# ColumbiaDVMM/ColumbiaImageSearch

Hardware: AMD Instinct MI355X
Metric: queries/sec @ recall@10 on 10M LOPQ index (higher is better)
Workload: dtype f64

## Files before the change

### columbiaimagesearch_amd/_lib.py

```python
import ctypes
import os
from ctypes import POINTER, c_char_p, c_double, c_float, c_int, c_int32, c_int64, c_uint8, c_uint16, c_uint32, c_void_p

import numpy as np

CIS_F32, CIS_F64 = 4, 8
CIS_OK, CIS_EINVAL, CIS_EHIP, CIS_ENOMEM, CIS_EUNSUPPORTED, CIS_ENODEVICE = 0, -1, -2, -3, -4, -5

_HERE = os.path.dirname(os.path.abspath(__file__))
LIB_PATH = os.environ.get("CIS_LIB_PATH") or os.path.join(_HERE, "lib", "libcis_hip.so")


class cis_hit(ctypes.Structure):
    _fields_ = [("dist", c_double), ("visit_rank", c_uint32), ("pos", c_uint32), ("id", c_int64),
                ("cell", c_int32), ("reserved", c_int32)]


HIT_DTYPE = np.dtype([("dist", "<f8"), ("visit_rank", "<u4"), ("pos", "<u4"), ("id", "<i8"),
                      ("cell", "<i4"), ("reserved", "<i4")])
assert HIT_DTYPE.itemsize == ctypes.sizeof(cis_hit) == 32


class HipError(RuntimeError):
    """A HIP runtime call inside libcis_hip.so failed (or no gfx950 device is visible)."""
# ... 7 lines not shown
    "cis_set_device": (c_int, [c_int]),
    "cis_selftest": (c_int, [POINTER(c_int)]),
    "cis_model_create": (c_int, [POINTER(c_void_p), c_int, c_int, c_int, c_int, c_int, c_int, c_void_p, c_void_p,
                                 c_void_p, c_void_p, c_void_p, c_void_p, c_int, c_int]),
    "cis_model_destroy": (None, [c_void_p]),
    "cis_apply_pca": (c_int, [c_void_p, c_void_p, c_int, c_int64, c_void_p]),
    "cis_encode": (c_int, [c_void_p, c_void_p, c_int, c_int64, c_void_p, c_void_p]),
    "cis_encode_dev": (c_int, [c_void_p, c_void_p, c_int, c_int64, c_void_p, c_void_p, c_void_p]),
    "cis_predict_coarse": (c_int, [c_void_p, c_void_p, c_int, c_int64, c_void_p]),
    "cis_project": (c_int, [c_void_p, c_void_p, c_int, c_int64, c_void_p, c_void_p]),
    "cis_predict_fine": (c_int, [c_void_p, c_void_p, c_int, c_int64, c_void_p, c_void_p]),
    "cis_subquantizer_distances": (c_int, [c_void_p, c_void_p, c_int, c_int64, c_void_p, c_void_p]),
    "cis_reconstruct": (c_int, [c_void_p, c_void_p, c_void_p, c_int64, c_void_p]),
    "cis_predict_cluster": (c_int, [c_void_p, c_int, c_void_p, c_int, c_int64, c_int, c_int, c_void_p]),
    "cis_multisequence": (c_int, [c_void_p, c_int, c_void_p, c_void_p, c_int, c_int64, c_int, c_int, c_int, c_void_p, c_void_p,
                                  POINTER(c_int)]),
    "cis_index_create": (c_int, [POINTER(c_void_p), c_void_p]),
    "cis_index_destroy": (None, [c_void_p]),
    "cis_index_create_view": (c_int, [POINTER(c_void_p), c_void_p]),
    "cis_index_insert_counters": (c_int, [c_void_p, c_void_p]),
    "cis_index_set_shard": (c_int, [c_void_p, c_int, c_int, c_void_p]),
    "cis_index_cell_counts": (c_int, [c_void_p, c_void_p]),
    "cis_index_add_remote_counts": (c_int, [c_void_p, c_void_p]),
    "cis_index_add": (c_int, [c_void_p, c_void_p, c_void_p, c_void_p, c_int64, c_int, POINTER(c_int64)]),
    "cis_index_size": (c_int64, [c_void_p]),
    "cis_index_add_dev": (c_int, [c_void_p, c_void_p, c_void_p, c_void_p, c_int64, c_int, POINTER(c_int64), POINTER(c_int64),
                                  c_void_p, c_void_p]),
    "cis_l2_normalize_dev": (c_int, [c_void_p, c_int, c_int64, c_int, c_void_p]),
    "cis_index_cell_counts_dev": (c_int, [c_void_p, c_void_p, c_void_p]),
    "cis_index_add_remote_counts_dev": (c_int, [c_void_p, c_void_p, c_void_p]),
    "cis_index_route_pack_dev": (c_int, [c_void_p, c_void_p, c_void_p, c_void_p, c_int64, c_void_p, c_void_p, c_void_p]),
    "cis_index_add_records_dev": (c_int, [c_void_p, c_void_p, c_int64, c_int, POINTER(c_int64), POINTER(c_int64), c_void_p,
                                          c_void_p]),
    "cis_index_get_cell": (c_int, [c_void_p, c_int, c_int, c_int64, c_void_p, c_void_p, POINTER(c_int64)]),
    "cis_index_get_codes": (c_int, [c_void_p, c_void_p, c_void_p, c_int64, c_void_p]),
    "cis_index_search": (c_int, [c_void_p, c_void_p, c_int, c_int, c_int64, c_int, c_void_p, c_void_p, c_void_p,
                                 c_void_p, c_void_p, c_void_p]),
    "cis_index_search_async": (c_int, [c_void_p, c_void_p, c_int, c_int, c_int64, c_int, c_void_p, c_void_p, c_void_p,
                                       c_void_p, c_void_p, c_void_p]),
    "cis_index_search_wait": (c_int, [c_void_p]),
    "cis_host_alloc": (c_int, [POINTER(c_void_p), ctypes.c_size_t]),
    "cis_host_free": (None, [c_void_p]),
    "cis_index_search_dev": (c_int, [c_void_p, c_void_p, c_int, c_int, c_int64, c_int, c_void_p, c_void_p, c_void_p,
                                     c_void_p, c_void_p, c_void_p, c_void_p]),
    "cis_index_search_partial_dev": (c_int, [c_void_p, c_void_p, c_int, c_int, c_int64, c_int, c_void_p, c_void_p,
                                             c_void_p]),
    "cis_index_query_owners_dev": (c_int, [c_void_p, c_void_p, c_int, c_int, c_int64, c_void_p, c_void_p, c_void_p]),
    "cis_routed_merge_tables_dev": (c_int, [c_void_p, c_int, c_int, c_void_p, c_void_p, c_int, c_void_p, c_void_p, c_void_p]),
    "cis_route_queries_dev": (c_int, [c_void_p, c_int, c_int, c_void_p, c_int, c_int, c_void_p, c_void_p, c_void_p, c_void_p, c_void_p]),
    "cis_index_search_partial_packed_dev": (c_int, [c_void_p, c_void_p, c_int, c_int, c_int64, c_int, c_void_p, c_void_p,
                                                    c_void_p, c_void_p, c_void_p, c_void_p]),
    "cis_merge_hits_dev": (c_int, [c_void_p, c_int, c_int, c_int, c_void_p, c_void_p, c_void_p, c_void_p, c_void_p,
                                   c_void_p]),
    "cis_merge_packed_dev": (c_int, [c_void_p, c_int, c_int64, c_void_p, c_void_p, c_int, c_int, c_void_p, c_void_p,
                                     c_void_p, c_void_p, c_void_p, c_void_p]),
    "cis_pyramid_down2_dev": (c_int, [c_void_p, c_int, c_int, c_void_p, c_void_p, c_void_p]),
    "cis_extract_chips_dev": (c_int, [c_void_p, c_int, c_int, c_void_p, c_int, c_int, c_void_p, c_void_p]),
    "cis_exchange_offsets_dev": (c_int, [c_void_p, c_int, c_int, c_int64, c_void_p, c_void_p, c_void_p, c_void_p]),
    "cis_rerank_dev": (c_int, [c_void_p, c_int, c_int64, c_int, c_void_p, c_int, c_void_p, c_int, c_void_p, c_void_p]),
    "cis_idmap_build_dev": (c_int, [c_void_p, c_int64, c_void_p, c_void_p, c_int64, c_void_p]),
    "cis_idmap_lookup_dev": (c_int, [c_void_p, c_void_p, c_int64, c_int64, c_void_p, c_int64, c_void_p, c_void_p]),
    "cis_rerank_select_dev": (c_int, [c_void_p, c_int, c_int64, c_int, c_void_p, c_void_p, c_int64, c_void_p, c_int, c_void_p,
                                      c_void_p, c_int, c_int, c_int, c_int, c_double, c_void_p, c_void_p, c_void_p, c_void_p,
                                      c_void_p]),
    "cis_exact_knn_dev": (c_int, [c_void_p, c_int, c_int64, c_int, c_void_p, c_int, c_int, c_int, c_int64, c_int, c_void_p, c_void_p,
                                  c_void_p]),
    "cis_exact_knn": (c_int, [c_void_p, c_int, c_int64, c_int, c_void_p, c_int, c_int, c_int, c_int64, c_int, c_void_p, c_void_p]),
    "cis_exact_knn_set_mode": (c_int, [c_int]),
    "cis_exact_knn_stats": (c_int, [c_void_p]),
    "cis_kmeans": (c_int, [c_void_p, c_int64, c_int, c_int, c_int, c_void_p, c_void_p, c_void_p]),
    "cis_train_gram": (c_int, [c_void_p, c_int64, c_int, c_void_p, c_int, c_void_p, c_void_p]),
    "cis_train_project": (c_int, [c_void_p, c_int64, c_int, c_void_p, c_int, c_void_p, c_void_p, c_void_p]),
    "cis_index_last_stats": (c_int, [c_void_p, c_void_p]),
    "cis_index_last_scan_kernel": (c_int, [c_void_p]),
    "cis_cnn_create": (c_int, [POINTER(c_void_p), c_int, c_void_p, c_int]),
    "cis_cnn_destroy": (None, [c_void_p]),
    "cis_cnn_create_view": (c_int, [POINTER(c_void_p), c_void_p]),
    "cis_cnn_feat_dim": (c_int, [c_int]),
    "cis_cnn_forward": (c_int, [c_void_p, c_void_p, c_int, c_void_p]),
    "cis_cnn_forward_dev": (c_int, [c_void_p, c_void_p, c_int, c_void_p, c_void_p]),
    "cis_index_set_profiling": (c_int, [c_void_p, c_int]),
    "cis_index_set_scan_mode": (c_int, [c_void_p, c_int]),
    "cis_index_stream_counters": (c_int, [c_void_p, c_void_p]),
    "cis_index_read_profile": (c_int, [c_void_p, c_void_p, POINTER(c_int64)]),
}

_lib = None


def exported_symbols():
    return sorted(_PROTOS)


def _load_hip_runtime():
    cands = []
    try:
        import torch
        cands.append(os.path.join(os.path.dirname(torch.__file__), "lib", "libamdhip64.so"))
    except ImportError:
        pass
    cands += ["libamdhip64.so.7", "/opt/rocm/lib/libamdhip64.so.7", "/opt/rocm/lib/libamdhip64.so", "libamdhip64.so"]
    for c in cands:
        try:
            return ctypes.CDLL(c, mode=ctypes.RTLD_GLOBAL)
        except OSError:
            continue
    raise ImportError("no HIP runtime (libamdhip64.so) found: install ROCm or PyTorch-ROCm")


def lib():
    global _lib
    if _lib is None:
        if not os.path.exists(LIB_PATH):
            raise ImportError(
                "%s not found: build it with `python -c 'import __graft_entry__ as g; g.build()'` "
                "(or `make -C columbiaimagesearch_amd/csrc`). columbiaimagesearch_amd has no CPU fallback." % LIB_PATH)
        _load_hip_runtime()
        L = ctypes.CDLL(LIB_PATH)
        for name, (res, args) in _PROTOS.items():
            fn = getattr(L, name)
            fn.restype = res
            fn.argtypes = args
        _lib = L
    return _lib


def last_error():
    return lib().cis_last_error().decode("utf-8", "replace")


def check(rc):
    if rc == CIS_OK:
        return
    msg = last_error()
    if rc == CIS_EINVAL:
        raise ValueError(msg)
    if rc == CIS_EUNSUPPORTED:
        raise NotImplementedError(msg)
    if rc == CIS_ENOMEM:
        raise MemoryError(msg)
    raise HipError(msg)


def ptr(a):
    if a is None:
        return None
    assert a.flags["C_CONTIGUOUS"]
    return a.ctypes.data_as(c_void_p)


def dtype_code(a):
    if a.dtype == np.float32:
        return CIS_F32
    if a.dtype == np.float64:
        return CIS_F64
    raise ValueError("only float32 / float64 vectors are supported, got %s" % a.dtype)


def as_float_matrix(x, cols=None):
    a = np.asarray(x)
    if a.dtype != np.float32 and a.dtype != np.float64:
        a = a.astype(np.float64)
    if a.ndim == 1:
        a = a[None, :]
    if a.ndim != 2:
        raise ValueError("expected a vector or a matrix of vectors, got shape %r" % (a.shape,))
# ... 41 lines not shown
```

### columbiaimagesearch_amd/csrc/lopq_batch.h

```cpp
#pragma once
#include <atomic>
#include <chrono>

#include "lopq_index.h"
#include "scan_common.h"

static const int GRP_SUB = 32;
#define GRP_WORDS(V) (6 * (V) * GRP_SUB + 2)
#define GRP_TILES(V) ((2 * (V) * GRP_SUB + 1023) / 1024)

static const int PLAN_PAR_STAGE = 4096;

struct Front {
    const void* xc;
    int ct;
    int* grp_cnt;
};

static const float* coarse_centroids(const cis_model* m, float) { return m->d_Cs32; }
static const double* coarse_centroids(const cis_model* m, double) { return m->d_Cs64; }

struct Scan2Geom { int G, NW, U, S; size_t lds; };

struct Route {
    bool w_pow2;
    bool split_tables;
    bool big;
    bool fast;
    bool tiny_cells;
    bool use3;
    bool stream_hint;
    bool par_plan, fused_front;
    int seg_max;
    int64_t stream_min;
    Scan2Geom geom;
    bool direct;
    bool stream;
    bool use5;
    bool drop_t32;
    Scan3Geom geom3;
    int S;
};

struct Batch {
    cis_index* ix;
    const void* dQ;
    int q_dtype, nq;
    int64_t quota;
    int L;
    SearchOut out;
    hipStream_t st;
    Front f;
    PlanOut* plan;
    int64_t *item_off, *tab_off, *totals;
    unsigned long long* qbound;
    int *grp_cur, *grp_base;
    int* plan_fb;
    uint64_t* vis_list;
    int vis_cap;
    unsigned long long* plan_hint;
    int hint_slot;
    const int64_t* d_tot;
    int64_t n_items, n_tabs, n_cand_all;
    WorkItem* items;
    TabDesc* tabs;
    int* tab_order;
    double *T, *px_buf;
    float* T32;
    cis_index::ProfRec pr;
    std::chrono::steady_clock::time_point t_entry;
};

static int mark(Batch& b, int i) {
    if (!b.ix->profiling) return CIS_OK;
    if (b.ix->profiling == 1 && i != 5 && i != 3) return CIS_OK;
    CIS_CHECK_HIP(hipEventCreate(&b.pr.ev[i]));
    CIS_CHECK_HIP(hipEventRecord(b.pr.ev[i], b.st));
    return CIS_OK;
}

struct Slots {
    int* qctr;
    int* n_slots;
    int* fhdr;
    int* slots;
    int* fslots;
    int64_t max_slots;
};
enum SlotMode {
    SLOTS_SORTED,
    SLOTS_IDENTITY,
    SLOTS_NONE
};

int front_prepare(cis_index* ix, const void* dQ, int q_dtype, int nq, hipStream_t st, Front* f);
template <typename CT>
int front_count(Batch& b, const Route& r);
int dump_plan_fallbacks(const Batch& b);
int plan_totals(Batch& b, const Route& r);
template <typename CT>
void emit_plan(Batch& b, const Route& r);
int build_slots(const Batch& b, SlotMode mode, int G, int64_t CH , int seg_max, Slots* s);
```

### columbiaimagesearch_amd/csrc/lopq_host.hip

```cpp
#include <algorithm>
#include <mutex>

#include "lopq_index.h"

static std::mutex g_copy_mu;
static hipStream_t g_copy_stream[64] = {nullptr};
static int cis_copy_stream(int device, hipStream_t* out) {
    std::lock_guard<std::mutex> lk(g_copy_mu);
    const int d = device & 63;
    if (!g_copy_stream[d]) CIS_CHECK_HIP(hipStreamCreateWithFlags(&g_copy_stream[d], hipStreamNonBlocking));
    *out = g_copy_stream[d];
    return CIS_OK;
}

static std::vector<cis_index*> g_host_pending;

static hipError_t host_copy_out_locked(cis_index* ix, hipStream_t cp) {
    const cis_index::HostOut& o = ix->h_out;
    const int nq = o.nq, L = o.L;
    hipError_t e = hipSuccess;
    auto cpy = [&](void* dst, const void* src, size_t bytes) { if (e == hipSuccess && dst) e = hipMemcpyAsync(dst, src, bytes, hipMemcpyDeviceToHost, cp); };
    if (nq > 0) {
        if (L > 0) {
            cpy(o.ids, ix->w_oids.p, (size_t)nq * L * sizeof(int64_t));
// ... 13 lines not shown
    for (size_t i = 0; i < g_host_pending.size();) {
        cis_index* o = g_host_pending[i];
        if (o != self && o->m->device == device && hipEventQuery(o->h_ev_out) == hipSuccess && host_copy_out_locked(o, cp) == hipSuccess) {
            g_host_pending[i] = g_host_pending.back();
            g_host_pending.pop_back();
        } else {
            ++i;
        }
    }
    (void)hipGetLastError();
}

void cis_host_forget(cis_index* ix) {
    std::lock_guard<std::mutex> lk(g_copy_mu);
    g_host_pending.erase(std::remove(g_host_pending.begin(), g_host_pending.end(), ix), g_host_pending.end());
}

static void host_abandon(cis_index* ix) {
    std::lock_guard<std::mutex> lk(g_copy_mu);
    g_host_pending.erase(std::remove(g_host_pending.begin(), g_host_pending.end(), ix), g_host_pending.end());
    ix->h_out = {nullptr, nullptr, nullptr, nullptr, nullptr, nullptr, 0, 0};
}

extern "C" int cis_host_alloc(void** out, size_t bytes) {
    CIS_REQUIRE(out != nullptr, "out is NULL");
    *out = nullptr;
    CIS_TRY(cis_lazy_init());
    hipError_t e = hipHostMalloc(out, bytes > 0 ? bytes : 1, hipHostMallocDefault);
    if (e != hipSuccess) {
        cis_set_error("hipHostMalloc(%zu) failed: %s", bytes, hipGetErrorString(e));
        *out = nullptr;
        return CIS_ENOMEM;
    }
    return CIS_OK;
}

extern "C" void cis_host_free(void* p) {
    if (p) (void)hipHostFree(p);
}

extern "C" int cis_index_search_wait(cis_index* ix);

extern "C" int cis_index_search_async(cis_index* ix, const void* Q, int q_dtype, int nq, int64_t quota, int limit,
                                      int64_t* ids, double* dists, int32_t* n_found, int32_t* visited, int32_t* cells,
                                      uint32_t* pos) {
    CIS_REQUIRE(ix != nullptr, "index is NULL");
    CIS_REQUIRE(q_dtype == CIS_F32 || q_dtype == CIS_F64, "q_dtype must be 4 or 8");
    int L;
    CIS_TRY(effective_limit(quota, limit, &L));
    if (nq == 0) return CIS_OK;
    CIS_REQUIRE(Q && n_found && visited && (L == 0 || (ids && dists)), "NULL buffer");
    CIS_TRY(cis_lazy_init());
    CIS_CHECK_HIP(hipSetDevice(ix->m->device));
    hipStream_t cp = nullptr;
    CIS_TRY(cis_copy_stream(ix->m->device, &cp));
    if (!ix->h_stream) {
        CIS_CHECK_HIP(hipStreamCreateWithFlags(&ix->h_stream, hipStreamNonBlocking));
        CIS_CHECK_HIP(hipEventCreateWithFlags(&ix->h_ev_in, hipEventDisableTiming));
        CIS_CHECK_HIP(hipEventCreateWithFlags(&ix->h_ev_out, hipEventDisableTiming));
        CIS_CHECK_HIP(hipEventCreateWithFlags(&ix->h_ev_done, hipEventDisableTiming));
    }
    hipStream_t st = ix->h_stream;
    if (ix->h_pending) CIS_TRY(cis_index_search_wait(ix));
    const size_t qbytes = (size_t)nq * ix->m->D_in * q_dtype;
    const int Lk = L > 0 ? L : 1;
    CIS_TRY(ix->w_q.reserve(qbytes));
    CIS_TRY(ix->w_oids.reserve((size_t)nq * Lk * sizeof(int64_t)));
    CIS_TRY(ix->w_odists.reserve((size_t)nq * Lk * sizeof(double)));
    CIS_TRY(ix->w_onf.reserve((size_t)nq * sizeof(int32_t)));
    CIS_TRY(ix->w_ovis.reserve((size_t)nq * sizeof(int32_t)));
    CIS_TRY(ix->w_ocell.reserve((size_t)nq * Lk * sizeof(int32_t)));
    CIS_TRY(ix->w_opos.reserve((size_t)nq * Lk * sizeof(uint32_t)));
    {
        std::lock_guard<std::mutex> lk(g_copy_mu);
        CIS_CHECK_HIP(hipMemcpyAsync(ix->w_q.p, Q, qbytes, hipMemcpyHostToDevice, cp));
        CIS_CHECK_HIP(hipEventRecord(ix->h_ev_in, cp));
        host_pump_locked(ix->m->device, cp, ix);
    }
    struct Guard {
        cis_index* ix; hipStream_t st; bool armed;
        ~Guard() { if (armed) { (void)hipStreamSynchronize(st); ix->h_pending = false; host_abandon(ix); } }
    } guard{ix, st, true};
    CIS_CHECK_HIP(hipStreamWaitEvent(st, ix->h_ev_in, 0));
    int rc = cis_index_search_dev(ix, ix->w_q.p, q_dtype, nq, quota, limit, ix->w_oids.as<int64_t>(),
                                  ix->w_odists.as<double>(), ix->w_onf.as<int32_t>(), ix->w_ovis.as<int32_t>(),
                                  ix->w_ocell.as<int32_t>(), ix->w_opos.as<uint32_t>(), st);
    if (rc != CIS_OK) return rc;
    CIS_CHECK_HIP(hipEventRecord(ix->h_ev_out, st));
    ix->h_out = {ids, dists, n_found, visited, cells, pos, nq, L};
    ix->h_out_enqueued = false;
    ix->h_pending = true;
    guard.armed = false;
    {
        std::lock_guard<std::mutex> lk(g_copy_mu);
        g_host_pending.push_back(ix);
    }
    return CIS_OK;
}

static int host_wait_pending(cis_index* ix) {
    CIS_CHECK_HIP(hipSetDevice(ix->m->device));
    ix->h_pending = false;
    hipStream_t cp = nullptr;
    CIS_TRY(cis_copy_stream(ix->m->device, &cp));
    bool enq;
    {
        std::lock_guard<std::mutex> lk(g_copy_mu);
        enq = ix->h_out_enqueued;
    }
    if (!enq) {
        CIS_CHECK_HIP(hipEventSynchronize(ix->h_ev_out));
        std::lock_guard<std::mutex> lk(g_copy_mu);
        if (!ix->h_out_enqueued) {
            g_host_pending.erase(std::remove(g_host_pending.begin(), g_host_pending.end(), ix), g_host_pending.end());
            CIS_CHECK_HIP(host_copy_out_locked(ix, cp));
        }
        host_pump_locked(ix->m->device, cp, ix);
    }
    CIS_CHECK_HIP(hipEventSynchronize(ix->h_ev_done));
    return CIS_OK;
}

extern "C" int cis_index_search_wait(cis_index* ix) {
    CIS_REQUIRE(ix != nullptr, "index is NULL");
    if (!(ix->h_stream && ix->h_pending)) return CIS_OK;
    const int rc = host_wait_pending(ix);
    if (rc != CIS_OK) {
        ix->h_pending = false;
        host_abandon(ix);
    }
    return rc;
}

extern "C" int cis_index_search(cis_index* ix, const void* Q, int q_dtype, int nq, int64_t quota, int limit,
                                int64_t* ids, double* dists, int32_t* n_found, int32_t* visited, int32_t* cells,
                                uint32_t* pos) {
    CIS_TRY(cis_index_search_async(ix, Q, q_dtype, nq, quota, limit, ids, dists, n_found, visited, cells, pos));
    return cis_index_search_wait(ix);
}
```

### columbiaimagesearch_amd/csrc/lopq_index.h

```cpp
#pragma once
#include "lopq_model.h"

struct CellStore {
    DevBuf codes[2];
    DevBuf ids[2];
    DevBuf loff[2];
    DevBuf cmax;
    int cur = 0;
    int64_t n = 0;
    int64_t cap = 0;
    bool with_codes = true;
    bool init = false;
    void release() {
        for (int i = 0; i < 2; ++i) { codes[i].release(); ids[i].release(); loff[i].release(); }
        cmax.release();
    }
};

struct cis_index {
    cis_model* m = nullptr;
    int V = 0, M = 0;
    int64_t ncells = 0;
    int rank = 0, world = 1;
    std::vector<int32_t> owner;
    DevBuf d_owner;
    CellStore own;
    CellStore ghost;
    DevBuf d_gcount;
    DevBuf d_plan_hint;
    bool had_plain_remote = false;
    int64_t nb_indexed = 0;
    bool stats_fresh = false;
    int64_t n_inplace = 0, n_rebuild = 0;
    cis_index* base = nullptr;
    std::vector<cis_index*> views;
    bool orphaned = false;
    const cis_index* st() const { return base ? base : this; }
    const uint8_t* codes_ptr() const { const cis_index* s = st(); return s->own.codes[s->own.cur].as<uint8_t>(); }
    const int64_t* ids_ptr() const { const cis_index* s = st(); return s->own.ids[s->own.cur].as<int64_t>(); }
    const int64_t* loff_ptr() const { const cis_index* s = st(); return s->own.loff[s->own.cur].as<int64_t>(); }
    const int64_t* gcount_ptr() const { return st()->d_gcount.as<int64_t>(); }
    unsigned long long* plan_hint_ptr() const { return st()->d_plan_hint.as<unsigned long long>(); }
    void sync_from_base() {
        if (!base) return;
        ncells = base->ncells; rank = base->rank; world = base->world; nb_indexed = base->nb_indexed; n_local = base->n_local;
        n_total = base->n_total; max_cell = base->max_cell; nonempty_cells = base->nonempty_cells;
    }
    int64_t n_local = 0;
    DevBuf wi_key[2], wi_val[2], wi_hist, wi_sid, wi_acc, wi_apre, wi_tmp, wi_in_ids, wi_in_coarse, wi_in_fine, wi_scan, wi_cnt, wi_cnt2;
    DevBuf d_stats;
    int64_t* h_ins = nullptr;
    DevBuf w_slack;
    DevBuf w_planfb, w_vis;
    DevBuf w_tiles;
    DevBuf w_xp, w_cd, w_order, w_sorted, w_plan, w_off, w_items, w_tabs, w_T, w_hits, w_hitn, w_part, w_q,
        w_oids, w_odists, w_onf, w_ovis, w_ocell, w_opos, w_order2, w_px, w_T32, w_grp, w_tord, w_y64, w_x64;
    int64_t stats[4] = {0, 0, 0, 0};
    bool force_exact_scan = false;
    bool force_scan2 = false;
    bool force_scan3 = false;
    int force_two_pass = -1;
    int batch_hint = 0;
    int64_t batch_hint_quota = -1;
    double retry_fraction = 0.5;
    int m16_holdoff = 0;
    int64_t m16_backoffs = 0;
    int last_scan_kernel = 0;
    bool force_prefilter_scan = false;
    hipStream_t h_stream = nullptr;
    hipEvent_t h_ev_in = nullptr, h_ev_out = nullptr, h_ev_done = nullptr;
    bool h_pending = false;
    bool h_out_enqueued = false;
    struct HostOut { int64_t* ids; double* dists; int32_t* n_found; int32_t* visited; int32_t* cells; uint32_t* pos; int nq, L; };
    HostOut h_out = {nullptr, nullptr, nullptr, nullptr, nullptr, nullptr, 0, 0};
    bool force_scan5 = false;
    DevBuf w_s5;
    DevBuf w_bmin;
    bool force_stream = false;
    bool stream_off = false;
    int64_t stream_batches = 0, stream_fallbacks = 0;
    int profiling = 0;
    int64_t* h_totals = nullptr;
    int64_t* d_h_totals = nullptr;
    int64_t plan_seq = 0;
    int64_t stats_pending_seq = 0;
    int64_t n_total = 0, max_cell = 0, nonempty_cells = 0;
    struct ProfRec { hipEvent_t ev[6]; bool has_scan; };
    std::vector<ProfRec> prof;
    double prof_ms[5] = {0, 0, 0, 0, 0};
    int64_t prof_launches = 0;

    bool owns(int64_t cell) const {
        if (world <= 1) return true;
        if (!owner.empty()) return owner[cell] == rank;
        return (int)(cell % world) == rank;
    }
};

int cis_index_ready(cis_index* ix);

void cis_host_forget(cis_index* ix);

static const int MAX_LDS_LIMIT = 3072;
static const int MAX_LIMIT = 1 << 24;

static inline int effective_limit(int64_t quota, int limit, int* L) {
    int64_t l = limit < 0 ? quota : limit;
    if (l < 0) l = 0;
    if (l > MAX_LIMIT) {
        cis_set_error("limit=%lld exceeds the %d ranked results per query supported by this build", (long long)l, MAX_LIMIT);
        return CIS_EUNSUPPORTED;
    }
    *L = (int)l;
    return CIS_OK;
}

int cis_search_partial(cis_index* ix, const void* dQ, int q_dtype, int nq, int64_t quota, int L, cis_hit* d_hits, int32_t* d_n_found,
                       int32_t* d_visited, hipStream_t st);
```

### columbiaimagesearch_amd/csrc/lopq_index.hip

```cpp
#include <algorithm>

#include "lopq_index.h"

static const int SCAN_T = 256, SCAN_PER = 8, SCAN_TILE = SCAN_T * SCAN_PER;

template <typename T>
__device__ __forceinline__ T wave_incl_scan(T v) {
    const int lane = threadIdx.x & 63;
#pragma unroll
    for (int o = 1; o < 64; o <<= 1) {
        const T u = __shfl_up(v, o);
        if (lane >= o) v += u;
    }
    return v;
}

template <typename T>
__device__ __forceinline__ T block_excl_scan(T v, T* sh , T* total) {
    const int lane = threadIdx.x & 63, w = threadIdx.x >> 6;
    const T inc = wave_incl_scan(v);
    if (lane == 63) sh[w] = inc;
    __syncthreads();
    T base = 0, tot = 0;
#pragma unroll
// ... 31 lines not shown
template <typename TO>
__global__ __launch_bounds__(SCAN_T) void k_scan_sums(TO* __restrict__ sums, int64_t m, TO* __restrict__ total, int64_t* __restrict__ total2) {
    __shared__ TO sh[SCAN_T / 64 + 1];
    TO carry = 0;
    for (int64_t b = 0; b < m; b += SCAN_T) {
        const int64_t i = b + threadIdx.x;
        const TO v = i < m ? sums[i] : (TO)0;
        TO tot;
        const TO e = block_excl_scan<TO>(v, sh, &tot);
        if (i < m) sums[i] = carry + e;
        carry += tot;
    }
    if (threadIdx.x == 0) {
        if (total) total[0] = carry;
        if (total2) total2[0] = (int64_t)carry;
    }
}

template <typename TO>
__global__ __launch_bounds__(SCAN_T) void k_scan_add(TO* __restrict__ out, const TO* __restrict__ sums, int64_t n) {
    const TO add = sums[blockIdx.x];
    const int64_t base = (int64_t)blockIdx.x * SCAN_TILE + (int64_t)threadIdx.x * SCAN_PER;
#pragma unroll
    for (int i = 0; i < SCAN_PER; ++i)
        if (base + i < n) out[base + i] += add;
}

template <typename TI, typename TO>
static void dev_exclusive_scan(const TI* in, TO* out, int64_t n, TO* sums, TO* total, int64_t* total2, hipStream_t st) {
    const int64_t m = n > 0 ? ceil_div(n, SCAN_TILE) : 0;
    if (m > 0) hipLaunchKernelGGL((k_scan_tiles<TI, TO>), dim3((unsigned)m), dim3(SCAN_T), 0, st, in, out, sums, n);
    hipLaunchKernelGGL((k_scan_sums<TO>), dim3(1), dim3(SCAN_T), 0, st, sums, m, total, total2);
    if (m > 1) hipLaunchKernelGGL((k_scan_add<TO>), dim3((unsigned)m), dim3(SCAN_T), 0, st, out, (const TO*)sums, n);
}

static const int RS_ROWS = 32, RS_TILE = RS_ROWS * 64;

__global__ __launch_bounds__(64) void k_rs_hist(const uint32_t* __restrict__ key, int64_t n, int shift, uint32_t* __restrict__ H, int nblk) {
    __shared__ uint32_t h[256];
    for (int i = threadIdx.x; i < 256; i += 64) h[i] = 0;
    __syncthreads();
    const int64_t base = (int64_t)blockIdx.x * RS_TILE;
    for (int r = 0; r < RS_ROWS; ++r) {
        const int64_t i = base + r * 64 + threadIdx.x;
        if (i < n) atomicAdd(&h[(key[i] >> shift) & 255u], 1u);
    }
    __syncthreads();
    for (int d = threadIdx.x; d < 256; d += 64) H[(int64_t)d * nblk + blockIdx.x] = h[d];
}

__global__ __launch_bounds__(64) void k_rs_scatter(const uint32_t* __restrict__ key, const uint32_t* __restrict__ val, int64_t n, int shift,
                                                   const uint32_t* __restrict__ H, int nblk, uint32_t* __restrict__ key_out,
                                                   uint32_t* __restrict__ val_out) {
    __shared__ uint32_t base[256];
    for (int d = threadIdx.x; d < 256; d += 64) base[d] = H[(int64_t)d * nblk + blockIdx.x];
    __syncthreads();
    const int lane = threadIdx.x;
    const int64_t b0 = (int64_t)blockIdx.x * RS_TILE;
    for (int r = 0; r < RS_ROWS; ++r) {
        const int64_t i = b0 + r * 64 + lane;
        const bool ok = i < n;
        const uint32_t k = ok ? key[i] : 0u;
        const uint32_t v = ok ? val[i] : 0u;
        const uint32_t d = (k >> shift) & 255u;
        unsigned long long peers = __ballot(ok);
#pragma unroll
        for (int b = 0; b < 8; ++b) {
            const unsigned long long m = __ballot((d >> b) & 1u);
            peers &= ((d >> b) & 1u) ? m : ~m;
        }
        const int before = __builtin_amdgcn_mbcnt_hi((unsigned)(peers >> 32), __builtin_amdgcn_mbcnt_lo((unsigned)peers, 0));
        const uint32_t start = base[d];
        __syncthreads();
        if (ok) {
            key_out[start + before] = k;
            val_out[start + before] = v;
            if (before == 0) base[d] = start + (uint32_t)__popcll(peers);
        }
        __syncthreads();
    }
}

enum { INS_ACC_OWN = 0, INS_INVALID = 1, INS_NTOTAL = 2, INS_MAXCELL = 3, INS_NONEMPTY = 4, INS_ERR = 5, INS_ACC_GHOST = 6,
       INS_REMOTE_PLAIN = 7, INS_OVERFLOW = 8, INS_WORDS = 9 };

__device__ __forceinline__ bool dev_owns(int64_t cell, const int32_t* __restrict__ owner, int rank, int world) {
    if (world <= 1) return true;
    return owner ? owner[cell] == rank : (int)(cell % world) == rank;
}

__global__ void k_ins_keys(const int64_t* __restrict__ ids, const uint16_t* __restrict__ coarse, const uint8_t* __restrict__ fine,
                           int64_t n, int V, int M, int K, const int32_t* __restrict__ owner, int rank, int world, int sel,
                           int dedup, uint32_t* __restrict__ key, uint32_t* __restrict__ val, int64_t* __restrict__ idv,
                           int64_t* __restrict__ gcount, int64_t* __restrict__ stats) {
    const int64_t i = (int64_t)blockIdx.x * blockDim.x + threadIdx.x;
    if (i >= n) return;
    const int c0 = coarse[2 * i], c1 = coarse[2 * i + 1];
    const int64_t id = ids[i];
    bool valid = c0 < V && c1 < V && id >= 0;
    if (valid && K < 256) {
        for (int j = 0; j < M; ++j) valid = valid && fine[i * M + j] < K;
    }
    uint32_t k = 0;
    int64_t keep = -1;
    if (!valid) {
        if (sel == 0) atomicAdd((unsigned long long*)&stats[INS_INVALID], 1ull);
    } else {
        const int64_t cell = (int64_t)c0 * V + c1;
        const bool mine = dev_owns(cell, owner, rank, world);
        if (mine == (sel == 0)) {
            k = (uint32_t)cell;
            keep = id;
        } else if (sel == 0 && !dedup) {
            atomicAdd((unsigned long long*)&gcount[cell], 1ull);
            atomicAdd((unsigned long long*)&stats[INS_REMOTE_PLAIN], 1ull);
        }
    }
    key[i] = k;
    val[i] = (uint32_t)i;
    idv[i] = keep;
}

__global__ void k_ins_gather(const int64_t* __restrict__ idv, const uint32_t* __restrict__ perm, int64_t n, int64_t* __restrict__ sid) {
    const int64_t j = (int64_t)blockIdx.x * blockDim.x + threadIdx.x;
    if (j < n) sid[j] = idv[perm[j]];
}

__device__ __forceinline__ int64_t lower_bound_u32(const uint32_t* __restrict__ a, int64_t n, uint32_t x) {
    int64_t lo = 0, hi = n;
    while (lo < hi) {
        const int64_t mid = (lo + hi) >> 1;
        if (a[mid] < x) lo = mid + 1;
        else hi = mid;
    }
    return lo;
}

__global__ __launch_bounds__(256) void k_ins_dedup(const uint32_t* __restrict__ key, const int64_t* __restrict__ sid, int64_t n, int dedup,
                                                   const int64_t* __restrict__ loff, const int64_t* __restrict__ lend,
                                                   const int64_t* __restrict__ old_ids, const unsigned long long* __restrict__ cmaxp,
                                                   uint32_t* __restrict__ acc) {
    const int64_t j = (int64_t)blockIdx.x * 4 + (threadIdx.x >> 6);
    const int lane = threadIdx.x & 63;
    if (j >= n) return;
    const int64_t id = sid[j];
    uint32_t a = id >= 0 ? 1u : 0u;
    if (a && dedup) {
        const uint32_t c = key[j];
        bool dup = false;
        if ((unsigned long long)id < cmaxp[c]) {
            const int64_t b = loff[c], e = lend[c];
            for (int64_t p0 = b; p0 < e && !dup; p0 += 64) {
                const int64_t p = p0 + lane;
                dup = __ballot(p < e && old_ids[p] == id) != 0ull;
            }
        }
        if (!dup) {
            const int64_t first = lower_bound_u32(key, n, c);
            for (int64_t j0 = first; j0 < j && !dup; j0 += 64) {
                const int64_t jj = j0 + lane;
                dup = __ballot(jj < j && sid[jj] == id) != 0ull;
            }
        }
        a = dup ? 0u : 1u;
    }
    if (lane == 0) acc[j] = a;
}
// ... 224 lines not shown
    if (on) {
        const int64_t dst = lend[c] + (int64_t)(pre - s_pre[l0]);
        const bool fits = dst < loff[c + 1];
        if (!fits) { s_over = 1; stats[INS_OVERFLOW] = 1; }
        const int64_t id = sid[j];
        if (fits) {
            ids_cur[dst] = id;
            if (codes_cur) {
                const int64_t i = perm[j];
                for (int bb = 0; bb < M; ++bb) codes_cur[dst * M + bb] = fine[i * M + bb];
            }
        }
        v = (unsigned long long)id + 1ull;
    }
    const uint32_t cm = on ? c : 0xffffffffu;
#pragma unroll
    for (int o = 1; o < 64; o <<= 1) {
        const unsigned long long u = __shfl_up(v, o);
        const uint32_t cu = __shfl_up(cm, o);
        if (lane >= o && cu == cm && u > v) v = u;
    }
    const uint32_t cn = __shfl_down(cm, 1);
    if (on && (lane == 63 || cn != cm)) atomicMax(&cmaxp[c], v);
    __threadfence();
    __syncthreads();
    if (s_over != 0) return;
    if (j < n && (j + 1 >= n || s_key[j + 1] != c)) {
        const int64_t add = (int64_t)(pre + a) - (int64_t)s_pre[l0];
        if (add > 0) {
            lend[c] += add;
            gcount[c] += add;
        }
    }
    if (!do_stats) return;
    __threadfence();
    __syncthreads();
    long long sum = 0, mx = 0, ne = 0;
    for (int64_t cc = j; cc < ncells; cc += 1024) {
        const long long g = gcount[cc];
        sum += g;
        mx = g > mx ? g : mx;
        ne += g > 0;
    }
    for (int o = 32; o > 0; o >>= 1) {
        sum += __shfl_xor(sum, o);
        const long long m2 = __shfl_xor(mx, o);
        mx = m2 > mx ? m2 : mx;
        ne += __shfl_xor(ne, o);
    }
    if (lane == 0) { s_sum[wv] = sum; s_max[wv] = mx; s_ne[wv] = ne; }
    __syncthreads();
    if (j == 0) {
        for (int w = 1; w < 16; ++w) { sum += s_sum[w]; mx = s_max[w] > mx ? s_max[w] : mx; ne += s_ne[w]; }
        stats[INS_NTOTAL] = sum; stats[INS_MAXCELL] = mx; stats[INS_NONEMPTY] = ne;
    }
}

__global__ __launch_bounds__(256) void k_gcount_stats(const int64_t* __restrict__ gcount, int64_t ncells, int64_t* __restrict__ stats) {
    __shared__ long long s_sum[4], s_max[4], s_ne[4];
    long long sum = 0, mx = 0, ne = 0;
    for (int64_t c = (int64_t)blockIdx.x * blockDim.x + threadIdx.x; c < ncells; c += (int64_t)gridDim.x * blockDim.x) {
        const long long g = gcount[c];
        sum += g;
        mx = g > mx ? g : mx;
        ne += g > 0;
    }
    for (int o = 32; o > 0; o >>= 1) {
        sum += __shfl_xor(sum, o);
        const long long m2 = __shfl_xor(mx, o);
        mx = m2 > mx ? m2 : mx;
        ne += __shfl_xor(ne, o);
    }
    const int w = threadIdx.x >> 6;
    if ((threadIdx.x & 63) == 0) { s_sum[w] = sum; s_max[w] = mx; s_ne[w] = ne; }
    __syncthreads();
    if (threadIdx.x == 0) {
        for (int i = 1; i < 4; ++i) { sum += s_sum[i]; mx = s_max[i] > mx ? s_max[i] : mx; ne += s_ne[i]; }
        atomicAdd((unsigned long long*)&stats[INS_NTOTAL], (unsigned long long)sum);
        atomicMax((unsigned long long*)&stats[INS_MAXCELL], (unsigned long long)mx);
        atomicAdd((unsigned long long*)&stats[INS_NONEMPTY], (unsigned long long)ne);
    }
}

__global__ void k_cell_delta(const int64_t* __restrict__ gcount, int64_t* __restrict__ delta, int64_t ncells) {
    const int64_t c = (int64_t)blockIdx.x * blockDim.x + threadIdx.x;
    if (c < ncells) delta[c] = gcount[c] - delta[c];
}

__global__ void k_add_remote(int64_t* __restrict__ gcount, const int64_t* __restrict__ delta, int64_t ncells,
                             const int32_t* __restrict__ owner, int rank, int world, int64_t* __restrict__ stats) {
    const int64_t c = (int64_t)blockIdx.x * blockDim.x + threadIdx.x;
    if (c >= ncells) return;
    const int64_t d = delta[c];
    if (d < 0) { stats[INS_ERR] = 1; return; }
    if (d == 0 || dev_owns(c, owner, rank, world)) return;
    gcount[c] += d;
}

__global__ void k_get_codes(const int32_t* __restrict__ cells, const uint32_t* __restrict__ pos, int64_t n, int64_t ncells,
                            const int64_t* __restrict__ loff, const uint8_t* __restrict__ codes, int M, uint8_t* __restrict__ out,
                            int64_t* __restrict__ stats) {
    const int64_t i = (int64_t)blockIdx.x * blockDim.x + threadIdx.x;
    if (i >= n) return;
    const int64_t c = cells[i];
    if (c < 0 || c >= ncells) { stats[INS_ERR] = 1 + i; return; }
    const int64_t a = loff[c], b = loff[ncells + 1 + c];
    if ((int64_t)pos[i] >= b - a) { stats[INS_ERR] = 1 + i; return; }
    for (int j = 0; j < M; ++j) out[i * M + j] = codes[(a + pos[i]) * M + j];
}

__global__ void k_route_keys(const uint16_t* __restrict__ coarse, int64_t n, int V, const int32_t* __restrict__ owner, int world,
                             uint32_t* __restrict__ key, uint32_t* __restrict__ val, int64_t* __restrict__ counts) {
    const int64_t i = (int64_t)blockIdx.x * blockDim.x + threadIdx.x;
    if (i >= n) return;
    const int c0 = coarse[2 * i], c1 = coarse[2 * i + 1];
    uint32_t dst = 0;
    if (c0 < V && c1 < V) {
        const int64_t cell = (int64_t)c0 * V + c1;
        dst = (uint32_t)(owner ? owner[cell] : (int)(cell % world));
    }
    key[i] = dst;
    val[i] = (uint32_t)i;
    atomicAdd((unsigned long long*)&counts[dst], 1ull);
}

__global__ void k_route_pack(const uint32_t* __restrict__ perm, const int64_t* __restrict__ ids, const uint16_t* __restrict__ coarse,
                             const uint8_t* __restrict__ fine, int64_t n, int M, uint8_t* __restrict__ rec) {
    const int64_t j = (int64_t)blockIdx.x * blockDim.x + threadIdx.x;
    if (j >= n) return;
    const int64_t i = perm[j];
    uint8_t* r = rec + j * (12 + M);
    const int64_t id = ids[i];
    for (int b = 0; b < 8; ++b) r[b] = (uint8_t)((uint64_t)id >> (8 * b));
    const uint16_t c0 = coarse[2 * i], c1 = coarse[2 * i + 1];
    r[8] = (uint8_t)c0; r[9] = (uint8_t)(c0 >> 8); r[10] = (uint8_t)c1; r[11] = (uint8_t)(c1 >> 8);
    for (int b = 0; b < M; ++b) r[12 + b] = fine[i * M + b];
}

__global__ void k_route_unpack(const uint8_t* __restrict__ rec, int64_t n, int M, int64_t* __restrict__ ids, uint16_t* __restrict__ coarse,
                               uint8_t* __restrict__ fine) {
    const int64_t j = (int64_t)blockIdx.x * blockDim.x + threadIdx.x;
    if (j >= n) return;
    const uint8_t* r = rec + j * (12 + M);
    uint64_t id = 0;
    for (int b = 0; b < 8; ++b) id |= (uint64_t)r[b] << (8 * b);
    ids[j] = (int64_t)id;
    coarse[2 * j] = (uint16_t)(r[8] | (r[9] << 8));
    coarse[2 * j + 1] = (uint16_t)(r[10] | (r[11] << 8));
    for (int b = 0; b < M; ++b) fine[j * M + b] = r[12 + b];
}

static inline unsigned grid_for(int64_t n, int t) { return (unsigned)(n > 0 ? ceil_div(n, t) : 1); }

static int store_init(cis_index* ix, CellStore& s, bool with_codes) {
    if (s.init) return CIS_OK;
    const int64_t nc = ix->ncells;
    s.with_codes = with_codes;
    for (int g = 0; g < 2; ++g) CIS_TRY(s.loff[g].reserve((size_t)(2 * nc + 1) * sizeof(int64_t)));
    CIS_TRY(s.cmax.reserve((size_t)nc * sizeof(int64_t)));
    CIS_TRY(s.ids[0].reserve(256));
    if (with_codes) CIS_TRY(s.codes[0].reserve(256));
    CIS_CHECK_HIP(hipMemset(s.loff[0].p, 0, (size_t)(2 * nc + 1) * sizeof(int64_t)));
    CIS_CHECK_HIP(hipMemset(s.cmax.p, 0, (size_t)nc * sizeof(int64_t)));
    s.cur = 0;
    s.n = 0;
    s.init = true;
    return CIS_OK;
}

int cis_index_ready(cis_index* ix) {
    CIS_REQUIRE(ix->base == nullptr, "this handle is a search view (cis_index_create_view): inserts and reads go to the base index");
    if (ix->own.init && ix->h_ins) return CIS_OK;
    CIS_TRY(cis_lazy_init());
    CIS_CHECK_HIP(hipSetDevice(ix->m->device));
    CIS_TRY(store_init(ix, ix->own, true));
    if (!ix->d_gcount.p) {
        CIS_TRY(ix->d_gcount.reserve((size_t)ix->ncells * sizeof(int64_t)));
        CIS_CHECK_HIP(hipMemset(ix->d_gcount.p, 0, (size_t)ix->ncells * sizeof(int64_t)));
    }
    if (!ix->d_plan_hint.p) {
        CIS_TRY(ix->d_plan_hint.reserve(4 * sizeof(unsigned long long)));
        CIS_CHECK_HIP(hipMemset(ix->d_plan_hint.p, 0, 4 * sizeof(unsigned long long)));
    }
    if (!ix->owner.empty() && !ix->d_owner.p) {
        CIS_TRY(ix->d_owner.reserve((size_t)ix->ncells * sizeof(int32_t)));
        CIS_CHECK_HIP(hipMemcpy(ix->d_owner.p, ix->owner.data(), (size_t)ix->ncells * sizeof(int32_t), hipMemcpyHostToDevice));
    }
    if (!ix->h_ins) {
        CIS_TRY(ix->d_stats.reserve(INS_WORDS * sizeof(int64_t)));
        CIS_CHECK_HIP(hipMemset(ix->d_stats.p, 0, INS_WORDS * sizeof(int64_t)));
        CIS_CHECK_HIP(hipHostMalloc((void**)&ix->h_ins, INS_WORDS * sizeof(int64_t), hipHostMallocDefault));
        for (int i = 0; i < INS_WORDS; ++i) ix->h_ins[i] = 0;
    }
    return CIS_OK;
}

extern "C" int cis_index_create(cis_index** out, cis_model* m) {
    CIS_REQUIRE(out != nullptr, "out is NULL");
    *out = nullptr;
    CIS_REQUIRE(m != nullptr, "model is NULL");
    cis_index* ix = new cis_index();
    ix->m = m;
    ix->V = m->V;
    ix->M = m->M;
    ix->ncells = (int64_t)m->V * m->V;
    *out = ix;
    return CIS_OK;
}

extern "C" int cis_index_create_view(cis_index** out, cis_index* base) {
    CIS_REQUIRE(out != nullptr, "out is NULL");
    *out = nullptr;
    CIS_REQUIRE(base != nullptr, "base index is NULL");
    CIS_REQUIRE(base->base == nullptr, "a view of a view: create views from the base index");
    cis_index* ix = new cis_index();
    ix->m = base->m;
    ix->V = base->V;
    ix->M = base->M;
    ix->base = base;
    ix->force_exact_scan = base->force_exact_scan; ix->force_scan2 = base->force_scan2; ix->force_scan3 = base->force_scan3;
    ix->force_two_pass = base->force_two_pass; ix->force_prefilter_scan = base->force_prefilter_scan; ix->force_stream = base->force_stream; ix->force_scan5 = base->force_scan5;
    ix->sync_from_base();
    base->views.push_back(ix);
    *out = ix;
    return CIS_OK;
}

extern "C" void cis_index_destroy(cis_index* ix) {
    if (!ix) return;
    if (ix->m) (void)hipSetDevice(ix->m->device);
    if (ix->base) {
        std::vector<cis_index*>& v = ix->base->views;
        for (size_t i = 0; i < v.size(); ++i)
            if (v[i] == ix) { v.erase(v.begin() + i); break; }
    }
    for (cis_index* v : ix->views) { v->base = nullptr; v->orphaned = true; }
    ix->views.clear();
    cis_host_forget(ix);
    if (ix->h_stream) {
        if (ix->h_pending && ix->h_ev_done) (void)hipEventSynchronize(ix->h_ev_done);
        (void)hipStreamSynchronize(ix->h_stream);
        (void)hipStreamDestroy(ix->h_stream);
        ix->h_stream = nullptr;
        for (hipEvent_t e : {ix->h_ev_in, ix->h_ev_out, ix->h_ev_done})
            if (e) (void)hipEventDestroy(e);
    }
    DevBuf* bufs[] = {&ix->d_gcount, &ix->d_plan_hint, &ix->d_owner, &ix->w_xp, &ix->w_cd, &ix->w_order,
                      &ix->w_sorted, &ix->w_plan, &ix->w_off, &ix->w_items, &ix->w_tabs, &ix->w_T, &ix->w_hits,
                      &ix->w_hitn, &ix->w_slack, &ix->w_planfb, &ix->w_vis, &ix->w_tiles, &ix->w_part, &ix->w_q, &ix->w_oids, &ix->w_odists, &ix->w_onf, &ix->w_ovis,
                      &ix->w_ocell, &ix->w_opos, &ix->w_order2, &ix->w_px, &ix->w_T32, &ix->w_grp, &ix->w_tord, &ix->w_y64, &ix->w_x64,
                      &ix->wi_key[0], &ix->wi_key[1], &ix->wi_val[0], &ix->wi_val[1], &ix->wi_hist, &ix->wi_sid, &ix->wi_acc,
                      &ix->w_s5, &ix->w_bmin, &ix->wi_apre, &ix->wi_tmp, &ix->wi_in_ids, &ix->wi_in_coarse, &ix->wi_in_fine, &ix->wi_scan, &ix->wi_cnt, &ix->wi_cnt2, &ix->d_stats};
    for (DevBuf* b : bufs) b->release();
    ix->own.release();
    ix->ghost.release();
    if (ix->h_totals) (void)hipHostFree(ix->h_totals);
    if (ix->h_ins) (void)hipHostFree(ix->h_ins);
    delete ix;
}

extern "C" int cis_index_set_shard(cis_index* ix, int rank, int world, const int32_t* owner) {
    CIS_REQUIRE(ix != nullptr, "index is NULL");
    CIS_REQUIRE(world >= 1 && rank >= 0 && rank < world, "bad shard %d of %d", rank, world);
    CIS_REQUIRE(ix->nb_indexed == 0, "set_shard must be called on an empty index");
    ix->rank = rank;
    ix->world = world;
    ix->owner.clear();
    ix->d_owner.release();
    if (owner) {
        ix->owner.assign(owner, owner + ix->ncells);
        for (int64_t c = 0; c < ix->ncells; ++c)
            CIS_REQUIRE(owner[c] >= 0 && owner[c] < world, "owner[%lld]=%d out of range", (long long)c, owner[c]);
    }
    return CIS_OK;
}
// ... 11 lines not shown
    const int64_t hn = (int64_t)256 * nblk;
    CIS_TRY(ix->wi_hist.reserve((size_t)hn * sizeof(uint32_t)));
    CIS_TRY(ix->wi_scan.reserve((size_t)(ceil_div(hn, SCAN_TILE) + 2) * sizeof(int64_t) + 64));
    int gen = 0;
    for (int shift = 0; shift < bits; shift += 8) {
        uint32_t* k0 = ix->wi_key[gen].as<uint32_t>();
        uint32_t* v0 = ix->wi_val[gen].as<uint32_t>();
        uint32_t* k1 = ix->wi_key[1 - gen].as<uint32_t>();
        uint32_t* v1 = ix->wi_val[1 - gen].as<uint32_t>();
        uint32_t* H = ix->wi_hist.as<uint32_t>();
        hipLaunchKernelGGL(k_rs_hist, dim3(nblk), dim3(64), 0, st, (const uint32_t*)k0, n, shift, H, nblk);
        dev_exclusive_scan<uint32_t, uint32_t>(H, H, hn, ix->wi_scan.as<uint32_t>(), nullptr, nullptr, st);
        hipLaunchKernelGGL(k_rs_scatter, dim3(nblk), dim3(64), 0, st, (const uint32_t*)k0, (const uint32_t*)v0, n, shift,
                           (const uint32_t*)H, nblk, k1, v1);
        gen = 1 - gen;
    }
    *gen_out = gen;
    return CIS_OK;
}

static int slack_const(const cis_index* ix) {
    static const int env = getenv("CIS_INSERT_SLACK") ? atoi(getenv("CIS_INSERT_SLACK")) : -2;
    if (env != -2) return env;
    return ix->ncells <= 65536 ? 32 : 2;
}
static const int64_t INPLACE_MAX = 65536;

static int store_merge(cis_index* ix, CellStore& s, int sel, const int64_t* d_ids, const uint16_t* d_coarse, const uint8_t* d_fine,
                       int64_t n, int dedup, int acc_word, hipStream_t st) {
    const int M = ix->M, V = ix->V, K = ix->m->K;
    const int64_t nc = ix->ncells;
    CIS_REQUIRE(n < ((int64_t)1 << 31), "at most 2^31 - 1 items per insert call");
    ix->stats_fresh = false;
    for (int g = 0; g < 2; ++g) {
        CIS_TRY(ix->wi_key[g].reserve((size_t)n * sizeof(uint32_t)));
        CIS_TRY(ix->wi_val[g].reserve((size_t)n * sizeof(uint32_t)));
    }
    CIS_TRY(ix->wi_tmp.reserve((size_t)n * sizeof(int64_t)));
    CIS_TRY(ix->wi_sid.reserve((size_t)n * sizeof(int64_t)));
    CIS_TRY(ix->wi_acc.reserve((size_t)n * sizeof(uint32_t)));
    CIS_TRY(ix->wi_apre.reserve((size_t)(n + 2) * sizeof(uint32_t)));
    CIS_TRY(ix->wi_scan.reserve((size_t)(ceil_div(std::max<int64_t>(std::max<int64_t>(n, nc + 1), (int64_t)256 * ceil_div(n, RS_TILE)), SCAN_TILE) + 2) * sizeof(int64_t) + 64));
    const int32_t* d_owner = ix->d_owner.as<int32_t>();
    int64_t* stats = ix->d_stats.as<int64_t>();
    int64_t* gcount = ix->d_gcount.as<int64_t>();
    static const bool no_small = getenv("CIS_INS_NO_SMALL") != nullptr;
    const bool small = n > 0 && n <= INS_SMALL && !no_small;
    int gen = 0;
    int64_t* sid = ix->wi_sid.as<int64_t>();
    if (small) {
        gen = 1;
        hipLaunchKernelGGL(k_ins_small_sort, dim3(1), dim3(1024), 0, st, d_ids, d_coarse, d_fine, (int)n, V, M, K, d_owner, ix->rank, ix->world, sel,
                           dedup, ix->wi_key[1].as<uint32_t>(), ix->wi_val[1].as<uint32_t>(), ix->wi_tmp.as<int64_t>(), sid, gcount, stats);
    } else {
        hipLaunchKernelGGL(k_ins_keys, dim3(grid_for(n, 256)), dim3(256), 0, st, d_ids, d_coarse, d_fine, n, V, M, K, d_owner, ix->rank,
                           ix->world, sel, dedup, ix->wi_key[0].as<uint32_t>(), ix->wi_val[0].as<uint32_t>(), ix->wi_tmp.as<int64_t>(),
                           gcount, stats);
        CIS_TRY(radix_sort_pairs(ix, n, key_bits(nc), st, &gen));
    }
    const uint32_t* skey = ix->wi_key[gen].as<uint32_t>();
    const uint32_t* perm = ix->wi_val[gen].as<uint32_t>();
    uint32_t* acc = ix->wi_acc.as<uint32_t>();
    uint32_t* apre = ix->wi_apre.as<uint32_t>();
    uint32_t* total = apre + n;
    int64_t* loff = s.loff[s.cur].as<int64_t>();
    int64_t* lend = loff + nc + 1;
    unsigned long long* cmaxp = s.cmax.as<unsigned long long>();
    if (!small) hipLaunchKernelGGL(k_ins_gather, dim3(grid_for(n, 256)), dim3(256), 0, st, (const int64_t*)ix->wi_tmp.as<int64_t>(), perm, n, sid);
    hipLaunchKernelGGL(k_ins_dedup, dim3(grid_for(n, 4)), dim3(256), 0, st, skey, (const int64_t*)sid, n, dedup, (const int64_t*)loff,
                       (const int64_t*)lend, (const int64_t*)s.ids[s.cur].as<int64_t>(), (const unsigned long long*)cmaxp, acc);
    const int slack = slack_const(ix);
    int64_t* gsink = gcount;
    const bool small_place = small && slack >= 0 && s.n > 0;
    if (!small_place) dev_exclusive_scan<uint32_t, uint32_t>(acc, apre, n, ix->wi_scan.as<uint32_t>(), total, stats + acc_word, st);
    if (small_place) {
        uint8_t* codes_cur = s.with_codes ? s.codes[s.cur].as<uint8_t>() : nullptr;
        const int do_stats = nc <= 65536 ? 1 : 0;
        hipLaunchKernelGGL(k_ins_small_place, dim3(1), dim3(1024), 0, st, skey, perm, (const int64_t*)sid, (const uint32_t*)acc, apre, (int)n, acc_word,
                           (const int64_t*)loff, lend, d_fine, M, s.ids[s.cur].as<int64_t>(), codes_cur, cmaxp, gsink, nc, do_stats, stats);
        if (!do_stats) {
            CIS_CHECK_HIP(hipMemsetAsync(stats + INS_NTOTAL, 0, 3 * sizeof(int64_t), st));
            hipLaunchKernelGGL(k_gcount_stats, dim3((unsigned)std::min<int64_t>(ceil_div(nc, 256), 1024)), dim3(256), 0, st, (const int64_t*)gcount, nc, stats);
        }
        CIS_CHECK_HIP(hipGetLastError());
        CIS_CHECK_HIP(hipMemcpyAsync(ix->h_ins, ix->d_stats.p, INS_WORDS * sizeof(int64_t), hipMemcpyDeviceToHost, st));
        CIS_CHECK_HIP(hipStreamSynchronize(st));
        if (ix->h_ins[INS_OVERFLOW] == 0) {
            s.n += ix->h_ins[acc_word];
            if (sel == 0) ix->n_inplace += 1;
            ix->n_total = ix->h_ins[INS_NTOTAL];
            ix->max_cell = ix->h_ins[INS_MAXCELL];
            ix->nonempty_cells = ix->h_ins[INS_NONEMPTY];
            ix->nb_indexed = ix->n_total;
            ix->stats_fresh = true;
            return CIS_OK;
        }
        CIS_CHECK_HIP(hipMemsetAsync(stats + INS_OVERFLOW, 0, sizeof(int64_t), st));
    }
    if (!small_place && slack >= 0 && s.n > 0 && n <= INPLACE_MAX) {
        uint8_t* codes_cur = s.with_codes ? s.codes[s.cur].as<uint8_t>() : nullptr;
        hipLaunchKernelGGL((k_ins_scatter<true>), dim3(grid_for(n, 256)), dim3(256), 0, st, skey, perm, (const int64_t*)sid, (const uint32_t*)acc,
                           (const uint32_t*)apre, n, (const int64_t*)loff, (const int64_t*)lend, (const int64_t*)nullptr, (const uint32_t*)nullptr,
                           d_fine, M, s.ids[s.cur].as<int64_t>(), codes_cur, cmaxp, stats);
        hipLaunchKernelGGL(k_ins_commit, dim3(grid_for(n, 256)), dim3(256), 0, st, skey, (const uint32_t*)acc, (const uint32_t*)apre, n, lend,
                           gsink, (const int64_t*)stats);
        CIS_CHECK_HIP(hipMemsetAsync(stats + INS_NTOTAL, 0, 3 * sizeof(int64_t), st));
        hipLaunchKernelGGL(k_gcount_stats, dim3((unsigned)std::min<int64_t>(ceil_div(nc, 256), 1024)), dim3(256), 0, st, (const int64_t*)gcount, nc, stats);
        CIS_CHECK_HIP(hipGetLastError());
        CIS_CHECK_HIP(hipMemcpyAsync(ix->h_ins, ix->d_stats.p, INS_WORDS * sizeof(int64_t), hipMemcpyDeviceToHost, st));
        CIS_CHECK_HIP(hipStreamSynchronize(st));
        if (ix->h_ins[INS_OVERFLOW] == 0) {
            s.n += ix->h_ins[acc_word];
            if (sel == 0) ix->n_inplace += 1;
            ix->n_total = ix->h_ins[INS_NTOTAL];
            ix->max_cell = ix->h_ins[INS_MAXCELL];
            ix->nonempty_cells = ix->h_ins[INS_NONEMPTY];
            ix->nb_indexed = ix->n_total;
            ix->stats_fresh = true;
            return CIS_OK;
        }
        CIS_CHECK_HIP(hipMemsetAsync(stats + INS_OVERFLOW, 0, sizeof(int64_t), st));
    }
    const int nxt = 1 - s.cur;
    const int64_t items_bound = s.n + n;
    const int64_t cap_new_bound = slack < 0 ? items_bound : items_bound + items_bound / 8 + (int64_t)slack * nc + 64;
    CIS_TRY(s.ids[nxt].reserve((size_t)(cap_new_bound > 0 ? cap_new_bound : 1) * sizeof(int64_t)));
    if (s.with_codes) CIS_TRY(s.codes[nxt].reserve((size_t)(cap_new_bound > 0 ? cap_new_bound : 1) * M + 64));
    CIS_TRY(ix->wi_cnt.reserve((size_t)(2 * nc + 2) * sizeof(int64_t) + (size_t)(nc + 1) * sizeof(uint32_t)));
    int64_t* cnt_new = ix->wi_cnt.as<int64_t>();
    int64_t* cap_new = cnt_new + nc + 1;
    uint32_t* a0v = reinterpret_cast<uint32_t*>(cap_new + nc + 1);
    int64_t* noff = s.loff[nxt].as<int64_t>();
    int64_t* nend = noff + nc + 1;
    hipLaunchKernelGGL(k_ins_counts, dim3(grid_for(nc, 256)), dim3(256), 0, st, skey, (const uint32_t*)apre, (const uint32_t*)total, n, nc,
                       (const int64_t*)loff, (const int64_t*)lend, cnt_new, cap_new, a0v, gsink, slack);
    dev_exclusive_scan<int64_t, int64_t>(cap_new, noff, nc, ix->wi_scan.as<int64_t>(), noff + nc, nullptr, st);
    hipLaunchKernelGGL(k_ins_ends, dim3(grid_for(nc, 256)), dim3(256), 0, st, (const int64_t*)noff, (const int64_t*)cnt_new, nc, nend);
    const uint8_t* ocodes = s.with_codes ? s.codes[s.cur].as<uint8_t>() : nullptr;
    uint8_t* ncodes = s.with_codes ? s.codes[nxt].as<uint8_t>() : nullptr;
    if (s.n > 0) {
        if (s.n / nc < 16 && nc >= 65536) {
            hipLaunchKernelGGL(k_ins_move_cells, dim3(grid_for(nc, 256)), dim3(256), 0, st, (const int64_t*)loff, (const int64_t*)lend, (const int64_t*)noff, nc,
                               (const int64_t*)s.ids[s.cur].as<int64_t>(), ocodes, M, s.ids[nxt].as<int64_t>(), ncodes);
        } else {
#define CIS_MOVE(MW)                                                                                                             \
    hipLaunchKernelGGL((k_ins_move<MW>), dim3(grid_for(s.cap, 256)), dim3(256), 0, st, (const int64_t*)loff, (const int64_t*)lend, (const int64_t*)noff, nc, s.cap, \
                       (const int64_t*)s.ids[s.cur].as<int64_t>(), ocodes, M, s.ids[nxt].as<int64_t>(), ncodes)
            if (M == 4) CIS_MOVE(1);
            else if (M == 8) CIS_MOVE(2);
            else if (M == 16) CIS_MOVE(4);
            else if (M == 32) CIS_MOVE(8);
            else CIS_MOVE(0);
#undef CIS_MOVE
        }
    }
    hipLaunchKernelGGL((k_ins_scatter<false>), dim3(grid_for(n, 256)), dim3(256), 0, st, skey, perm, (const int64_t*)sid, (const uint32_t*)acc,
                       (const uint32_t*)apre, n, (const int64_t*)loff, (const int64_t*)lend, (const int64_t*)noff, (const uint32_t*)a0v, d_fine, M,
                       s.ids[nxt].as<int64_t>(), ncodes, cmaxp, stats);
    CIS_CHECK_HIP(hipGetLastError());
    CIS_CHECK_HIP(hipMemcpyAsync(ix->h_ins, ix->d_stats.p, INS_WORDS * sizeof(int64_t), hipMemcpyDeviceToHost, st));
    CIS_CHECK_HIP(hipStreamSynchronize(st));
    s.n += ix->h_ins[acc_word];
    if (sel == 0) ix->n_rebuild += 1;
    s.cap = cap_new_bound;
    s.cur = nxt;
    return CIS_OK;
}

static int stats_zero(cis_index* ix, hipStream_t st) {
    CIS_CHECK_HIP(hipMemsetAsync(ix->d_stats.p, 0, INS_WORDS * sizeof(int64_t), st));
    return CIS_OK;
}

static int stats_fetch(cis_index* ix, hipStream_t st) {
    CIS_CHECK_HIP(hipMemcpyAsync(ix->h_ins, ix->d_stats.p, INS_WORDS * sizeof(int64_t), hipMemcpyDeviceToHost, st));
    CIS_CHECK_HIP(hipStreamSynchronize(st));
    return CIS_OK;
}

static int refresh_stats(cis_index* ix, hipStream_t st) {
    int64_t* stats = ix->d_stats.as<int64_t>();
    CIS_CHECK_HIP(hipMemsetAsync(stats + INS_NTOTAL, 0, 3 * sizeof(int64_t), st));
    const int64_t nc = ix->ncells;
    const unsigned grid = (unsigned)std::min<int64_t>(ceil_div(nc, 256), 1024);
    hipLaunchKernelGGL(k_gcount_stats, dim3(grid), dim3(256), 0, st, (const int64_t*)ix->d_gcount.as<int64_t>(), nc, stats);
    CIS_TRY(stats_fetch(ix, st));
    ix->n_total = ix->h_ins[INS_NTOTAL];
    ix->max_cell = ix->h_ins[INS_MAXCELL];
    ix->nonempty_cells = ix->h_ins[INS_NONEMPTY];
    ix->nb_indexed = ix->n_total;
    return CIS_OK;
}

static const int64_t DEDUP_CHUNK = 262144;
static const int64_t PLAIN_CHUNK = (int64_t)1 << 28;

static int index_add_dev(cis_index* ix, const int64_t* d_ids, const uint16_t* d_coarse, const uint8_t* d_fine, int64_t n, int dedup,
                         int64_t* n_added, int64_t* n_invalid, int64_t* d_cell_delta, hipStream_t st) {
    CIS_TRY(cis_index_ready(ix));
    CIS_CHECK_HIP(hipSetDevice(ix->m->device));
    if (n_added) *n_added = 0;
    if (n_invalid) *n_invalid = 0;
    if (d_cell_delta) {
        if (n == 0) CIS_CHECK_HIP(hipMemsetAsync(d_cell_delta, 0, (size_t)ix->ncells * sizeof(int64_t), st));
        else CIS_CHECK_HIP(hipMemcpyAsync(d_cell_delta, ix->d_gcount.p, (size_t)ix->ncells * sizeof(int64_t), hipMemcpyDeviceToDevice, st));
    }
    if (n == 0) return CIS_OK;
    const bool sharded = ix->world > 1;
    if (dedup && ix->had_plain_remote) {
        cis_set_error("dedup add after plain (dedup=0) adds that counted other shards' cells is not supported on a sharded index");
        return CIS_EUNSUPPORTED;
    }
    const int64_t chunk = dedup ? DEDUP_CHUNK : PLAIN_CHUNK;
    int64_t added = 0, invalid = 0;
    for (int64_t a = 0; a < n; a += chunk) {
        const int64_t bn = std::min(chunk, n - a);
        ix->stats_fresh = false;
        CIS_TRY(stats_zero(ix, st));
        CIS_TRY(store_merge(ix, ix->own, 0, d_ids + a, d_coarse + 2 * a, d_fine + a * ix->M, bn, dedup, INS_ACC_OWN, st));
        if (sharded && dedup) {
            const int64_t seen = ix->h_ins[INS_ACC_OWN] + ix->h_ins[INS_INVALID];
            added += ix->h_ins[INS_ACC_OWN];
            invalid += ix->h_ins[INS_INVALID];
            bool foreign = seen < bn;
            if (foreign) {
                CIS_TRY(store_init(ix, ix->ghost, false));
                CIS_TRY(store_merge(ix, ix->ghost, 1, d_ids + a, d_coarse + 2 * a, d_fine + a * ix->M, bn, 1, INS_ACC_GHOST, st));
                added += ix->h_ins[INS_ACC_GHOST];
            }
        } else {
            added += ix->h_ins[INS_ACC_OWN] + ix->h_ins[INS_REMOTE_PLAIN];
            invalid += ix->h_ins[INS_INVALID];
            if (ix->h_ins[INS_REMOTE_PLAIN] > 0) ix->had_plain_remote = true;
        }
    }
    ix->n_local = ix->own.n;
    if (d_cell_delta)
        hipLaunchKernelGGL(k_cell_delta, dim3(grid_for(ix->ncells, 256)), dim3(256), 0, st, (const int64_t*)ix->d_gcount.as<int64_t>(),
                           d_cell_delta, ix->ncells);
    if (!ix->stats_fresh) CIS_TRY(refresh_stats(ix, st));
    if (n_added) *n_added = added;
    if (n_invalid) *n_invalid = invalid;
    return CIS_OK;
}

extern "C" int cis_index_add_dev(cis_index* ix, const int64_t* d_ids, const uint16_t* d_coarse, const uint8_t* d_fine, int64_t n,
                                 int dedup, int64_t* n_added, int64_t* n_invalid, int64_t* d_cell_delta, void* stream) {
    CIS_REQUIRE(ix != nullptr, "index is NULL");
    CIS_REQUIRE(n >= 0 && (n == 0 || (d_ids && d_coarse && d_fine)), "NULL buffer");
    return index_add_dev(ix, d_ids, d_coarse, d_fine, n, dedup, n_added, n_invalid, d_cell_delta, (hipStream_t)stream);
}

extern "C" int cis_index_add(cis_index* ix, const int64_t* ids, const uint16_t* coarse, const uint8_t* fine,
                             int64_t n, int dedup, int64_t* n_added) {
    CIS_REQUIRE(ix != nullptr, "index is NULL");
    CIS_REQUIRE(n >= 0 && (n == 0 || (ids && coarse && fine)), "NULL buffer");
    const int V = ix->V, M = ix->M, K = ix->m->K;
    for (int64_t i = 0; i < n; ++i)
        CIS_REQUIRE(coarse[2 * i] < V && coarse[2 * i + 1] < V, "item %lld: coarse code out of range (V=%d)",
                    (long long)i, V);
    if (K < 256)
        for (int64_t i = 0; i < n * M; ++i)
            CIS_REQUIRE(fine[i] < K, "fine code %d out of range (K=%d)", (int)fine[i], K);
    for (int64_t i = 0; i < n; ++i) CIS_REQUIRE(ids[i] >= 0, "item %lld: ids must be >= 0", (long long)i);
    if (n_added) *n_added = 0;
    if (n == 0) return CIS_OK;
    CIS_TRY(cis_index_ready(ix));
    CIS_CHECK_HIP(hipSetDevice(ix->m->device));
    CIS_TRY(ix->wi_in_ids.reserve((size_t)n * sizeof(int64_t)));
    CIS_TRY(ix->wi_in_coarse.reserve((size_t)n * 2 * sizeof(uint16_t)));
    CIS_TRY(ix->wi_in_fine.reserve((size_t)n * M));
    CIS_CHECK_HIP(hipMemcpy(ix->wi_in_ids.p, ids, (size_t)n * sizeof(int64_t), hipMemcpyHostToDevice));
    CIS_CHECK_HIP(hipMemcpy(ix->wi_in_coarse.p, coarse, (size_t)n * 2 * sizeof(uint16_t), hipMemcpyHostToDevice));
// ... 174 lines not shown
```

### columbiaimagesearch_amd/csrc/lopq_plan.hip

```cpp
#include "lopq_batch.h"

template <typename CT>
__global__ void k_rank(const CT* __restrict__ dist , int nq, int V,
                       uint16_t* __restrict__ order , CT* __restrict__ sorted ,
                       int* __restrict__ grp ) {
    extern __shared__ __attribute__((aligned(16))) char smem[];
    uint64_t* sb = reinterpret_cast<uint64_t*>(smem);
    const int q = blockIdx.x, s = blockIdx.y;
    if (q == 0 && s == 0)
        for (int i = threadIdx.x; i < 4 * V * GRP_SUB; i += blockDim.x) grp[i] = 0;
    const CT* d = dist + ((int64_t)s * nq + q) * V;
    for (int v = threadIdx.x; v < V; v += blockDim.x) sb[v] = f2bits(d[v]);
    __syncthreads();
    for (int v = threadIdx.x; v < V; v += blockDim.x) {
        const uint64_t mine = sb[v];
        int r = 0;
        for (int u = 0; u < V; ++u) {
            const uint64_t o = sb[u];
            r += (o < mine) || (o == mine && u < v);
        }
        order[((int64_t)q * 2 + s) * V + r] = (uint16_t)v;
        sorted[((int64_t)q * 2 + s) * V + r] = d[v];
    }
}
// ... 20 lines not shown
            const uint32_t oij = __shfl_xor(bij, off);
            if (ok < bk || (ok == bk && oij < bij)) { bk = ok; bij = oij; }
        }
    } else {
        bij = (uint32_t)__builtin_amdgcn_readfirstlane((int)bij);
    }
    return bij;
}

static __device__ __forceinline__ void walk_advance(int* t, int& rows, int V, int lane, int bi, int bj) {
    __syncthreads();
    if (lane == 0) t[bi] = bj + 1;
    if (bi + 2 > rows) rows = (bi + 2 < V) ? bi + 2 : V;
    __syncthreads();
}

template <typename CT, bool FIRST_ALONE, bool LISTS, typename Visit>
static __device__ __forceinline__ int walk_quota(const CT* d0, const CT* d1, const uint16_t* o0, const uint16_t* o1, int* t, int V, int lane,
                                                 const int64_t* __restrict__ gcount, const int64_t* __restrict__ loff, int64_t quota, Visit visit) {
    int visited = 0;
    int64_t retrieved = 0;
    int rows = 1;
    const int64_t total_cells = (int64_t)V * V;
    while ((int64_t)visited < total_cells) {
        const uint32_t bij = walk_step<CT, FIRST_ALONE>(d0, d1, t, rows, V, lane);
        if (bij == WALK_NONE) break;
        const int bi = (int)(bij >> 16), bj = (int)(bij & 0xffff);
        const int c0 = o0[bi], c1 = o1[bj];
        const int64_t cell = (int64_t)c0 * V + c1;
        const int64_t gc = gcount[cell];
        int64_t ls = 0, ll = 0;
        if constexpr (LISTS) {
            ls = loff[cell];
            ll = loff[(int64_t)V * V + 1 + cell] - ls;
        }
        visit(visited, bi, bj, cell, gc, ls, ll);
        visited += 1;
        retrieved += gc;
        walk_advance(t, rows, V, lane, bi, bj);
        if (retrieved >= quota) break;
    }
    return visited;
}

static __device__ __forceinline__ void count_table_group(int* __restrict__ grp_cnt, int g, int q) {
    atomicAdd(&grp_cnt[g * GRP_SUB + (q % GRP_SUB)], 1);
}

static __device__ __forceinline__ void walk_count_out(PlanOut* __restrict__ plan, int* __restrict__ grp_cnt, const uint16_t* o0, const uint16_t* o1,
                                                      int V, int q, int lane, int visited, int n_items, int max_i, int max_j, int64_t ncand) {
    if (lane == 0) {
        PlanOut p;
        p.visited = visited; p.n_items = n_items; p.ntab0 = max_i + 1; p.ntab1 = max_j + 1; p.ncand = ncand;
        plan[q] = p;
    }
    for (int i = lane; i < max_i + 1 + max_j + 1; i += 64)
        count_table_group(grp_cnt, i <= max_i ? (int)o0[i] : V + (int)o1[i - (max_i + 1)], q);
}

static __device__ __forceinline__ void emit_chunks(WorkItem* __restrict__ dst, int q, int rank, int tab0, int tab1, int64_t cell, int64_t ls,
                                                   int64_t ll, int seg_max, int nch, int ch0, int step) {
    for (int ch = ch0; ch < nch; ch += step) {
        WorkItem it;
        it.q = q; it.rank = rank;
        it.tab0 = tab0;
        it.tab1 = tab1;
        it.pos0 = ch * seg_max;
        it.cell = (int)cell; it.pad = 0;
        it.start = ls + (int64_t)ch * seg_max;
        const int64_t rem = ll - (int64_t)ch * seg_max;
        it.len = (int)(rem < seg_max ? rem : seg_max);
        dst[ch] = it;
    }
}

template <typename CT, bool EMIT>
__global__ __launch_bounds__(64) void k_plan(const CT* __restrict__ sorted, const uint16_t* __restrict__ order,
                                             const int64_t* __restrict__ gcount, const int64_t* __restrict__ loff,
                                             int nq, int V, int64_t quota, int seg_max, PlanOut* __restrict__ plan,
                                             const int64_t* __restrict__ item_off, const int64_t* __restrict__ tab_off,
                                             WorkItem* __restrict__ items, TabDesc* __restrict__ tabs,
                                             int* __restrict__ grp_cnt , const int* __restrict__ grp_base ,
                                             int* __restrict__ grp_cur , int* __restrict__ tab_order ,
                                             const int* __restrict__ only ) {
    extern __shared__ __attribute__((aligned(16))) char smem[];
    int* t = reinterpret_cast<int*>(smem);
    const int q = blockIdx.x;
    const int lane = threadIdx.x;
    if (only && !only[q]) return;
    const CT* d0 = sorted + ((int64_t)q * 2 + 0) * V;
    const CT* d1 = sorted + ((int64_t)q * 2 + 1) * V;
    const uint16_t* o0 = order + ((int64_t)q * 2 + 0) * V;
    const uint16_t* o1 = order + ((int64_t)q * 2 + 1) * V;
    for (int i = lane; i < V; i += 64) t[i] = 0;
    __syncthreads();
    int n_items = 0, max_i = -1, max_j = -1;
    int64_t ncand = 0;
    int64_t ibase = 0, tbase = 0;
    int ntab0 = 0;
    if (EMIT) {
        ibase = item_off[q];
        tbase = tab_off[q];
        ntab0 = plan[q].ntab0;
    }
    const int visited = walk_quota<CT, false, true>(d0, d1, o0, o1, t, V, lane, gcount, loff, quota,
                                                    [&](int rank, int bi, int bj, int64_t cell, int64_t, int64_t ls, int64_t ll) {
        if (ll > 0) {
            const int nch = (int)((ll + seg_max - 1) / seg_max);
            if (EMIT) emit_chunks(items + ibase + n_items, q, rank, (int)(tbase + bi), (int)(tbase + ntab0 + bj), cell, ls, ll, seg_max, nch, lane, 64);
            n_items += nch;
            ncand += ll;
            max_i = bi > max_i ? bi : max_i;
            max_j = bj > max_j ? bj : max_j;
        }
    });
    if (!EMIT) {
        walk_count_out(plan, grp_cnt, o0, o1, V, q, lane, visited, n_items, max_i, max_j, ncand);
    } else {
        const int nt0 = plan[q].ntab0, nt1 = plan[q].ntab1;
        for (int i = lane; i < nt0 + nt1; i += 64) {
            TabDesc td;
            td.q = q; td.pad = 0;
            if (i < nt0) { td.split = 0; td.cluster = o0[i]; }
            else { td.split = 1; td.cluster = o1[i - nt0]; }
            tabs[tbase + i] = td;
            const int g = (td.split * V + td.cluster) * GRP_SUB + (q % GRP_SUB);
            tab_order[grp_base[g] + atomicAdd(&grp_cur[g], 1)] = (int)(tbase + i);
        }
    }
}

template <typename CT>
__global__ __launch_bounds__(64) void k_front_small(const CT* __restrict__ X , int D, int h, const CT* __restrict__ Cs ,
                                                    PwProg prog, const int64_t* __restrict__ gcount, const int64_t* __restrict__ loff,
                                                    int nq, int V, int64_t quota, int seg_max, uint16_t* __restrict__ order ,
                                                    CT* __restrict__ sorted , PlanOut* __restrict__ plan,
                                                    int* __restrict__ grp_cnt ) {
    extern __shared__ __attribute__((aligned(16))) char smem[];
    uint64_t* sb = reinterpret_cast<uint64_t*>(smem);
    CT* sd = reinterpret_cast<CT*>(sb + 2 * V);
    uint16_t* so = reinterpret_cast<uint16_t*>(sb + 4 * V);
    int* t = reinterpret_cast<int*>(so + 2 * V);
    const int q = blockIdx.x, lane = threadIdx.x;
    const CT* xr = X + (int64_t)q * D;
    for (int e = lane; e < 2 * V; e += 64) {
        const int s = e / V, c = e - s * V;
        const CT* x = xr + s * h;
        const CT* cc = Cs + ((int64_t)s * V + c) * h;
        auto elem = [&](int i) -> CT { const CT df = x[i] - cc[i]; return df * df; };
        const CT d = pw_sum<CT>(prog, elem);
        sb[e] = f2bits(d);
    }
    for (int i = lane; i < V; i += 64) t[i] = 0;
    __syncthreads();
    for (int e = lane; e < 2 * V; e += 64) {
        const int s = e / V, v = e - s * V;
        const uint64_t mine = sb[e];
        int r = 0;
        for (int u = 0; u < V; ++u) {
            const uint64_t o = sb[s * V + u];
            r += (o < mine) || (o == mine && u < v);
        }
        CT d;
        if constexpr (sizeof(CT) == 4) d = __uint_as_float((uint32_t)mine);
        else d = __longlong_as_double((long long)mine);
        sd[s * V + r] = d;
        so[s * V + r] = (uint16_t)v;
        order[((int64_t)q * 2 + s) * V + r] = (uint16_t)v;
        sorted[((int64_t)q * 2 + s) * V + r] = d;
    }
    __syncthreads();
    const CT* d0 = sd;
// ... 524 lines not shown
                count_table_group(grp_cnt, split ? V + (int)o1[r] : (int)o0[r], q);
            }
        }
        PLAN_DBG(11, wall_clock64() - dbg_k0);
    }
}

template <typename CT>
__global__ __launch_bounds__(64) void k_multiseq_list(const CT* __restrict__ sorted, const uint16_t* __restrict__ order, int V,
                                                      int max_cells, int32_t* __restrict__ cells, double* __restrict__ dists) {
    extern __shared__ __attribute__((aligned(16))) char smem[];
    int* t = reinterpret_cast<int*>(smem);
    const int q = blockIdx.x, lane = threadIdx.x;
    const CT* d0 = sorted + ((int64_t)q * 2 + 0) * V;
    const CT* d1 = sorted + ((int64_t)q * 2 + 1) * V;
    const uint16_t* o0 = order + ((int64_t)q * 2 + 0) * V;
    const uint16_t* o1 = order + ((int64_t)q * 2 + 1) * V;
    for (int i = lane; i < V; i += 64) t[i] = 0;
    __syncthreads();
    int rows = 1;
    for (int n = 0; n < max_cells; ++n) {
        const uint32_t bij = walk_step<CT, false>(d0, d1, t, rows, V, lane);
        if (bij == WALK_NONE) break;
        const int bi = (int)(bij >> 16), bj = (int)(bij & 0xffff);
        if (lane == 0) {
            cells[((int64_t)q * max_cells + n) * 2 + 0] = o0[bi];
            cells[((int64_t)q * max_cells + n) * 2 + 1] = o1[bj];
            dists[(int64_t)q * max_cells + n] = (double)(CT)(d0[bi] + d1[bj]);
        }
        walk_advance(t, rows, V, lane, bi, bj);
    }
}

static const int GROUP_TILE = 1024;
__global__ __launch_bounds__(256) void k_group_bases(int* __restrict__ grp_cnt, int* __restrict__ grp_base, int n_groups,
                                                     unsigned long long* __restrict__ agg , uint32_t tag) {
    __shared__ int s_w[8];
    const int tid = threadIdx.x, lane = tid & 63, wv = tid >> 6, t = blockIdx.x;
    const int g = t * GROUP_TILE + tid * 4;
    int c[4];
#pragma unroll
    for (int i = 0; i < 4; ++i) c[i] = g + i < n_groups ? grp_cnt[g + i] : 0;
    const int tot = c[0] + c[1] + c[2] + c[3];
    int x = tot;
#pragma unroll
    for (int d = 1; d < 64; d <<= 1) {
        const int y = __shfl_up(x, d);
        if (lane >= d) x += y;
    }
    if (lane == 63) s_w[wv] = x;
    __syncthreads();
    if (tid == 0)
        __hip_atomic_store(&agg[t], ((unsigned long long)tag << 32) | (unsigned long long)(uint32_t)(s_w[0] + s_w[1] + s_w[2] + s_w[3]),
                           __ATOMIC_RELEASE, __HIP_MEMORY_SCOPE_AGENT);
    int pre = 0;
    for (int p = tid; p < t; p += 256) {
        unsigned long long v;
        do { v = __hip_atomic_load(&agg[p], __ATOMIC_ACQUIRE, __HIP_MEMORY_SCOPE_AGENT); } while ((uint32_t)(v >> 32) != tag);
        pre += (int)(uint32_t)v;
    }
#pragma unroll
    for (int o = 32; o > 0; o >>= 1) pre += __shfl_xor(pre, o);
    if (lane == 0) s_w[4 + wv] = pre;
    __syncthreads();
    int r = s_w[4] + s_w[5] + s_w[6] + s_w[7] + x - tot;
    for (int w = 0; w < wv; ++w) r += s_w[w];
#pragma unroll
    for (int i = 0; i < 4; ++i) {
        if (g + i < n_groups) {
            grp_base[g + i] = r;
            grp_cnt[g + i] = 0;
            grp_cnt[n_groups + g + i] = 0;
        }
        r += c[i];
    }
}

__global__ __launch_bounds__(1024) void k_plan_scan(const PlanOut* __restrict__ plan, int nq, int64_t* __restrict__ item_off,
                                                    int64_t* __restrict__ tab_off, int64_t* __restrict__ totals,
                                                    unsigned long long* __restrict__ qbound ,
                                                    volatile int64_t* __restrict__ host_totals , int64_t seq,
                                                    int* __restrict__ grp_cnt ,
                                                    int* __restrict__ grp_base, int n_groups,
                                                    unsigned long long* __restrict__ hint_zero ) {
    if (hint_zero && threadIdx.x == 0) { hint_zero[0] = 0ull; hint_zero[1] = 0ull; }
    constexpr int R = 8;
    __shared__ int s_wi[R][16], s_wt[R][16];
    __shared__ int64_t s_cand[16];
    __shared__ int64_t s_base_i[R][16], s_base_t[R][16];
    const int tid = threadIdx.x, lane = tid & 63, wv = tid >> 6;
    if (wv == 15 && n_groups > 0) {
        int run = 0;
        for (int g0 = 0; g0 < n_groups; g0 += 1024) {
            int c[16];
#pragma unroll
            for (int i = 0; i < 16; ++i) {
                const int g = g0 + lane * 16 + i;
                c[i] = g < n_groups ? grp_cnt[g] : 0;
            }
            int tot = 0;
#pragma unroll
            for (int i = 0; i < 16; ++i) tot += c[i];
            int x = tot;
#pragma unroll
            for (int d = 1; d < 64; d <<= 1) {
                const int y = __shfl_up(x, d);
                if (lane >= d) x += y;
            }
            int r = run + x - tot;
#pragma unroll
            for (int i = 0; i < 16; ++i) {
                const int g = g0 + lane * 16 + i;
                if (g < n_groups) {
                    grp_base[g] = r;
                    grp_cnt[g] = 0;
                    grp_cnt[n_groups + g] = 0;
                }
                r += c[i];
            }
            run += __shfl(x, 63);
        }
    }
    int ni[R], nt[R], xi[R], xt[R];
    int64_t lc = 0;
#pragma unroll
    for (int r = 0; r < R; ++r) {
        const int q = r * 1024 + tid;
        const bool on = q < nq;
        const PlanOut pl = plan[on ? q : 0];
        ni[r] = on ? pl.n_items : 0;
        nt[r] = on ? pl.ntab0 + pl.ntab1 : 0;
        lc += on ? pl.ncand : 0;
        xi[r] = ni[r]; xt[r] = nt[r];
    }
    for (int q = R * 1024 + tid; q < nq; q += 1024) lc += plan[q].ncand;
#pragma unroll
    for (int d = 1; d < 64; d <<= 1) {
#pragma unroll
        for (int r = 0; r < R; ++r) {
            const int yi = __shfl_up(xi[r], d), yt = __shfl_up(xt[r], d);
            if (lane >= d) { xi[r] += yi; xt[r] += yt; }
        }
    }
#pragma unroll
    for (int d = 32; d > 0; d >>= 1) lc += __shfl_xor(lc, d);
    if (lane == 63) {
#pragma unroll
        for (int r = 0; r < R; ++r) { s_wi[r][wv] = xi[r]; s_wt[r][wv] = xt[r]; }
    }
    if (lane == 0) s_cand[wv] = lc;
    __syncthreads();
    if (wv == 0) {
        const int e0 = 2 * lane, e1 = 2 * lane + 1;
        const int a_i = (&s_wi[0][0])[e0], b_i = (&s_wi[0][0])[e1], a_t = (&s_wt[0][0])[e0], b_t = (&s_wt[0][0])[e1];
        int64_t xi2 = (int64_t)a_i + b_i, xt2 = (int64_t)a_t + b_t;
        const int64_t own_i = xi2, own_t = xt2;
#pragma unroll
        for (int d = 1; d < 64; d <<= 1) {
            const int64_t yi = __shfl_up(xi2, d), yt = __shfl_up(xt2, d);
            if (lane >= d) { xi2 += yi; xt2 += yt; }
        }
        (&s_base_i[0][0])[e0] = xi2 - own_i; (&s_base_i[0][0])[e1] = xi2 - own_i + a_i;
        (&s_base_t[0][0])[e0] = xt2 - own_t; (&s_base_t[0][0])[e1] = xt2 - own_t + a_t;
        int64_t ri = __shfl(xi2, 63), rt = __shfl(xt2, 63);
        int64_t rc = lane < 16 ? s_cand[lane] : 0;
#pragma unroll
        for (int d = 32; d > 0; d >>= 1) rc += __shfl_xor(rc, d);
        if (lane == 0) {
            for (int q = R * 1024; q < nq; ++q) {
                item_off[q] = ri; tab_off[q] = rt;
                qbound[q] = 0x7ff0000000000000ull;
                ri += plan[q].n_items; rt += plan[q].ntab0 + plan[q].ntab1;
            }
            totals[0] = ri; totals[1] = rt; totals[2] = rc;
            host_totals[0] = ri; host_totals[1] = rt; host_totals[2] = rc;
            __threadfence_system();
            host_totals[3] = seq;
            __threadfence_system();
            item_off[nq] = ri; tab_off[nq] = rt;
        }
    }
    __syncthreads();
#pragma unroll
    for (int r = 0; r < R; ++r) {
        const int q = r * 1024 + tid;
        if (q < nq) {
            item_off[q] = s_base_i[r][wv] + xi[r] - ni[r];
            tab_off[q] = s_base_t[r][wv] + xt[r] - nt[r];
            qbound[q] = 0x7ff0000000000000ull;
        }
    }
}

__global__ void k_slots_init(int* __restrict__ qctr16, int* __restrict__ cell_cnt, int ncells, int* __restrict__ slots,
                             int64_t n_slot_entries) {
    const int64_t i = (int64_t)blockIdx.x * blockDim.x + threadIdx.x;
    if (i < 64) qctr16[i] = 0;
    if (i < ncells) cell_cnt[i] = 0;
    if (i < n_slot_entries) slots[i] = -1;
}

static __device__ __forceinline__ int q8_begin(int x, int ncells) { return (int)(((int64_t)x * ncells + 7) / 8); }
static __device__ __forceinline__ int slot_key(const WorkItem& it, int ncells, int CH, int seg_max) {
    const int x = (int)(((int64_t)it.cell * 8) / ncells);
    const int b = q8_begin(x, ncells), sz = q8_begin(x + 1, ncells) - b;
    int ch = CH > 1 ? it.pos0 / seg_max : 0;
    ch = ch < CH ? ch : CH - 1;
    return (2 * b + (it.rank > 0 ? sz : 0) + (it.cell - b)) * CH + ch;
}

__global__ void k_item_hist(const WorkItem* __restrict__ items, int64_t n, int* __restrict__ cell_cnt, int ncells, int CH, int seg_max,
                            const int64_t* __restrict__ d_totals = nullptr ) {
    if (d_totals) n = d_totals[0];
    const int64_t i = (int64_t)blockIdx.x * blockDim.x + threadIdx.x;
    if (i < n) atomicAdd(&cell_cnt[slot_key(items[i], ncells, CH, seg_max)], 1);
}

__global__ __launch_bounds__(1024) void k_cell_scan(int* __restrict__ cell_cnt, int* __restrict__ slot_off, int nkeys, int G,
                                                    int* __restrict__ n_slots, int* __restrict__ qstart , int CH) {
    __shared__ int s_w[16];
    __shared__ int s_tot;
    const int tid = threadIdx.x, lane = tid & 63, wv = tid >> 6;
    int run = 0;
    for (int c0 = 0; c0 < nkeys; c0 += 1024) {
        const int c = c0 + tid;
        const int x = c < nkeys ? (cell_cnt[c] + G - 1) / G : 0;
        int inc = x;
#pragma unroll
        for (int d = 1; d < 64; d <<= 1) {
            const int y = __shfl_up(inc, d);
            if (lane >= d) inc += y;
        }
        __syncthreads();
        if (lane == 63) s_w[wv] = inc;
        __syncthreads();
        int base = run, tot = 0;
#pragma unroll
        for (int w = 0; w < 16; ++w) {
            const int v = s_w[w];
            if (w < wv) base += v;
            tot += v;
        }
        if (c < nkeys) {
            slot_off[c] = base + inc - x;
            cell_cnt[c] = 0;
        }
        run += tot;
    }
    if (tid == 0) { *n_slots = run; s_tot = run; }
    __threadfence();
    __syncthreads();
    if (tid < 8) {
        const int k0 = 2 * q8_begin(tid, nkeys / (2 * CH)) * CH;
        qstart[tid] = k0 < nkeys ? __hip_atomic_load(&slot_off[k0], __ATOMIC_RELAXED, __HIP_MEMORY_SCOPE_AGENT) : s_tot;
    }
    if (tid == 8) qstart[8] = s_tot;
}

__global__ void k_item_scatter(const WorkItem* __restrict__ items, int64_t n, const int* __restrict__ slot_off,
                               int* __restrict__ cursor, int G, int* __restrict__ slots, int ncells, int CH, int seg_max,
                               const int64_t* __restrict__ d_totals = nullptr ) {
    if (d_totals) n = d_totals[0];
    const int64_t i = (int64_t)blockIdx.x * blockDim.x + threadIdx.x;
    if (i >= n) return;
    const int c = slot_key(items[i], ncells, CH, seg_max);
    const int r = atomicAdd(&cursor[c], 1);
    slots[(slot_off[c] + r / G) * G + (r % G)] = (int)i;
}

__global__ void k_identity_slots(int64_t n, int G, int* __restrict__ slots, int* __restrict__ n_slots, int* __restrict__ qstart) {
    const int64_t i = (int64_t)blockIdx.x * blockDim.x + threadIdx.x;
// ... 142 lines not shown
template <typename CT>
static void launch_rank(cis_index* ix, int nq, bool reg_sorts, int* grp_cnt, hipStream_t st) {
    const int V = ix->m->V;
    int Vp2 = 64;
    while (Vp2 < V) Vp2 <<= 1;
    const CT* cd = ix->w_cd.as<CT>();
    uint16_t* order = ix->w_order.as<uint16_t>();
    CT* sorted = ix->w_sorted.as<CT>();
    if constexpr (sizeof(CT) == 4) {
        const bool sort_lds = getenv("CIS_RANK_SORT_LDS") != nullptr;
        if (reg_sorts && V > 256 && !sort_lds && (Vp2 == 1024 || Vp2 == 2048 || Vp2 == 4096)) {
            if (Vp2 == 1024) hipLaunchKernelGGL(k_rank_sort_reg<4>, dim3(nq, 2), dim3(256), 0, st, cd, nq, V, order, sorted, grp_cnt);
            else if (Vp2 == 2048) hipLaunchKernelGGL(k_rank_sort_reg<8>, dim3(nq, 2), dim3(256), 0, st, cd, nq, V, order, sorted, grp_cnt);
            else hipLaunchKernelGGL(k_rank_sort_reg<16>, dim3(nq, 2), dim3(256), 0, st, cd, nq, V, order, sorted, grp_cnt);
            return;
        }
    }
    if (V > 256 && Vp2 <= 4096)
        hipLaunchKernelGGL(k_rank_sort<CT>, dim3(nq, 2), dim3(256), (size_t)Vp2 * 16, st, cd, nq, V, Vp2, order, sorted, grp_cnt);
    else
        hipLaunchKernelGGL(k_rank<CT>, dim3(nq, 2), dim3(V <= 64 ? 64 : 256), (size_t)V * 8, st, cd, nq, V, order, sorted, grp_cnt);
}

#ifdef CIS_PLAN_DBG
static void dump_plan_dbg(int nq) {
    unsigned long long h[12];
    (void)hipDeviceSynchronize();
    (void)hipMemcpyFromSymbol(h, HIP_SYMBOL(g_plan_dbg), sizeof(h));
    fprintf(stderr, "[cis] k_plan_par: %d queries, probes %.1f / query, bands %.2f / query, bisection %.1f us / query, after rows %.1f, after cells %.1f, after sort %.1f, after cut %.1f us / query (cumulative), cells per band %.0f (100 MHz clock)\n",
            nq, (double)h[0] / nq, (double)h[1] / nq, (double)h[2] / nq / 100.0, (double)h[5] / nq / 100.0, (double)h[6] / nq / 100.0, (double)h[7] / nq / 100.0, (double)h[3] / nq / 100.0, h[1] ? (double)h[4] / (double)h[1] : 0.0);
    fprintf(stderr, "[cis] k_plan_par since kernel start: staged %.1f, bands done %.1f, visited pass %.1f, end %.1f us / query\n", (double)h[8] / nq / 100.0, (double)h[9] / nq / 100.0, (double)h[10] / nq / 100.0, (double)h[11] / nq / 100.0);
    memset(h, 0, sizeof(h));
    (void)hipMemcpyToSymbol(HIP_SYMBOL(g_plan_dbg), h, sizeof(h));
}
#endif

int dump_plan_fallbacks(const Batch& b) {
    std::vector<int> fbh(b.nq);
    CIS_CHECK_HIP(hipMemcpyAsync(fbh.data(), b.plan_fb, (size_t)b.nq * sizeof(int), hipMemcpyDeviceToHost, b.st));
    CIS_CHECK_HIP(hipStreamSynchronize(b.st));
    int nfb = 0;
    for (int i = 0; i < b.nq; ++i) nfb += fbh[i] != 0;
    fprintf(stderr, "[cis] k_plan_par: %d of %d queries fall back to the frontier walk (quota %lld)\n", nfb, b.nq, (long long)b.quota);
    return CIS_OK;
}

static void host_timing(const Batch& b, std::chrono::steady_clock::time_point t0) {
    static const bool ht = getenv("CIS_HOST_TIMING") != nullptr;
    if (!ht) return;
    static std::atomic<long long> n_{0}, wait_ns{0}, front_ns{0};
    const auto t1 = std::chrono::steady_clock::now();
    wait_ns += std::chrono::duration_cast<std::chrono::nanoseconds>(t1 - t0).count();
    front_ns += std::chrono::duration_cast<std::chrono::nanoseconds>(t0 - b.t_entry).count();
    if (++n_ % 400 == 0)
        fprintf(stderr, "[cis] host timing over %lld batches: front-end enqueue %.1f us, wait for the plan totals %.1f us per batch\n", (long long)n_,
                front_ns / 1e3 / n_, wait_ns / 1e3 / n_);
}

template <typename CT>
int front_count(Batch& b, const Route& r) {
    cis_index* ix = b.ix;
    cis_model* m = ix->m;
    hipStream_t st = b.st;
    const int V = m->V, nq = b.nq;
    uint16_t* order = ix->w_order.as<uint16_t>();
    CT* sorted = ix->w_sorted.as<CT>();
    if (r.fused_front) {
        const size_t flds = (size_t)V * (32 + 4 + 4);
        hipLaunchKernelGGL(k_front_small<CT>, dim3(nq), dim3(64), flds, st, (const CT*)b.f.xc, m->D, m->h, coarse_centroids(m, CT()), m->prog_h,
                           ix->gcount_ptr(), ix->loff_ptr(), nq, V, b.quota, r.seg_max, order, sorted, b.plan, b.f.grp_cnt);
        return CIS_OK;
    }
    CIS_TRY(cis_launch_sqdist_both(m, b.f.xc, b.f.ct, nq, ix->w_cd.p, st));
    launch_rank<CT>(ix, nq, true, b.f.grp_cnt, st);
    if (r.par_plan)
        hipLaunchKernelGGL((k_plan_par<CT, false>), dim3(nq), dim3(256), (size_t)2 * (V < PLAN_SP ? V : PLAN_SP) * sizeof(CT), st, sorted, order,
                           ix->gcount_ptr(), ix->loff_ptr(), nq, V, b.quota, r.seg_max, b.plan, nullptr, nullptr, nullptr,
                           nullptr, b.f.grp_cnt, nullptr, nullptr, nullptr, b.vis_list, b.plan_fb, b.vis_cap, b.plan_hint, b.hint_slot);
#ifdef CIS_PLAN_DBG
    if constexpr (sizeof(CT) == 4)
        if (r.par_plan) dump_plan_dbg(nq);
#endif
    hipLaunchKernelGGL((k_plan<CT, false>), dim3(nq), dim3(64), (size_t)V * sizeof(int), st, sorted, order, ix->gcount_ptr(), ix->loff_ptr(), nq, V,
                       b.quota, r.seg_max, b.plan, nullptr, nullptr, nullptr, nullptr, b.f.grp_cnt, nullptr, nullptr, nullptr, b.plan_fb);
    return CIS_OK;
}
template int front_count<float>(Batch&, const Route&);
template int front_count<double>(Batch&, const Route&);

template <typename CT>
void emit_plan(Batch& b, const Route& r) {
    cis_index* ix = b.ix;
    cis_model* m = ix->m;
    hipStream_t st = b.st;
    const int V = m->V, nq = b.nq;
    const uint16_t* order = ix->w_order.as<uint16_t>();
    const CT* sorted = ix->w_sorted.as<CT>();
    if (r.par_plan)
        hipLaunchKernelGGL((k_plan_par<CT, true>), dim3(nq), dim3(256), 0, st, sorted, order, ix->gcount_ptr(), ix->loff_ptr(), nq, V, b.quota,
                           r.seg_max, b.plan, b.item_off, b.tab_off, b.items, b.tabs, nullptr, b.grp_base, b.grp_cur, b.tab_order, b.vis_list,
                           b.plan_fb, b.vis_cap, nullptr, 0);
    hipLaunchKernelGGL((k_plan<CT, true>), dim3(nq), dim3(64), (size_t)V * sizeof(int), st, sorted, order, ix->gcount_ptr(), ix->loff_ptr(), nq, V,
                       b.quota, r.seg_max, b.plan, b.item_off, b.tab_off, b.items, b.tabs, nullptr, b.grp_base, b.grp_cur, b.tab_order, b.plan_fb);
}
template void emit_plan<float>(Batch&, const Route&);
template void emit_plan<double>(Batch&, const Route&);

int plan_totals(Batch& b, const Route& r) {
    cis_index* ix = b.ix;
    cis_model* m = ix->m;
    hipStream_t st = b.st;
    const int V = m->V, nq = b.nq, L = b.L;
    if (!ix->h_totals) {
        CIS_CHECK_HIP(hipHostMalloc((void**)&ix->h_totals, 12 * sizeof(int64_t), hipHostMallocMapped | hipHostMallocCoherent));
        CIS_CHECK_HIP(hipHostGetDevicePointer((void**)&ix->d_h_totals, ix->h_totals, 0));
        ix->h_totals[3] = 0;
        ix->h_totals[4] = 0;
        for (int i = 6; i < 12; ++i) ix->h_totals[i] = 0;
    }
    const int64_t seq = ++ix->plan_seq;
    const int n_groups = 2 * V * GRP_SUB;
    const bool groups_apart = n_groups > 8192;
    int* grp_cnt = b.f.grp_cnt;
    if (groups_apart)
        hipLaunchKernelGGL(k_group_bases, dim3((n_groups + GROUP_TILE - 1) / GROUP_TILE), dim3(256), 0, st, grp_cnt, b.grp_base, n_groups,
                           reinterpret_cast<unsigned long long*>(grp_cnt + GRP_WORDS(V)), (uint32_t)(seq & 0x7fffffff) | 0x80000000u);
    hipLaunchKernelGGL(k_plan_scan, dim3(1), dim3(1024), 0, st, b.plan, nq, b.item_off, b.tab_off, b.totals, b.qbound, ix->d_h_totals, seq, grp_cnt, b.grp_base,
                       groups_apart ? 0 : n_groups, b.plan_hint ? b.plan_hint + (b.hint_slot ^ 1) * 2 : nullptr);
    volatile int64_t* h_tot = ix->h_totals;
    b.d_tot = nullptr;
    b.n_items = b.n_tabs = b.n_cand_all = 0;
    {
        static const bool no_bounds = getenv("CIS_NO_BOUNDS") != nullptr;
        const int64_t q_eff = b.quota < 0 ? 0 : b.quota;
        const int64_t per_q = (q_eff < ix->n_total ? q_eff : ix->n_total) + ix->max_cell;
        const int64_t items_q = ix->nonempty_cells + per_q / r.seg_max + 2;
        const bool small_all = !no_bounds && !r.stream_hint && nq <= 64 && L <= MAX_LDS_LIMIT && r.split_tables && r.big && items_q <= 4096 &&
                               (double)nq * (double)per_q < 64.0e6;
        static const bool no_stream_bounds = getenv("CIS_STREAM_WAIT") != nullptr;
        const bool sure_stream = !no_bounds && !no_stream_bounds && r.stream_hint && r.split_tables && items_q <= 65536 &&
                                 (double)nq * (double)items_q < 4.0e6 &&
                                 (ix->force_stream || (q_eff < ix->n_total ? q_eff : ix->n_total) >= r.stream_min) && ix->n_total > 0 && nq <= 64;
        if (small_all || sure_stream) {
            b.d_tot = b.totals;
            b.n_items = (int64_t)nq * items_q;
            b.n_tabs = (int64_t)nq * 2 * V;
            b.n_cand_all = (int64_t)nq * per_q;
            ix->stats_pending_seq = seq;
        }
    }
    if (!b.d_tot) {
        static const bool no_poll = getenv("CIS_NO_POLL") != nullptr;
        const auto t0 = std::chrono::steady_clock::now();
        bool got = false;
        while (!no_poll) {
            if (__atomic_load_n(&ix->h_totals[3], __ATOMIC_ACQUIRE) == seq) { got = true; break; }
            if (std::chrono::steady_clock::now() - t0 > std::chrono::milliseconds(2)) break;
        }
        if (!got) {
            CIS_CHECK_HIP(hipStreamSynchronize(st));
            CIS_REQUIRE(__atomic_load_n(&ix->h_totals[3], __ATOMIC_ACQUIRE) == seq, "plan totals did not arrive");
        }
        host_timing(b, t0);
        b.n_items = h_tot[0]; b.n_tabs = h_tot[1]; b.n_cand_all = h_tot[2];
        ix->stats_pending_seq = 0;
    }
    CIS_REQUIRE(b.n_items < ((int64_t)1 << 31) && b.n_tabs < ((int64_t)1 << 31), "query batch too large");
    return CIS_OK;
}

int build_slots(const Batch& b, SlotMode mode, int G, int64_t CH , int seg_max, Slots* s) {
    cis_index* ix = b.ix;
    hipStream_t st = b.st;
    const int64_t n_items = b.n_items;
    const int64_t nkeys = 2 * ix->ncells * CH;
    const int64_t max_slots = mode == SLOTS_IDENTITY ? n_items : (n_items + nkeys) / G + nkeys + 2;
    CIS_TRY(ix->w_order2.reserve((size_t)(64 + 2 * nkeys + 2 * max_slots * G) * sizeof(int)));
    int* qctr = ix->w_order2.as<int>();
    int* n_slots = qctr + 8;
    int* qstart = qctr + 16;
    int* cell_cnt = qctr + 64;
    int* slot_off = cell_cnt + nkeys;
    int* slots = slot_off + nkeys;
    s->qctr = qctr;
    s->n_slots = n_slots;
    s->fhdr = qctr + 32;
    s->slots = mode == SLOTS_NONE ? nullptr : slots;
    s->fslots = slots + max_slots * G;
    s->max_slots = max_slots;
    if (mode == SLOTS_SORTED) {
        const int64_t ninit = max_slots * G > nkeys ? max_slots * G : nkeys;
        hipLaunchKernelGGL(k_slots_init, dim3((unsigned)ceil_div(ninit < 16 ? 16 : ninit, 256)), dim3(256), 0, st, qctr, cell_cnt, (int)nkeys, slots, max_slots * G);
        hipLaunchKernelGGL(k_item_hist, dim3((unsigned)ceil_div(n_items, 256)), dim3(256), 0, st, b.items, n_items, cell_cnt, (int)ix->ncells, (int)CH, seg_max, b.d_tot);
        hipLaunchKernelGGL(k_cell_scan, dim3(1), dim3(1024), 0, st, cell_cnt, slot_off, (int)nkeys, G, n_slots, qstart, (int)CH);
        hipLaunchKernelGGL(k_item_scatter, dim3((unsigned)ceil_div(n_items, 256)), dim3(256), 0, st, b.items, n_items, slot_off, cell_cnt, G, slots, (int)ix->ncells, (int)CH, seg_max, b.d_tot);
    } else if (mode == SLOTS_IDENTITY) {
        CIS_CHECK_HIP(hipMemsetAsync(qctr, 0, 64 * sizeof(int), st));
        hipLaunchKernelGGL(k_identity_slots, dim3((unsigned)ceil_div(n_items < 9 ? 9 : n_items, 256)), dim3(256), 0, st, n_items, G, slots, n_slots, qstart);
    }
    return CIS_OK;
}

extern "C" int cis_multisequence(const void* X, int x_dtype, const void* C0, const void* C1, int c_dtype, int64_t n, int V,
                                 int h, int max_cells, int32_t* cells, double* dists, int* dist_dtype) {
    CIS_REQUIRE((x_dtype == CIS_F32 || x_dtype == CIS_F64) && (c_dtype == CIS_F32 || c_dtype == CIS_F64), "dtype must be 4 or 8");
    CIS_REQUIRE(n >= 0 && V >= 1 && V <= 65535 && h >= 1 && max_cells >= 1 && (n == 0 || (X && C0 && C1 && cells && dists)),
                "bad arguments");
    if ((int64_t)max_cells > (int64_t)V * V) max_cells = V * V;
    const int ct = (x_dtype == CIS_F32 && c_dtype == CIS_F32) ? CIS_F32 : CIS_F64;
    if (dist_dtype) *dist_dtype = ct;
    if (n == 0) return CIS_OK;
    CIS_TRY(cis_lazy_init());
    const size_t csz = (size_t)ct;
    DevBuf bx, bc, bd, bs, bo, bcell, bdist;
    int rc = CIS_OK;
    auto done = [&](int r) { bx.release(); bc.release(); bd.release(); bs.release(); bo.release(); bcell.release(); bdist.release(); return r; };
    auto up = [&](const void* src, int dt, size_t cnt, DevBuf* b, size_t off_elems) -> int {
        if (dt == ct) { CIS_CHECK_HIP(hipMemcpy((char*)b->p + off_elems * csz, src, cnt * csz, hipMemcpyHostToDevice)); return CIS_OK; }
        std::vector<double> tmp(cnt);
        for (size_t i = 0; i < cnt; ++i) tmp[i] = (double)((const float*)src)[i];
        CIS_CHECK_HIP(hipMemcpy((char*)b->p + off_elems * csz, tmp.data(), cnt * sizeof(double), hipMemcpyHostToDevice));
        return CIS_OK;
    };
    if ((rc = bx.reserve((size_t)n * 2 * h * csz)) != CIS_OK) return done(rc);
    if ((rc = bc.reserve((size_t)2 * V * h * csz)) != CIS_OK) return done(rc);
    if ((rc = up(X, x_dtype, (size_t)n * 2 * h, &bx, 0)) != CIS_OK) return done(rc);
    if ((rc = up(C0, c_dtype, (size_t)V * h, &bc, 0)) != CIS_OK) return done(rc);
    if ((rc = up(C1, c_dtype, (size_t)V * h, &bc, (size_t)V * h)) != CIS_OK) return done(rc);
    if ((rc = bd.reserve((size_t)2 * n * V * csz)) != CIS_OK) return done(rc);
    if ((rc = bs.reserve((size_t)2 * n * V * csz)) != CIS_OK) return done(rc);
    if ((rc = bo.reserve((size_t)2 * n * V * sizeof(uint16_t))) != CIS_OK) return done(rc);
    if ((rc = bcell.reserve((size_t)n * max_cells * 2 * sizeof(int32_t))) != CIS_OK) return done(rc);
    if ((rc = bdist.reserve((size_t)n * max_cells * sizeof(double))) != CIS_OK) return done(rc);
    DevBuf bgrp;
    if ((rc = bgrp.reserve((size_t)4 * V * GRP_SUB * sizeof(int))) != CIS_OK) return done(rc);
    for (int s = 0; s < 2; ++s)
        if ((rc = cis_launch_sqdist_generic(bx.p, ct, 2 * h, s * h, (char*)bc.p + (size_t)s * V * h * csz, n, V, h,
                                            (char*)bd.p + (size_t)s * n * V * csz, nullptr)) != CIS_OK) return done(rc);
    if (ct == CIS_F32) {
        hipLaunchKernelGGL(k_rank<float>, dim3((unsigned)n, 2), dim3(V <= 64 ? 64 : 256), (size_t)V * 8, nullptr, bd.as<float>(), (int)n, V,
                           bo.as<uint16_t>(), bs.as<float>(), bgrp.as<int>());
        hipLaunchKernelGGL(k_multiseq_list<float>, dim3((unsigned)n), dim3(64), (size_t)V * sizeof(int), nullptr, bs.as<float>(),
                           bo.as<uint16_t>(), V, max_cells, bcell.as<int32_t>(), bdist.as<double>());
    } else {
        hipLaunchKernelGGL(k_rank<double>, dim3((unsigned)n, 2), dim3(V <= 64 ? 64 : 256), (size_t)V * 8, nullptr, bd.as<double>(), (int)n, V,
                           bo.as<uint16_t>(), bs.as<double>(), bgrp.as<int>());
        hipLaunchKernelGGL(k_multiseq_list<double>, dim3((unsigned)n), dim3(64), (size_t)V * sizeof(int), nullptr, bs.as<double>(),
                           bo.as<uint16_t>(), V, max_cells, bcell.as<int32_t>(), bdist.as<double>());
    }
// ... 67 lines not shown
```

### columbiaimagesearch_amd/csrc/lopq_search.hip

```cpp
#include "lopq_batch.h"

template <typename CT>
__global__ __launch_bounds__(256) void k_tables(const CT* __restrict__ X , const CT* __restrict__ Cs,
                                                const double* __restrict__ Rt, const double* __restrict__ mus,
                                                const double* __restrict__ subs, const TabDesc* __restrict__ tabs,
                                                int V, int h, int w, int nf, int K, int D,
                                                double* __restrict__ T , PwProg prog_w,
                                                double* __restrict__ px_out ,
                                                const int* __restrict__ tab_order, int first) {
    extern __shared__ __attribute__((aligned(16))) char smem[];
    double* v = reinterpret_cast<double*>(smem);
    double* px = v + h;
    const int tab = tab_order ? tab_order[first + blockIdx.x] : first + (int)blockIdx.x;
    const TabDesc td = tabs[tab];
    const int s = td.split, c = td.cluster;
    const CT* x = X + (int64_t)td.q * D + s * h;
    const CT* Cc = Cs + ((int64_t)s * V + c) * h;
    const double* mu = mus + ((int64_t)s * V + c) * h;
    const double* R = Rt + ((int64_t)s * V + c) * h * h;
    for (int k = threadIdx.x; k < h; k += blockDim.x) {
        const CT res = x[k] - Cc[k];
        v[k] = (double)res - mu[k];
    }
    __syncthreads();
// ... 1582 lines not shown
}

__global__ void k_selftest(int* __restrict__ errors) {
    const uint32_t v = (uint32_t)threadIdx.x * 7919u + blockIdx.x * 104729u + 17u;
    int bad = selftest_xor<1>(v) + selftest_xor<2>(v) + selftest_xor<4>(v) + selftest_xor<8>(v) + selftest_xor<16>(v) +
              selftest_xor<32>(v);
    bad += selftest_sort<4>(blockIdx.x * 977u + 1u) + selftest_sort<8>(blockIdx.x * 31u + 5u);
    if (bad) atomicAdd(errors, bad);
}

#ifdef CIS_SCAN_COUNTERS
extern "C" int cis_debug_counters(unsigned long long* out, int reset) {
    CIS_CHECK_HIP(hipMemcpyFromSymbol(out, HIP_SYMBOL(g_scan_ctr), 16 * sizeof(unsigned long long)));
    if (reset) {
        unsigned long long z[16] = {0};
        CIS_CHECK_HIP(hipMemcpyToSymbol(HIP_SYMBOL(g_scan_ctr), z, sizeof(z)));
    }
    return CIS_OK;
}
#endif

extern "C" int cis_selftest(int* n_errors) {
    CIS_REQUIRE(n_errors != nullptr, "NULL argument");
    CIS_TRY(cis_lazy_init());
    int* d = nullptr;
    CIS_CHECK_HIP(hipMalloc((void**)&d, sizeof(int)));
    CIS_CHECK_HIP(hipMemset(d, 0, sizeof(int)));
    hipLaunchKernelGGL(k_selftest, dim3(64), dim3(64), 0, nullptr, d);
    CIS_CHECK_HIP(hipMemcpy(n_errors, d, sizeof(int), hipMemcpyDeviceToHost));
    (void)hipFree(d);
    return CIS_OK;
}

extern "C" int cis_index_set_scan_mode(cis_index* ix, int mode) {
    CIS_REQUIRE(ix != nullptr && mode >= 0 && mode <= 7, "bad scan mode");
    ix->force_stream = (mode == 6);
    ix->force_scan5 = (mode == 7);
    ix->force_exact_scan = (mode == 1);
    ix->force_prefilter_scan = (mode >= 2 && mode <= 5) || mode == 7;
    ix->force_scan2 = (mode == 2);
    ix->force_scan3 = (mode == 3 || mode == 4 || mode == 5 || mode == 7);
    ix->force_two_pass = mode == 3 ? 0 : (mode == 4 ? 1 : ((mode == 5 || mode == 7) ? 2 : -1));
    return CIS_OK;
}

extern "C" int cis_index_read_profile(cis_index* ix, double ms[5], int64_t* launches) {
    CIS_REQUIRE(ix != nullptr && ms != nullptr, "NULL argument");
    for (auto& r : ix->prof) {
        hipEvent_t last = r.ev[4] ? r.ev[4] : r.ev[3];
        if (last) CIS_CHECK_HIP(hipEventSynchronize(last));
        for (int i = 0; i < 4; ++i) {
            if (!r.ev[i] || !r.ev[i + 1]) continue;
            float t = 0.f;
            CIS_CHECK_HIP(hipEventElapsedTime(&t, r.ev[i], r.ev[i + 1]));
            ix->prof_ms[i] += t;
        }
        if (r.has_scan && r.ev[5] && r.ev[3]) {
            float t = 0.f;
            CIS_CHECK_HIP(hipEventElapsedTime(&t, r.ev[5], r.ev[3]));
            ix->prof_ms[4] += t;
            ix->prof_launches += 1;
        }
        for (int i = 0; i < 6; ++i)
            if (r.ev[i]) (void)hipEventDestroy(r.ev[i]);
    }
    ix->prof.clear();
    for (int i = 0; i < 5; ++i) { ms[i] = ix->prof_ms[i]; ix->prof_ms[i] = 0; }
    if (launches) *launches = ix->prof_launches;
    ix->prof_launches = 0;
    return CIS_OK;
}

extern "C" int cis_index_last_scan_kernel(cis_index* ix) { return ix ? ix->last_scan_kernel : 0; }

extern "C" int cis_index_stream_counters(cis_index* ix, int64_t counters[2]) {
    CIS_REQUIRE(ix != nullptr && counters != nullptr, "NULL argument");
    counters[0] = ix->stream_batches;
    counters[1] = ix->stream_fallbacks;
    return CIS_OK;
}

extern "C" int cis_index_last_stats(cis_index* ix, int64_t stats[4]) {
    CIS_REQUIRE(ix != nullptr && stats != nullptr, "NULL argument");
    if (ix->stats_pending_seq) {
        if (__atomic_load_n(&ix->h_totals[3], __ATOMIC_ACQUIRE) != ix->stats_pending_seq) CIS_CHECK_HIP(hipDeviceSynchronize());
        ix->stats[0] += ix->h_totals[2];
        ix->stats[1] += ix->h_totals[0];
        ix->stats[2] += ix->h_totals[1];
        ix->stats_pending_seq = 0;
    }
    for (int i = 0; i < 4; ++i) stats[i] = ix->stats[i];
    return CIS_OK;
}

template <int CAP, int U>
static void launch_scan_m(int M, const ScanArgs& a, int S, const int* flag) {
    const size_t lds = (size_t)CAP * 16 + (size_t)M * a.K * sizeof(double) + 16;
    dispatch_int<0, 4, 8, 16>((M == 4 || M == 8 || M == 16) ? M : 0, [&](auto m) {
        hipLaunchKernelGGL((k_adc_scan<decltype(m)::value, CAP, U>), dim3((unsigned)a.n_items), dim3(256), lds, a.st, a.items, a.T, a.codes, a.ids, M, a.K, a.L, S, flag,
                           reinterpret_cast<cis_hit*>(a.hits), a.hitn);
    });
}

static void launch_scan_exact(int M, const ScanArgs& a, int S, const int* flag) {
    if (a.L <= 512) launch_scan_m<1024, 2>(M, a, S, flag);
    else if (a.L <= 1024) launch_scan_m<2048, 4>(M, a, S, flag);
    else launch_scan_m<4096, 4>(M, a, S, flag);
}

static const int SCAN2_MAX_LIMIT = 952;
static bool scan2_supported(int M, int K, int L) {
    return (M == 4 || M == 8 || M == 16) && K <= 256 && K % 4 == 0 && L >= 1 && L <= SCAN2_MAX_LIMIT;
}

static Scan2Geom scan2_geom(int M, int K, int L, int nq) {
    Scan2Geom g;
    const int NR = (L <= 184) ? 4 : (L <= 440 ? 8 : 16);
    g.G = (nq >= 64 && NR < 16) ? 2 : 1;
    g.NW = 4;
    g.U = (g.G == 2) ? 4 : 2;
    if (const char* e = getenv("CIS_SCAN_GEOM")) {
        int a = 0, b = 0, c = 0;
        if (NR < 16 && sscanf(e, "%d,%d,%d", &a, &b, &c) == 3 && ((a == 1 && b == 4) || (a == 2 && b == 4) || (a == 2 && b == 8 && c == 2) || (a == 2 && (b == 1 || b == 2) && c == 4) || (a == 4 && b == 4 && c == 4 && NR == 4)) && (c == 2 || c == 4)) {
            g.G = a; g.NW = b; g.U = c;
        }
    }
    g.S = g.NW * (NR * 64 - 8);
    g.lds = (size_t)K * M * g.G * 4 + (size_t)g.G * g.NW * (NR * 64 - 8 + 64) * 8 + g.G * sizeof(ScanShared) + 16;
    return g;
}

template <int M, int NR, int G, int NW, int U>
static void launch_scan2_t(const Scan2Geom& g, const ScanArgs& a) {
    const float eps = 2.0f * (float)M * 5.9604645e-8f;
    const float margin = 1.0f + 3.0f * eps;
    const int per_cu = (int)(163840 / g.lds) < (32 / NW) ? (int)(163840 / g.lds) : (32 / NW);
    hipLaunchKernelGGL((k_adc_scan2<M, NR, U, G, NW>), dim3(persistent_grid(a, G, per_cu)), dim3(NW * 64), g.lds, a.st, a.items, a.slots, a.n_slots, a.T, a.T32, a.codes, a.ids,
                       a.K, a.L, g.S, margin, a.qctr, a.hits, a.hitn, a.qbound);
}

template <int M, int NR>
static void launch_scan2_mr(const Scan2Geom& g, const ScanArgs& a) {
#define CIS_SCAN2_CASE(GG, WW, UU) if (g.G == GG && g.NW == WW && g.U == UU) return launch_scan2_t<M, NR, GG, WW, UU>(g, a);
    CIS_SCAN2_CASE(1, 4, 2)
    if constexpr (NR != 16) {
        CIS_SCAN2_CASE(1, 4, 4)
        CIS_SCAN2_CASE(2, 4, 4)
        CIS_SCAN2_CASE(2, 4, 2)
        CIS_SCAN2_CASE(2, 8, 2)
        CIS_SCAN2_CASE(2, 1, 4)
        CIS_SCAN2_CASE(2, 2, 4)
    }
    if constexpr (NR == 4) { CIS_SCAN2_CASE(4, 4, 4) }
#undef CIS_SCAN2_CASE
}

static void launch_scan2(int M, const Scan2Geom& g, const ScanArgs& a) {
    dispatch_int<4, 8, 16>(M, [&](auto m) { dispatch_nr<16>(a.L, [&](auto nr) { launch_scan2_mr<decltype(m)::value, decltype(nr)::value>(g, a); }); });
}

int cis_seg_sort_u64(void* temp, size_t* temp_bytes, const uint64_t* keys_in, uint64_t* keys_out, const uint64_t* vals_in,
                     uint64_t* vals_out, int64_t n, int nseg, const int64_t* seg_begin, const int64_t* seg_end, hipStream_t st);

__global__ void k_item_lens(const WorkItem* __restrict__ items, int64_t n, int64_t* __restrict__ lens) {
    const int64_t i = (int64_t)blockIdx.x * blockDim.x + threadIdx.x;
    if (i < n) lens[i] = items[i].len;
}

__global__ void k_seg_begin(const int64_t* __restrict__ cand_start, const int64_t* __restrict__ item_off, int nq, int64_t n_items,
                            int64_t n_cand, int64_t* __restrict__ seg, unsigned long long* __restrict__ qmin,
                            unsigned long long* __restrict__ qmax) {
    const int q = blockIdx.x * blockDim.x + threadIdx.x;
    if (q > nq) return;
    const int64_t it = item_off[q];
// ... 1200 lines not shown
    r->fast = scan2_supported(M, K, L) && !ix->force_exact_scan;
    r->tiny_cells = index_has_tiny_cells(ix);
    r->geom = scan2_geom(M, K, L, nq);
    static const int env_scan = getenv("CIS_FORCE_SCAN") ? atoi(getenv("CIS_FORCE_SCAN")) : 0;
    const bool short_cells = ix->nonempty_cells > 0 && ix->n_total / ix->nonempty_cells < 8192 && M <= 8;
    static const int env_long = getenv("CIS_SCAN_LONG") ? atoi(getenv("CIS_SCAN_LONG")) : 1;
    static const int env_m16 = getenv("CIS_S4_M16") ? atoi(getenv("CIS_S4_M16")) : 1;
    if (M == 16 && env_m16 && ix->h_totals) {
        const int32_t* fb = reinterpret_cast<const int32_t*>(&ix->h_totals[4]);
        const int32_t n_s = __atomic_load_n(&fb[0], __ATOMIC_RELAXED), n_f = __atomic_load_n(&fb[1], __ATOMIC_RELAXED);
        if (ix->m16_holdoff > 0) --ix->m16_holdoff;
        else if (n_s > 0 && (int64_t)n_f * 8 > n_s) { ix->m16_holdoff = 64; ++ix->m16_backoffs; ix->h_totals[4] = 0; }
    }
    const bool long_cells = env_long != 0 && !short_cells && (M <= 8 || (env_m16 && ix->m16_holdoff == 0)) && L <= 128 && ix->ncells <= 65536;
    r->use3 = !ix->force_exact_scan && scan3_supported(M, K, L) && !r->big &&
              (ix->force_scan3 || (nq >= 256 && !ix->force_scan2 && (env_scan == 3 || (env_scan == 0 && (short_cells || long_cells)))));
    int seg_max = r->use3 ? (nq >= 64 ? 65536 : 4096) : (nq >= 1024 ? (1 << 20) : (nq >= 64 ? 16384 : 4096));
    static const int64_t stream_min = getenv("CIS_STREAM_MIN") ? atoll(getenv("CIS_STREAM_MIN")) : 262144;
    static const int stream_nq = getenv("CIS_STREAM_NQ") ? atoi(getenv("CIS_STREAM_NQ")) : 16;
    r->stream_min = stream_min;
    const bool stream_auto = !ix->stream_off && !ix->force_exact_scan && !ix->force_prefilter_scan && !ix->force_scan2 && !ix->force_scan3 &&
                             nq <= stream_nq && L <= 440 && ix->world == 1 &&
                             ((quota < ix->n_total ? (quota < 0 ? 0 : quota) : ix->n_total) + ix->max_cell) >= stream_min;
    r->stream_hint = (ix->force_stream || stream_auto) && !ix->stream_off && stream_supported(M, K, L) && (K % 4 == 0) &&
                     ix->ncells <= 65536 && !r->tiny_cells;
    if (r->stream_hint) {
        const int64_t cap_len = (((int64_t)1 << 31) - 65536) / M;
        int64_t want = ix->max_cell > 65536 ? ix->max_cell : 65536;
        want = want < cap_len ? want : cap_len;
        if (const char* e = getenv("CIS_STREAM_CHUNK")) want = atoi(e) > 0 ? atoi(e) : want;
        seg_max = (int)(ceil_div(want, (int64_t)1024) * 1024);
        const int64_t need = ceil_div(ix->max_cell > 0 ? ix->max_cell : 1, (int64_t)16);
        if (need > seg_max) seg_max = (int)ceil_div(need, (int64_t)1024) * 1024;
        if (ix->force_stream && getenv("CIS_STREAM_SEG")) seg_max = atoi(getenv("CIS_STREAM_SEG")) > 0 ? atoi(getenv("CIS_STREAM_SEG")) : seg_max;
    }
    if (const char* e = getenv("CIS_SEG_MAX")) seg_max = atoi(e) > 0 ? atoi(e) : seg_max;
    r->seg_max = seg_max;
    const bool no_par_plan = getenv("CIS_NO_PAR_PLAN") != nullptr;
    const bool stream_par = r->stream_hint && V >= 8 && ix->n_total > 0 &&
                            (double)(quota < 0 ? 0 : quota) * (double)ix->nonempty_cells >= 32.0 * (double)ix->n_total;
    r->par_plan = ((V >= 128 || stream_par) && V <= PLAN_PAR_STAGE) && !no_par_plan;
    static const bool no_fused_front = getenv("CIS_NO_FUSED_FRONT") != nullptr;
    r->fused_front = V <= 64 && !r->par_plan && !no_fused_front;
}

template <typename CT>
static void emit_and_tables(Batch& b, const Route& r) {
    cis_model* m = b.ix->m;
    const int V = m->V, h = m->h;
    const size_t tab_lds = (size_t)(2 * h + (h < 256 ? 256 : 0)) * sizeof(double);
    emit_plan<CT>(b, r);
    if (b.n_tabs > 0)
        launch_tables<CT>(b.n_tabs, tab_lds, b.st, (const CT*)b.f.xc, coarse_centroids(m, CT()), m->d_Rt, m->d_mus, m->d_subs, b.tabs, b.tab_order, V, h,
                          m->w, m->nf, m->K, m->D, b.T, m->prog_w, b.px_buf, b.d_tot, r.direct ? b.T32 : nullptr);
}

static int route_decide(Batch& b, Route* r) {
    cis_index* ix = b.ix;
    cis_model* m = ix->m;
    const int K = m->K, M = m->M, h = m->h, nf = m->nf, nq = b.nq, L = b.L;
    r->direct = !b.d_tot && r->big && r->tiny_cells && h <= 256 && direct_jp(M, K, m->w) > 0 &&
                !getenv("CIS_TABLES_UNGROUPED") && !getenv("CIS_NO_DIRECT");
    r->stream = r->stream_hint && b.n_items > 0 && (r->w_pow2 || r->fast) &&
                (ix->force_stream || b.d_tot != nullptr || b.n_cand_all / (nq > 0 ? nq : 1) >= r->stream_min);
    if (!r->stream) {
        const int64_t S_ = r->fast ? r->geom.S : L;
        double need = (double)b.n_items * S_ * (r->fast ? sizeof(uint64_t) : sizeof(cis_hit)) + (double)b.n_tabs * nf * K * sizeof(double);
        if (r->big) {
            const SelectPlan sp_ = select_plan(L, nq, b.n_cand_all);
            need = (sp_.select ? 8.0 * (double)b.n_cand_all + (sp_.sort_lds ? 16.0 : 32.0) * (double)nq * (double)sp_.stride : 32.0 * (double)b.n_cand_all) +
                   (r->direct ? (double)b.n_tabs * h * sizeof(double) : (double)b.n_tabs * nf * K * sizeof(double));
        }
        const double budget = (getenv("CIS_WORKSPACE_GB") ? atof(getenv("CIS_WORKSPACE_GB")) : 24.0) * 1.0e9;
        if (need > budget && nq > 1) {
            ix->retry_fraction = 0.9 * budget / need;
            return CIS_RETRY_SMALLER;
        }
    }
    if (!b.d_tot) {
        ix->stats[0] += b.n_cand_all;
        ix->stats[1] += b.n_items;
        ix->stats[2] += b.n_tabs;
    }
    r->geom3 = scan3_geom(M, K, L, b.n_items > 0 ? b.n_cand_all / b.n_items : 0, ix->force_two_pass);
    r->S = r->fast ? (r->use3 ? r->geom3.S : r->geom.S) : L;
    r->use5 = false;
    if (!r->stream && !r->big && r->fast && b.n_items > 0) {
        static const int env_s5 = getenv("CIS_SCAN5") ? atoi(getenv("CIS_SCAN5")) : 0;
        r->use5 = r->use3 && r->geom3.two_pass == 2 && scan5_supported(M, K, L) && (ix->force_scan5 || (env_s5 != 0 && !ix->force_scan3 && L <= 128));
    }
    static const bool no_t32 = getenv("CIS_NO_T32") != nullptr && atoi(getenv("CIS_NO_T32")) != 0;
    r->drop_t32 = no_t32 && !r->direct && r->split_tables;
    return CIS_OK;
}

static int reserve_batch(Batch& b, const Route& r) {
    cis_index* ix = b.ix;
    cis_model* m = ix->m;
    const int K = m->K, h = m->h, nf = m->nf;
    const int64_t n_items = b.n_items, n_tabs = b.n_tabs;
    CIS_TRY(ix->w_items.reserve((size_t)(n_items + 1) * sizeof(WorkItem)));
    CIS_TRY(ix->w_tabs.reserve((size_t)(n_tabs + 1) * sizeof(TabDesc)));
    CIS_TRY(ix->w_T.reserve(r.direct ? 256 : (size_t)(n_tabs + 1) * nf * K * sizeof(double)));
    if (!r.big && !r.stream) CIS_TRY(ix->w_hits.reserve((size_t)(n_items + 1) * r.S * (r.fast ? sizeof(uint64_t) : sizeof(cis_hit))));
    CIS_TRY(ix->w_hitn.reserve((size_t)(n_items + 1) * 2 * sizeof(int)));
    if (r.use3) CIS_TRY(ix->w_slack.reserve((size_t)(n_items + 1) * 2 * sizeof(float)));
    b.items = ix->w_items.as<WorkItem>();
    b.tabs = ix->w_tabs.as<TabDesc>();
    CIS_TRY(ix->w_tord.reserve((size_t)(n_tabs + 1) * sizeof(int)));
    b.tab_order = ix->w_tord.as<int>();
    b.T = ix->w_T.as<double>();
    if (!r.drop_t32) CIS_TRY(ix->w_T32.reserve(r.direct ? (size_t)(n_tabs + 1) * h * sizeof(float) : (size_t)(n_tabs + 1) * nf * K * sizeof(float)));
    b.T32 = r.drop_t32 ? nullptr : ix->w_T32.as<float>();
    b.px_buf = nullptr;
    if (r.split_tables) {
        CIS_TRY(ix->w_px.reserve((size_t)(n_tabs + 1) * h * sizeof(double)));
        b.px_buf = ix->w_px.as<double>();
    }
    return CIS_OK;
}

static void finish_tables(const Batch& b, const Route& r) {
    cis_model* m = b.ix->m;
    hipStream_t st = b.st;
    const int K = m->K, h = m->h, nf = m->nf;
    const int64_t n_tabs = b.n_tabs;
    double *T = b.T, *px_buf = b.px_buf;
    float* T32 = b.T32;
    TabDesc* tabs = b.tabs;
    const int64_t* d_tot = b.d_tot;
    if (r.direct) {
    } else if (r.split_tables && n_tabs > 0) {
        const bool few = n_tabs <= 1024;
        dim3 g((unsigned)ceil_div(n_tabs, few ? 8 : 64), (unsigned)nf, 2);
#define CIS_TFP(WW)                                                                                                                                      \
        if (few) hipLaunchKernelGGL((k_tables_from_px<WW, 8>), g, dim3(256), 0, st, px_buf, tabs, (int)n_tabs, m->d_subs, h, nf, K, T, T32, d_tot);      \
        else hipLaunchKernelGGL((k_tables_from_px<WW, 64>), g, dim3(256), 0, st, px_buf, tabs, (int)n_tabs, m->d_subs, h, nf, K, T, T32, d_tot)
        switch (m->w) {
            case 4: CIS_TFP(4); break;
            case 8: CIS_TFP(8); break;
            case 16: CIS_TFP(16); break;
            default: CIS_TFP(32); break;
        }
#undef CIS_TFP
    } else if (r.fast && n_tabs > 0) {
        const int64_t ne = n_tabs * nf * K;
        hipLaunchKernelGGL(k_tables_f32, dim3((unsigned)ceil_div(ne, 256)), dim3(256), 0, st, T, ne, nf, K, T32, tabs);
    }
}

static int search_batch(cis_index* ix, const void* dQ, int q_dtype, int nq, int64_t quota, int L, const SearchOut& out, hipStream_t st);

static int run_stream(Batch& b, const Route& r) {
    cis_index* ix = b.ix;
    hipStream_t st = b.st;
    const int K = ix->m->K, M = ix->m->M, nq = b.nq, L = b.L;
    const int64_t n_items = b.n_items, n_cand_all = b.n_cand_all;
    const SearchOut& out = b.out;
    CIS_TRY(mark(b, 2));
    const uint8_t* codes = ix->codes_ptr();
    const int64_t* ids = ix->ids_ptr();
    const bool shared_cells = b.quota >= ix->n_total / 2;
    const int G = (nq >= 3 && shared_cells && stream_max_group() >= 4) ? 4 : (nq >= 2 ? 2 : 1);
    const int cap = STREAM_CAP, B = STREAM_B;
    const SelectPlan sp = select_plan(L, nq, (int64_t)nq * cap);
    CIS_REQUIRE(sp.sort_lds, "streaming route: limit above the LDS-ranked range");
    int64_t CH = ceil_div(ix->max_cell > 0 ? ix->max_cell : 1, (int64_t)r.seg_max);
// ... 227 lines not shown
}

static int run_fast_scan(Batch& b, const Route& r) {
    cis_index* ix = b.ix;
    hipStream_t st = b.st;
    const int M = ix->m->M;
    const bool use3 = r.use3;
    const Scan3Geom& geom3 = r.geom3;
    const bool sort_items = ix->ncells <= 65536;
    const bool use5 = r.use5;
    const int G = use5 ? 8 : (use3 ? geom3.G : r.geom.G);
    int64_t CH = use3 ? ceil_div(ix->max_cell > 0 ? ix->max_cell : 1, (int64_t)r.seg_max) : 1;
    CH = CH < 1 ? 1 : (CH > 16 ? 16 : CH);
    Slots sl;
    CIS_TRY(build_slots(b, sort_items ? SLOTS_SORTED : SLOTS_IDENTITY, G, CH, r.seg_max, &sl));
    CIS_TRY(mark(b, 5));
    ix->last_scan_kernel = use5 ? 6 : (use3 ? (geom3.two_pass == 2 ? 4 : 3) : 2);
    const ScanArgs a = scan_args(b, sl);
    if (use5) {
        CIS_TRY(ix->w_s5.reserve(scan5_workspace_bytes(b.nq)));
        launch_scan5(M, geom3, a, ix->w_s5.p);
    } else if (use3) {
        Scan3Geom g3 = geom3;
        const float sat16 = getenv("CIS_S4_SAT") ? (float)atof(getenv("CIS_S4_SAT")) : 0.75f;
        if (M == 16 && g3.two_pass == 2) g3.sat = sat16;
        launch_scan3(M, g3, a);
        if (g3.sat > 0.f && ix->h_totals)
            CIS_CHECK_HIP(hipMemcpyAsync(&ix->h_totals[4], sl.qctr + 9, 2 * sizeof(int), hipMemcpyDeviceToHost, st));
    } else
        launch_scan2(M, r.geom, a);
    return CIS_OK;
}

template <int CAP, int MT, int NEMAX>
static void merge_survivors(const Batch& b, const Route& r) {
    cis_index* ix = b.ix;
    hipStream_t st = b.st;
    const int nq = b.nq, L = b.L, S = r.S, M = ix->m->M, K = ix->m->K;
    const SearchOut& out = b.out;
    const uint64_t* surv = ix->w_hits.as<uint64_t>();
    const int* hitn = ix->w_hitn.as<int>();
    const uint8_t* codes = ix->codes_ptr();
    const int64_t* ids = ix->ids_ptr();
    const float* slack = r.use3 ? ix->w_slack.as<float>() : (const float*)nullptr;
    hipLaunchKernelGGL((k_merge_survivors<CAP, MT, NEMAX>), dim3((unsigned)ceil_div(nq, 4)), dim3(256), (size_t)4 * CAP * 16, st,
                       surv, hitn, b.item_off, b.items, b.T, codes, ids, nq, M, K, L, S, out.hits, out.ids, out.dists,
                       out.n_found, out.cells, out.pos, b.plan, out.visited, slack);
}

template <int CAP>
static void merge_survivors_m(const Batch& b, const Route& r, bool many) {
    dispatch_int<4, 8, 16>(b.ix->m->M, [&](auto m) {
        dispatch_int<4, 8>(many ? 8 : 4, [&](auto ne) { merge_survivors<CAP, decltype(m)::value, decltype(ne)::value>(b, r); });
    });
}

template <int CAPM>
static void merge_items(const Batch& b, int S) {
    const SearchOut& out = b.out;
    hipLaunchKernelGGL(k_merge_items<CAPM>, dim3(b.nq), dim3(256), (size_t)CAPM * 24 + 16, b.st, b.ix->w_hits.as<cis_hit>(), b.ix->w_hitn.as<int>(), b.item_off, b.L, S,
                       out.hits, out.ids, out.dists, out.n_found, out.cells, out.pos);
}

static int run_scan_and_merge(Batch& b, const Route& r) {
    cis_index* ix = b.ix;
    hipStream_t st = b.st;
    const int M = ix->m->M, nq = b.nq, L = b.L, S = r.S;
    const int64_t n_items = b.n_items;
    const SearchOut& out = b.out;
    CIS_TRY(mark(b, 2));
    if (n_items > 0) {
        b.pr.has_scan = true;
        if (r.fast) {
            CIS_TRY(run_fast_scan(b, r));
        } else {
            CIS_TRY(mark(b, 5));
            ix->last_scan_kernel = 1;
            launch_scan_exact(M, scan_args(b, Slots{}), S, nullptr);
        }
        ix->stats[3] += 1;
    }
    CIS_TRY(mark(b, 3));
    if (r.fast) {
        const bool many = n_items > nq + nq / 4;
        if (L <= 128) merge_survivors_m<256>(b, r, many);
        else if (L <= 256) merge_survivors_m<512>(b, r, many);
        else if (L <= 440) merge_survivors_m<1024>(b, r, many);
        else merge_survivors_m<2048>(b, r, many);
    } else if (L <= 512) merge_items<1024>(b, S);
    else if (L <= 1024) merge_items<2048>(b, S);
    else merge_items<4096>(b, S);
    if (out.visited && !r.fast)
        hipLaunchKernelGGL(k_copy_visited, dim3((unsigned)ceil_div(nq, 256)), dim3(256), 0, st, b.plan, nq, out.visited);
    CIS_CHECK_HIP(hipGetLastError());
    CIS_TRY(mark(b, 4));
    if (ix->profiling) ix->prof.push_back(b.pr);
    return CIS_OK;
}

static int search_batch(cis_index* ix, const void* dQ, int q_dtype, int nq, int64_t quota, int L, const SearchOut& out,
                        hipStream_t st) {
    const int V = ix->m->V;
    Batch b{};
    b.ix = ix; b.dQ = dQ; b.q_dtype = q_dtype; b.nq = nq; b.quota = quota; b.L = L; b.out = out; b.st = st;
    b.t_entry = std::chrono::steady_clock::now();
    ix->last_scan_kernel = 0;
    b.pr.has_scan = false;
    for (int i = 0; i < 6; ++i) b.pr.ev[i] = nullptr;
    CIS_TRY(mark(b, 0));
    CIS_TRY(front_prepare(ix, dQ, q_dtype, nq, st, &b.f));
    CIS_TRY(ix->w_plan.reserve((size_t)nq * sizeof(PlanOut)));
    CIS_TRY(ix->w_off.reserve((size_t)(2 * (nq + 1) + 4 + nq) * sizeof(int64_t)));
    b.item_off = ix->w_off.as<int64_t>();
    b.tab_off = b.item_off + (nq + 1);
    b.totals = b.tab_off + (nq + 1);
    b.qbound = reinterpret_cast<unsigned long long*>(b.totals + 4);
    b.plan = ix->w_plan.as<PlanOut>();
    b.grp_cur = b.f.grp_cnt + 2 * V * GRP_SUB;
    b.grp_base = b.f.grp_cnt + 4 * V * GRP_SUB;
    Route r{};
    route_hints(ix, nq, quota, L, &r);
    b.plan_hint = (r.par_plan && !getenv("CIS_NO_PLAN_HINT")) ? ix->plan_hint_ptr() : nullptr;
    b.hint_slot = (int)((ix->plan_seq + 1) & 1);
    int64_t vis_cap64 = ((int64_t)1 << 31) / ((int64_t)(nq > 0 ? nq : 1) * 16);
    if (vis_cap64 < 4096) vis_cap64 = 4096;
    if (vis_cap64 > (1 << 20)) vis_cap64 = 1 << 20;
    if (vis_cap64 > (int64_t)V * V) vis_cap64 = (int64_t)V * V;
    b.vis_cap = (int)vis_cap64;
    if (r.par_plan) {
        CIS_TRY(ix->w_planfb.reserve((size_t)2 * nq * sizeof(int)));
        CIS_TRY(ix->w_vis.reserve((size_t)nq * b.vis_cap * 2 * sizeof(uint64_t)));
        b.plan_fb = ix->w_planfb.as<int>();
        b.vis_list = ix->w_vis.as<uint64_t>();
    }
    const bool f32 = b.f.ct == CIS_F32;
    CIS_TRY(f32 ? front_count<float>(b, r) : front_count<double>(b, r));
    if (r.par_plan && getenv("CIS_DEBUG_PLAN")) CIS_TRY(dump_plan_fallbacks(b));
    CIS_TRY(plan_totals(b, r));
    CIS_TRY(route_decide(b, &r));
    CIS_TRY(mark(b, 1));
    CIS_TRY(reserve_batch(b, r));
    if (f32) emit_and_tables<float>(b, r);
    else emit_and_tables<double>(b, r);
    finish_tables(b, r);
    if (r.stream) return run_stream(b, r);
    if (r.big) return run_all_candidates(b, r);
    return run_scan_and_merge(b, r);
}

static const int QUERY_BATCH = 8192;

static int search_all(cis_index* ix, const void* dQ, int q_dtype, int nq, int64_t quota, int L, const SearchOut& out,
                      hipStream_t st) {
    CIS_REQUIRE(ix != nullptr, "index is NULL");
    CIS_REQUIRE(q_dtype == CIS_F32 || q_dtype == CIS_F64, "q_dtype must be 4 or 8");
    CIS_REQUIRE(nq >= 0, "nq must be >= 0");
    CIS_REQUIRE(!ix->orphaned, "this view's base index was destroyed: close views before their base");
    CIS_TRY(cis_index_ready(ix->base ? ix->base : ix));
    ix->sync_from_base();
    CIS_CHECK_HIP(hipSetDevice(ix->m->device));
    for (int i = 0; i < 4; ++i) ix->stats[i] = 0;
    ix->stats_pending_seq = 0;
    int batch = (ix->batch_hint > 0 && ix->batch_hint_quota == quota) ? ix->batch_hint : QUERY_BATCH;
    for (int a = 0; a < nq;) {
        const int bn = (nq - a < batch) ? (nq - a) : batch;
        const char* q = (const char*)dQ + (size_t)a * ix->m->D_in * q_dtype;
        int rc;
        if (L > 0) {
            rc = search_batch(ix, q, q_dtype, bn, quota, L, out.at(a, L), st);
        } else {
            SearchOut o{};
            o.visited = out.visited ? out.visited + a : nullptr;
            CIS_TRY(ix->w_part.reserve((size_t)bn * sizeof(cis_hit)));
            o.hits = ix->w_part.as<cis_hit>();
            rc = search_batch(ix, q, q_dtype, bn, quota, 1, o, st);
        }
        if (rc == CIS_RETRY_SMALLER) {
            int nb = (int)((double)bn * ix->retry_fraction);
            if (nb > bn / 2 && bn / 2 >= 64) nb = nb / 64 * 64;
            if (nb >= bn) nb = bn / 2;
            batch = nb > 1 ? nb : 1;
            ix->batch_hint = batch;
            ix->batch_hint_quota = quota;
            continue;
        }
        CIS_TRY(rc);
        a += bn;
    }
    return CIS_OK;
}

int cis_search_partial(cis_index* ix, const void* dQ, int q_dtype, int nq, int64_t quota, int L, cis_hit* d_hits, int32_t* d_n_found,
                       int32_t* d_visited, hipStream_t st) {
    SearchOut o{};
    o.hits = d_hits;
    o.n_found = d_n_found;
    o.visited = d_visited;
    return search_all(ix, dQ, q_dtype, nq, quota, L, o, st);
}

extern "C" int cis_index_search_partial_dev(cis_index* ix, const void* dQ, int q_dtype, int nq, int64_t quota,
                                            int limit, cis_hit* d_hits, int32_t* d_visited, void* stream) {
    int L;
    CIS_TRY(effective_limit(quota, limit, &L));
    SearchOut o{};
    o.hits = d_hits;
    o.visited = d_visited;
    return search_all(ix, dQ, q_dtype, nq, quota, L, o, (hipStream_t)stream);
}

extern "C" int cis_index_search_dev(cis_index* ix, const void* dQ, int q_dtype, int nq, int64_t quota, int limit,
                                    int64_t* d_ids, double* d_dists, int32_t* d_n_found, int32_t* d_visited,
                                    int32_t* d_cells, uint32_t* d_pos, void* stream) {
    int L;
    CIS_TRY(effective_limit(quota, limit, &L));
    if (nq == 0) return CIS_OK;
    SearchOut o{};
    o.ids = d_ids; o.dists = d_dists; o.n_found = d_n_found; o.cells = d_cells; o.pos = d_pos; o.visited = d_visited;
    if (L == 0 && d_n_found) CIS_CHECK_HIP(hipMemsetAsync(d_n_found, 0, (size_t)nq * sizeof(int32_t), (hipStream_t)stream));
    return search_all(ix, dQ, q_dtype, nq, quota, L, o, (hipStream_t)stream);
}
```

### columbiaimagesearch_amd/lopq/search.py

```python
import os
from collections import namedtuple
from itertools import count

import numpy as np

from .. import _lib
from . import kvlog
from .model import LOPQCode, LOPQModel, LOPQModelPCA, _code_dtype

_SLOT_BASE = 1 << 62


def _is_int(x):
    return isinstance(x, (int, np.integer)) and not isinstance(x, (bool, np.bool_))


def multisequence_batch(X, centroids, max_cells=64):
    C0, C1 = _lib.as_float_matrix(centroids[0]), _lib.as_float_matrix(centroids[1])
    if C0.dtype != C1.dtype:
        C0, C1 = C0.astype(np.float64), C1.astype(np.float64)
    V, h = C0.shape
    X = _lib.as_float_matrix(X, 2 * h)
    mc = int(min(max_cells, V * V))
    cells = np.empty((X.shape[0], mc, 2), dtype=np.int32)
# ... 327 lines not shown
        return results, int(r["visited"][0])


    def _dev_args(self, q, quota, limit):
        import torch
        if not (q.is_cuda and q.is_contiguous() and q.dim() == 2 and q.shape[1] == self._input_dim):
            raise ValueError("q must be a contiguous [nq, %d] tensor on the GPU" % self._input_dim)
        if q.dtype not in (torch.float32, torch.float64):
            raise ValueError("q must be float32 or float64")
        L = int(quota) if limit is None else int(limit)
        code = _lib.CIS_F32 if q.dtype == torch.float32 else _lib.CIS_F64
        return max(L, 0), code, torch.cuda.current_stream(q.device).cuda_stream

    def search_batch_dev(self, q, quota=10, limit=None, out=None, with_codes=False):
        import torch
        L, code, stream = self._dev_args(q, quota, limit)
        nq = q.shape[0]
        if out is None:
            out = {"ids": torch.empty((nq, L), dtype=torch.int64, device=q.device),
                   "dists": torch.empty((nq, L), dtype=torch.float64, device=q.device),
                   "n_found": torch.empty(nq, dtype=torch.int32, device=q.device),
                   "visited": torch.empty(nq, dtype=torch.int32, device=q.device)}
            if with_codes:
                out["cells"] = torch.empty((nq, L), dtype=torch.int32, device=q.device)
                out["pos"] = torch.empty((nq, L), dtype=torch.int32, device=q.device)
        cells = out["cells"].data_ptr() if "cells" in out else None
        pos = out["pos"].data_ptr() if "pos" in out else None
        _lib.check(_lib.lib().cis_index_search_dev(self._ix, q.data_ptr(), code, nq, int(quota),
                                                   -1 if limit is None else int(limit), out["ids"].data_ptr(),
                                                   out["dists"].data_ptr(), out["n_found"].data_ptr(),
                                                   out["visited"].data_ptr(), cells, pos, stream))
        return out

    def search_rerank_dev(self, q, feats, quota=10, limit=None, rerank_nb=None, max_returned=None, near_dup_th=None):
        r = self.search_batch_dev(q, quota=quota, limit=limit)
        out = feats.rerank_dev(q, r["ids"], r["dists"], rerank_nb=rerank_nb, max_returned=max_returned, near_dup_th=near_dup_th)
        out["visited"] = r["visited"]
        return out

    def search_partial_dev(self, q, quota=10, limit=None):
        import torch
        L, code, stream = self._dev_args(q, quota, limit)
        nq = q.shape[0]
        hits = torch.empty((nq, L, _lib.HIT_DTYPE.itemsize), dtype=torch.uint8, device=q.device)
        visited = torch.empty(nq, dtype=torch.int32, device=q.device)
        _lib.check(_lib.lib().cis_index_search_partial_dev(self._ix, q.data_ptr(), code, nq, int(quota),
                                                           -1 if limit is None else int(limit), hits.data_ptr(),
                                                           visited.data_ptr(), stream))
        return hits, visited

    def query_owners_dev(self, q, quota=10):
        import torch
        _, code, stream = self._dev_args(q, quota, 1)
        nq = q.shape[0]
        mask = torch.empty(nq, dtype=torch.int64, device=q.device)
        visited = torch.empty(nq, dtype=torch.int32, device=q.device)
        _lib.check(_lib.lib().cis_index_query_owners_dev(self._ix, q.data_ptr(), code, nq, int(quota), mask.data_ptr(),
                                                         visited.data_ptr(), stream))
        return mask, visited

    def search_partial_packed_dev(self, q, quota=10, limit=None):
        import torch
        L, code, stream = self._dev_args(q, quota, limit)
        nq = q.shape[0]
        dev = q.device
        out = {"packed": torch.empty((max(nq * L, 1), 4), dtype=torch.int64, device=dev),
               "cnt": torch.empty(nq, dtype=torch.int32, device=dev), "off": torch.empty(nq, dtype=torch.int64, device=dev),
               "total": torch.empty(1, dtype=torch.int64, device=dev), "visited": torch.empty(nq, dtype=torch.int32, device=dev),
               "L": L}
        _lib.check(_lib.lib().cis_index_search_partial_packed_dev(
            self._ix, q.data_ptr(), code, nq, int(quota), -1 if limit is None else int(limit), out["packed"].data_ptr(),
            out["cnt"].data_ptr(), out["off"].data_ptr(), out["total"].data_ptr(), out["visited"].data_ptr(), stream))
        return out

    def insert_counters(self):
        c = np.zeros(2, dtype=np.int64)
        _lib.check(_lib.lib().cis_index_insert_counters(self._ix, _lib.ptr(c)))
        return int(c[0]), int(c[1])

    def stream_counters(self):
        c = np.zeros(2, dtype=np.int64)
        _lib.check(_lib.lib().cis_index_stream_counters(self._ix, _lib.ptr(c)))
        return int(c[0]), int(c[1])

    def last_stats(self):
        st = np.zeros(4, dtype=np.int64)
        _lib.check(_lib.lib().cis_index_last_stats(self._ix, _lib.ptr(st)))
        kind = int(_lib.lib().cis_index_last_scan_kernel(self._ix))
        return {"candidates": int(st[0]), "items": int(st[1]), "tables": int(st[2]), "scan_launches": int(st[3]),
                "scan_kernel": {0: None, 1: "k_adc_scan", 2: "k_adc_scan2", 3: "k_adc_scan3", 4: "k_adc_scan4", 5: "k_adc_stream", 6: "k_adc_scan5"}.get(kind)}


    default_prefilter_only = False
    default_scan_mode = 0

    def set_scan_mode(self, exact_only=False, prefilter_only=None, mode=None):
        if mode is None:
            if prefilter_only is None:
                prefilter_only = type(self).default_prefilter_only
            mode = 1 if exact_only else (2 if prefilter_only else type(self).default_scan_mode)
        _lib.check(_lib.lib().cis_index_set_scan_mode(self._ix, int(mode)))

    def set_profiling(self, enable=True, scan_only=False):
        _lib.check(_lib.lib().cis_index_set_profiling(self._ix, 0 if not enable else (1 if scan_only else 2)))

    def read_profile(self):
        ms = np.zeros(5, dtype=np.float64)
        n = _lib.c_int64(0)
        _lib.check(_lib.lib().cis_index_read_profile(self._ix, _lib.ptr(ms), _lib.ctypes.byref(n)))
        return {"front_ms": float(ms[0]), "tables_ms": float(ms[1]), "scan_ms": float(ms[2]),
                "merge_ms": float(ms[3]), "scan_kernel_ms": float(ms[4]), "scan_launches": int(n.value)}


def merge_hits_dev(parts, with_codes=False):
    import torch
    world, nq, L = int(parts.shape[0]), int(parts.shape[1]), int(parts.shape[2])
    if not (parts.is_cuda and parts.is_contiguous() and parts.dtype == torch.uint8 and parts.shape[3] == 32):
        raise ValueError("parts must be a contiguous uint8 [world, nq, L, 32] tensor on the GPU")
    dev = parts.device
    out = {"ids": torch.empty((nq, L), dtype=torch.int64, device=dev),
           "dists": torch.empty((nq, L), dtype=torch.float64, device=dev),
           "n_found": torch.zeros(nq, dtype=torch.int32, device=dev)}
    if with_codes:
        out["cells"] = torch.empty((nq, L), dtype=torch.int32, device=dev)
        out["pos"] = torch.empty((nq, L), dtype=torch.int32, device=dev)
    _lib.check(_lib.lib().cis_merge_hits_dev(parts.data_ptr(), world, nq, L, out["ids"].data_ptr(),
                                             out["dists"].data_ptr(), out["n_found"].data_ptr(),
                                             out["cells"].data_ptr() if with_codes else None,
                                             out["pos"].data_ptr() if with_codes else None,
                                             torch.cuda.current_stream(dev).cuda_stream))
    return out


def merge_packed_dev(parts, off, cnt, nq, L, with_codes=False):
    import torch
    if parts.dim() == 2:
        world, stride = int(off.shape[0]), 0
        if not (parts.is_cuda and parts.is_contiguous() and parts.dtype == torch.int64 and parts.shape[1] == 4):
            raise ValueError("parts must be a contiguous int64 [n, 4] tensor on the GPU")
    else:
        world, stride = int(parts.shape[0]), int(parts.shape[1])
        if not (parts.is_cuda and parts.is_contiguous() and parts.dtype == torch.int64 and parts.shape[2] == 4):
            raise ValueError("parts must be a contiguous int64 [world, stride, 4] tensor on the GPU")
    if not (off.is_contiguous() and off.dtype == torch.int64 and cnt.is_contiguous() and cnt.dtype == torch.int32
            and tuple(off.shape) == (world, nq) and tuple(cnt.shape) == (world, nq)):
        raise ValueError("off / cnt must be contiguous [world, nq] int64 / int32 tensors")
    dev = parts.device
    out = {"ids": torch.empty((nq, L), dtype=torch.int64, device=dev),
           "dists": torch.empty((nq, L), dtype=torch.float64, device=dev),
           "n_found": torch.zeros(nq, dtype=torch.int32, device=dev)}
    if with_codes:
        out["cells"] = torch.empty((nq, L), dtype=torch.int32, device=dev)
        out["pos"] = torch.empty((nq, L), dtype=torch.int32, device=dev)
    _lib.check(_lib.lib().cis_merge_packed_dev(parts.data_ptr(), world, stride, off.data_ptr(), cnt.data_ptr(), nq, L,
                                               out["ids"].data_ptr(), out["dists"].data_ptr(), out["n_found"].data_ptr(),
                                               out["cells"].data_ptr() if with_codes else None,
                                               out["pos"].data_ptr() if with_codes else None,
                                               torch.cuda.current_stream(dev).cuda_stream))
    return out


class LOPQSearcherLMDB(LOPQSearcherBase):

    def __init__(self, model, lmdb_path=None, id_lambda=int):
        super(LOPQSearcherLMDB, self).__init__()
        self.model = model
# ... 197 lines not shown
```

### include/cis_hip.h

```cpp
#ifndef CIS_HIP_H
#define CIS_HIP_H

#include <stddef.h>
#include <stdint.h>

#ifdef __cplusplus
extern "C" {
#endif

#define CIS_F32 4
#define CIS_F64 8

#define CIS_OK 0
#define CIS_EINVAL -1
#define CIS_EHIP -2
#define CIS_ENOMEM -3
#define CIS_EUNSUPPORTED -4
#define CIS_ENODEVICE -5

typedef struct cis_model cis_model;
typedef struct cis_index cis_index;
typedef struct cis_cnn cis_cnn;

typedef struct cis_hit {
// ... 50 lines not shown
int cis_index_route_pack_dev(cis_index* ix, const int64_t* d_ids, const uint16_t* d_coarse, const uint8_t* d_fine,
                             int64_t n, uint8_t* d_records, int64_t* d_counts, void* stream);
int cis_index_add_records_dev(cis_index* ix, const uint8_t* d_records, int64_t n, int dedup, int64_t* n_added,
                              int64_t* n_invalid, int64_t* d_cell_delta, void* stream);

int cis_index_add(cis_index* ix, const int64_t* ids, const uint16_t* coarse, const uint8_t* fine,
                  int64_t n, int dedup, int64_t* n_added);
int cis_index_add_dev(cis_index* ix, const int64_t* d_ids, const uint16_t* d_coarse, const uint8_t* d_fine, int64_t n,
                      int dedup, int64_t* n_added, int64_t* n_invalid, int64_t* d_cell_delta ,
                      void* stream);
int cis_l2_normalize_dev(void* d_x, int dtype, int64_t n, int d, void* stream);
int64_t cis_index_size(cis_index* ix);
int cis_index_get_cell(cis_index* ix, int c0, int c1, int64_t cap, int64_t* ids, uint8_t* fine, int64_t* n);

int cis_index_search(cis_index* ix, const void* Q, int q_dtype, int nq, int64_t quota, int limit,
                     int64_t* ids, double* dists, int32_t* n_found, int32_t* visited,
                     int32_t* cells, uint32_t* pos);
int cis_index_search_dev(cis_index* ix, const void* dQ, int q_dtype, int nq, int64_t quota, int limit,
                         int64_t* d_ids, double* d_dists, int32_t* d_n_found, int32_t* d_visited,
                         int32_t* d_cells, uint32_t* d_pos, void* stream);
int cis_index_search_async(cis_index* ix, const void* Q, int q_dtype, int nq, int64_t quota, int limit,
                           int64_t* ids, double* dists, int32_t* n_found, int32_t* visited,
                           int32_t* cells, uint32_t* pos);
int cis_index_search_wait(cis_index* ix);
int cis_host_alloc(void** out, size_t bytes);
void cis_host_free(void* p);
int cis_index_get_codes(cis_index* ix, const int32_t* cells, const uint32_t* pos, int64_t n, uint8_t* fine);

int cis_index_search_partial_dev(cis_index* ix, const void* dQ, int q_dtype, int nq, int64_t quota,
                                 int limit, cis_hit* d_hits, int32_t* d_visited, void* stream);
int cis_index_search_partial_packed_dev(cis_index* ix, const void* dQ, int q_dtype, int nq, int64_t quota, int limit,
                                        cis_hit* d_packed, int32_t* d_cnt, int64_t* d_off, int64_t* d_total,
                                        int32_t* d_visited, void* stream);
int cis_index_query_owners_dev(cis_index* ix, const void* d_q, int q_dtype, int nq, int64_t quota, uint64_t* d_mask,
                               int32_t* d_visited, void* stream);
int cis_route_queries_dev(const void* d_q, int nq, int row_bytes, const uint64_t* d_mask, int world, int cap, void* d_out_q,
                          int32_t* d_slot, int32_t* d_cnt, int32_t* d_overflow, void* stream);

int cis_routed_merge_tables_dev(const int32_t* d_slot, int world, int nq, const int64_t* h_base, const cis_hit* d_hits, int limit,
                                int64_t* d_off, int32_t* d_cnt, void* stream);

int cis_merge_hits_dev(const cis_hit* d_parts, int world, int nq, int limit, int64_t* d_ids,
                       double* d_dists, int32_t* d_n_found, int32_t* d_cells ,
                       uint32_t* d_pos , void* stream);

int cis_merge_packed_dev(const cis_hit* d_parts, int world, int64_t stride, const int64_t* d_off ,
                         const int32_t* d_cnt , int nq, int limit, int64_t* d_ids, double* d_dists,
                         int32_t* d_n_found, int32_t* d_cells , uint32_t* d_pos , void* stream);

int cis_exchange_offsets_dev(const int32_t* d_cnt_all, int world, int nq, int64_t stride, int64_t* d_off, int64_t* d_totals,
                             int32_t* d_overflow, void* stream);

int cis_rerank_dev(const void* d_feats, int f_dtype, int64_t n_feats, int D, const void* d_q, int nq,
                   const int64_t* d_rows, int L, double* d_dists, void* stream);

int cis_idmap_build_dev(const int64_t* d_ids, int64_t n, int64_t* d_keys, int64_t* d_rows, int64_t cap, void* stream);
int cis_idmap_lookup_dev(const int64_t* d_keys, const int64_t* d_rows, int64_t cap, int64_t n_feats, const int64_t* d_ids, int64_t m,
                         int64_t* d_out, void* stream);

int cis_rerank_select_dev(const void* d_feats, int f_dtype, int64_t n_feats, int D, const int64_t* d_map_keys,
                          const int64_t* d_map_rows, int64_t map_cap, const void* d_q, int nq, const int64_t* d_ids,
                          const double* d_adc, int L, int nb, int max_returned, int use_th, double near_dup_th,
                          int64_t* d_out_ids, double* d_out_dists, int32_t* d_out_src, int32_t* d_n_kept, void* stream);

int cis_exact_knn_dev(const void* d_data, int data_dtype, int64_t m2, int d, const void* d_q, int q_dtype, int m1, int k,
                      int64_t base, int accumulate, int64_t* d_idx, double* d_dist, void* stream);
int cis_exact_knn(const void* data, int data_dtype, int64_t m2, int d, const void* q, int q_dtype, int m1, int k, int64_t base,
                  int accumulate, int64_t* idx, double* dist);
int cis_exact_knn_set_mode(int mode);
int cis_exact_knn_stats(int64_t stats[3]);

int cis_kmeans(const float* X, int64_t n, int d, int k, int iters, float* centroids, int32_t* assign, double* inertia);

int cis_train_gram(const double* X, int64_t n, int d, const int64_t* group_off, int groups, double* G, double* S);
int cis_train_project(const double* X, int64_t n, int d, const int64_t* group_off, int groups, const double* R,
                      const double* mu, double* Y);

int cis_index_last_stats(cis_index* ix, int64_t stats[4]);
int cis_index_last_scan_kernel(cis_index* ix);

int cis_index_set_profiling(cis_index* ix, int level );
int cis_index_set_scan_mode(cis_index* ix, int mode);
int cis_index_stream_counters(cis_index* ix, int64_t counters[2]);
int cis_index_read_profile(cis_index* ix, double ms[5], int64_t* launches);

#define CIS_CNN_SENTIBANK 1
#define CIS_CNN_DLIB_RESNET 2
int cis_cnn_create(cis_cnn** out, int arch, const float* const* tensors, int n_tensors);
void cis_cnn_destroy(cis_cnn* c);
int cis_cnn_feat_dim(int arch);
int cis_cnn_forward(cis_cnn* c, const float* nchw, int n, float* feats);
int cis_cnn_forward_dev(cis_cnn* c, const float* d_nchw, int n, float* d_feats, void* stream);
int cis_cnn_create_view(cis_cnn** out, cis_cnn* base);

int cis_pyramid_down2_dev(const uint8_t* d_img, int nr, int nc, uint8_t* d_out, int* d_tmp, void* stream);
int cis_extract_chips_dev(const uint8_t* d_img, int nr, int nc, const double* d_maps, int n, int size, float* d_chips, void* stream);

#ifdef __cplusplus
}
#endif
#endif
```

Measured before the change: 23.11 million.

## Run ahead of plan totals using host-computed upper bounds instead of waiting

```diff
diff --git a/columbiaimagesearch_amd/_lib.py b/columbiaimagesearch_amd/_lib.py
--- a/columbiaimagesearch_amd/_lib.py
+++ b/columbiaimagesearch_amd/_lib.py
@@ -113,6 +113,8 @@
     "cis_index_set_profiling": (c_int, [c_void_p, c_int]),
     "cis_index_set_scan_mode": (c_int, [c_void_p, c_int]),
     "cis_index_stream_counters": (c_int, [c_void_p, c_void_p]),
+    "cis_index_set_run_ahead": (c_int, [c_void_p, c_int]),
+    "cis_index_run_ahead_counters": (c_int, [c_void_p, c_void_p]),
     "cis_index_read_profile": (c_int, [c_void_p, c_void_p, POINTER(c_int64)]),
 }
 
diff --git a/columbiaimagesearch_amd/csrc/lopq_batch.h b/columbiaimagesearch_amd/csrc/lopq_batch.h
--- a/columbiaimagesearch_amd/csrc/lopq_batch.h
+++ b/columbiaimagesearch_amd/csrc/lopq_batch.h
@@ -62,6 +62,7 @@
     int hint_slot;
     const int64_t* d_tot;
     int64_t n_items, n_tabs, n_cand_all;
+    int64_t est_items, est_cand;
     WorkItem* items;
     TabDesc* tabs;
     int* tab_order;
@@ -98,6 +99,8 @@
 int front_count(Batch& b, const Route& r);
 int dump_plan_fallbacks(const Batch& b);
 int plan_totals(Batch& b, const Route& r);
+int settle_pending_totals(cis_index* ix);
+int check_run_ahead_error(cis_index* ix);
 template <typename CT>
 void emit_plan(Batch& b, const Route& r);
 int build_slots(const Batch& b, SlotMode mode, int G, int64_t CH , int seg_max, Slots* s);
diff --git a/columbiaimagesearch_amd/csrc/lopq_bounds.h b/columbiaimagesearch_amd/csrc/lopq_bounds.h
--- /dev/null
+++ b/columbiaimagesearch_amd/csrc/lopq_bounds.h
@@ -0,0 +1,58 @@
+#pragma once
+#include <stdint.h>
+
+#if defined(__HIPCC__)
+#define CIS_BOUNDS_FN static __host__ __device__ inline
+#else
+#define CIS_BOUNDS_FN static inline
+#endif
+
+static const int CIS_PREFIX_MAX = 256;
+
+struct CisCellStats {
+    int64_t n_total;
+    int64_t max_cell;
+    int64_t nonempty;
+    int64_t ncells;
+    int n_prefix;
+    const int64_t* prefix;
+};
+
+struct CisBatchBound {
+    int ok;
+    int64_t kvis;
+    int64_t items, tabs, cand;
+};
+
+CIS_BOUNDS_FN int64_t cis_bound_kvis(const CisCellStats& c, int64_t quota) {
+    if (c.nonempty <= 0) return 0;
+    int64_t below = 0;
+    while (below < c.n_prefix && c.prefix[below] < quota) ++below;
+    if (below == c.n_prefix && (int64_t)c.n_prefix < c.nonempty) return -1;
+    const int64_t k = 1 + below;
+    return k < c.nonempty ? k : c.nonempty;
+}
+
+CIS_BOUNDS_FN CisBatchBound cis_batch_bound(const CisCellStats& c, int V, int64_t seg_max, int64_t quota, int64_t nq) {
+    CisBatchBound b;
+    b.ok = 0; b.kvis = 0; b.items = 0; b.tabs = 0; b.cand = 0;
+    if (seg_max <= 0 || nq < 0 || V <= 0) return b;
+    const int64_t kvis = cis_bound_kvis(c, quota);
+    if (kvis < 0) return b;
+    const int64_t q_eff = quota < 0 ? 0 : quota;
+    const int64_t per_q = (q_eff < c.n_total ? q_eff : c.n_total) + c.max_cell;
+    const int64_t empty = c.ncells - c.nonempty;
+    int64_t tabs_q = kvis + empty + 1;
+    if (tabs_q > 2 * (int64_t)V) tabs_q = 2 * (int64_t)V;
+    if (kvis == 0) tabs_q = 0;
+    b.ok = 1;
+    b.kvis = kvis;
+    b.items = nq * (kvis == 0 ? 0 : kvis + per_q / seg_max + 2);
+    b.tabs = nq * tabs_q;
+    b.cand = nq * (kvis == 0 ? 0 : per_q);
+    return b;
+}
+
+CIS_BOUNDS_FN int cis_totals_fit(int64_t items, int64_t tabs, int64_t cand, int64_t cap_items, int64_t cap_tabs, int64_t cap_cand) {
+    return items <= cap_items && tabs <= cap_tabs && cand <= cap_cand;
+}
diff --git a/columbiaimagesearch_amd/csrc/lopq_host.hip b/columbiaimagesearch_amd/csrc/lopq_host.hip
--- a/columbiaimagesearch_amd/csrc/lopq_host.hip
+++ b/columbiaimagesearch_amd/csrc/lopq_host.hip
@@ -119,9 +119,11 @@
         ~Guard() { if (armed) { (void)hipStreamSynchronize(st); ix->h_pending = false; host_abandon(ix); } }
     } guard{ix, st, true};
     CIS_CHECK_HIP(hipStreamWaitEvent(st, ix->h_ev_in, 0));
+    ix->ra_hold = true;
     int rc = cis_index_search_dev(ix, ix->w_q.p, q_dtype, nq, quota, limit, ix->w_oids.as<int64_t>(),
                                   ix->w_odists.as<double>(), ix->w_onf.as<int32_t>(), ix->w_ovis.as<int32_t>(),
                                   ix->w_ocell.as<int32_t>(), ix->w_opos.as<uint32_t>(), st);
+    ix->ra_hold = false;
     if (rc != CIS_OK) return rc;
     CIS_CHECK_HIP(hipEventRecord(ix->h_ev_out, st));
     ix->h_out = {ids, dists, n_found, visited, cells, pos, nq, L};
diff --git a/columbiaimagesearch_amd/csrc/lopq_index.h b/columbiaimagesearch_amd/csrc/lopq_index.h
--- a/columbiaimagesearch_amd/csrc/lopq_index.h
+++ b/columbiaimagesearch_amd/csrc/lopq_index.h
@@ -1,4 +1,5 @@
 #pragma once
+#include "lopq_bounds.h"
 #include "lopq_model.h"
 
 struct CellStore {
@@ -45,6 +46,8 @@
         if (!base) return;
         ncells = base->ncells; rank = base->rank; world = base->world; nb_indexed = base->nb_indexed; n_local = base->n_local;
         n_total = base->n_total; max_cell = base->max_cell; nonempty_cells = base->nonempty_cells;
+        n_prefix = base->n_prefix;
+        for (int i = 0; i < n_prefix; ++i) cell_prefix[i] = base->cell_prefix[i];
     }
     int64_t n_local = 0;
     DevBuf wi_key[2], wi_val[2], wi_hist, wi_sid, wi_acc, wi_apre, wi_tmp, wi_in_ids, wi_in_coarse, wi_in_fine, wi_scan, wi_cnt, wi_cnt2;
@@ -85,6 +88,23 @@
     int64_t plan_seq = 0;
     int64_t stats_pending_seq = 0;
     int64_t n_total = 0, max_cell = 0, nonempty_cells = 0;
+    int64_t cell_prefix[CIS_PREFIX_MAX];
+    int n_prefix = 0;
+    int run_ahead_mode = 0;
+    bool ra_hold = false;
+    struct RunAheadEst { int nq = -1, L = 0; int64_t quota = 0, n_total = -1, items = 0, tabs = 0, cand = 0; };
+    static const int RA_ESTS = 4;
+    RunAheadEst ra_ests[RA_ESTS];
+    int ra_est_next = 0;
+    RunAheadEst* ra_find(int nq, int64_t quota, int L) {
+        for (int i = 0; i < RA_ESTS; ++i)
+            if (ra_ests[i].nq == nq && ra_ests[i].quota == quota && ra_ests[i].L == L && ra_ests[i].n_total == n_total) return &ra_ests[i];
+        return nullptr;
+    }
+    int64_t ra_counters[6] = {0, 0, 0, 0, 0, 0};
+    RunAheadEst* ra_pending_est = nullptr;
+    hipStream_t pending_stream = nullptr;
+    int64_t ra_cap[3] = {0, 0, 0};
     struct ProfRec { hipEvent_t ev[6]; bool has_scan; };
     std::vector<ProfRec> prof;
     double prof_ms[5] = {0, 0, 0, 0, 0};
diff --git a/columbiaimagesearch_amd/csrc/lopq_index.hip b/columbiaimagesearch_amd/csrc/lopq_index.hip
--- a/columbiaimagesearch_amd/csrc/lopq_index.hip
+++ b/columbiaimagesearch_amd/csrc/lopq_index.hip
@@ -137,7 +137,8 @@
 }
 
 enum { INS_ACC_OWN = 0, INS_INVALID = 1, INS_NTOTAL = 2, INS_MAXCELL = 3, INS_NONEMPTY = 4, INS_ERR = 5, INS_ACC_GHOST = 6,
-       INS_REMOTE_PLAIN = 7, INS_OVERFLOW = 8, INS_WORDS = 9 };
+       INS_REMOTE_PLAIN = 7, INS_OVERFLOW = 8, INS_WORDS = 9,
+       INS_PREFIX_N = 9, INS_PREFIX = 10, INS_ALL = INS_PREFIX + CIS_PREFIX_MAX };
 
 __device__ __forceinline__ bool dev_owns(int64_t cell, const int32_t* __restrict__ owner, int rank, int world) {
     if (world <= 1) return true;
@@ -528,6 +529,60 @@
     }
 }
 
+static const int CELL_PREFIX_CELLS = 4096;
+__global__ __launch_bounds__(1024) void k_cell_prefix(const int64_t* __restrict__ gcount, int ncells, int64_t* __restrict__ stats) {
+    __shared__ unsigned long long s_k[CELL_PREFIX_CELLS];
+    int N = 64;
+    while (N < ncells) N <<= 1;
+    for (int i = threadIdx.x; i < N; i += 1024) {
+        const long long g = i < ncells ? gcount[i] : 0;
+        s_k[i] = g > 0 ? (unsigned long long)g : ~0ull;
+    }
+    __syncthreads();
+    for (int k = 2; k <= N; k <<= 1) {
+        for (int j = k >> 1; j > 0; j >>= 1) {
+            for (int t = threadIdx.x; t < N / 2; t += 1024) {
+                const int i = ((t / j) * 2 * j) + (t % j), p = i + j;
+                const unsigned long long a = s_k[i], b = s_k[p];
+                if ((a > b) == ((i & k) == 0)) { s_k[i] = b; s_k[p] = a; }
+            }
+            __syncthreads();
+        }
+    }
+    if (threadIdx.x < 64) {
+        const int lane = threadIdx.x;
+        long long run = 0;
+        int n = 0;
+        for (int b0 = 0; b0 < CIS_PREFIX_MAX && b0 < N; b0 += 64) {
+            const unsigned long long v = s_k[b0 + lane];
+            const bool on = v != ~0ull;
+            long long x = on ? (long long)v : 0;
+            for (int d = 1; d < 64; d <<= 1) {
+                const long long y = __shfl_up(x, d);
+                if (lane >= d) x += y;
+            }
+            if (on) stats[INS_PREFIX + b0 + lane] = run + x;
+            run += __shfl(x, 63);
+            n += __popcll(__ballot(on));
+        }
+        if (lane == 0) stats[INS_PREFIX_N] = n;
+    }
+}
+
+static void launch_cell_prefix(cis_index* ix, hipStream_t st) {
+    if (ix->ncells > CELL_PREFIX_CELLS) return;
+    hipLaunchKernelGGL(k_cell_prefix, dim3(1), dim3(1024), 0, st, (const int64_t*)ix->d_gcount.as<int64_t>(), (int)ix->ncells, ix->d_stats.as<int64_t>());
+}
+
+static void adopt_cell_stats(cis_index* ix) {
+    ix->n_total = ix->h_ins[INS_NTOTAL];
+    ix->max_cell = ix->h_ins[INS_MAXCELL];
+    ix->nonempty_cells = ix->h_ins[INS_NONEMPTY];
+    ix->nb_indexed = ix->n_total;
+    ix->n_prefix = ix->ncells <= CELL_PREFIX_CELLS ? (int)ix->h_ins[INS_PREFIX_N] : 0;
+    for (int i = 0; i < ix->n_prefix; ++i) ix->cell_prefix[i] = ix->h_ins[INS_PREFIX + i];
+}
+
 __global__ void k_cell_delta(const int64_t* __restrict__ gcount, int64_t* __restrict__ delta, int64_t ncells) {
     const int64_t c = (int64_t)blockIdx.x * blockDim.x + threadIdx.x;
     if (c < ncells) delta[c] = gcount[c] - delta[c];
@@ -633,10 +688,10 @@
         CIS_CHECK_HIP(hipMemcpy(ix->d_owner.p, ix->owner.data(), (size_t)ix->ncells * sizeof(int32_t), hipMemcpyHostToDevice));
     }
     if (!ix->h_ins) {
-        CIS_TRY(ix->d_stats.reserve(INS_WORDS * sizeof(int64_t)));
-        CIS_CHECK_HIP(hipMemset(ix->d_stats.p, 0, INS_WORDS * sizeof(int64_t)));
-        CIS_CHECK_HIP(hipHostMalloc((void**)&ix->h_ins, INS_WORDS * sizeof(int64_t), hipHostMallocDefault));
-        for (int i = 0; i < INS_WORDS; ++i) ix->h_ins[i] = 0;
+        CIS_TRY(ix->d_stats.reserve(INS_ALL * sizeof(int64_t)));
+        CIS_CHECK_HIP(hipMemset(ix->d_stats.p, 0, INS_ALL * sizeof(int64_t)));
+        CIS_CHECK_HIP(hipHostMalloc((void**)&ix->h_ins, INS_ALL * sizeof(int64_t), hipHostMallocDefault));
+        for (int i = 0; i < INS_ALL; ++i) ix->h_ins[i] = 0;
     }
     return CIS_OK;
 }
@@ -814,16 +869,14 @@
             CIS_CHECK_HIP(hipMemsetAsync(stats + INS_NTOTAL, 0, 3 * sizeof(int64_t), st));
             hipLaunchKernelGGL(k_gcount_stats, dim3((unsigned)std::min<int64_t>(ceil_div(nc, 256), 1024)), dim3(256), 0, st, (const int64_t*)gcount, nc, stats);
         }
+        launch_cell_prefix(ix, st);
         CIS_CHECK_HIP(hipGetLastError());
-        CIS_CHECK_HIP(hipMemcpyAsync(ix->h_ins, ix->d_stats.p, INS_WORDS * sizeof(int64_t), hipMemcpyDeviceToHost, st));
+        CIS_CHECK_HIP(hipMemcpyAsync(ix->h_ins, ix->d_stats.p, INS_ALL * sizeof(int64_t), hipMemcpyDeviceToHost, st));
         CIS_CHECK_HIP(hipStreamSynchronize(st));
         if (ix->h_ins[INS_OVERFLOW] == 0) {
             s.n += ix->h_ins[acc_word];
             if (sel == 0) ix->n_inplace += 1;
-            ix->n_total = ix->h_ins[INS_NTOTAL];
-            ix->max_cell = ix->h_ins[INS_MAXCELL];
-            ix->nonempty_cells = ix->h_ins[INS_NONEMPTY];
-            ix->nb_indexed = ix->n_total;
+            adopt_cell_stats(ix);
             ix->stats_fresh = true;
             return CIS_OK;
         }
@@ -838,16 +891,14 @@
                            gsink, (const int64_t*)stats);
         CIS_CHECK_HIP(hipMemsetAsync(stats + INS_NTOTAL, 0, 3 * sizeof(int64_t), st));
         hipLaunchKernelGGL(k_gcount_stats, dim3((unsigned)std::min<int64_t>(ceil_div(nc, 256), 1024)), dim3(256), 0, st, (const int64_t*)gcount, nc, stats);
+        launch_cell_prefix(ix, st);
         CIS_CHECK_HIP(hipGetLastError());
-        CIS_CHECK_HIP(hipMemcpyAsync(ix->h_ins, ix->d_stats.p, INS_WORDS * sizeof(int64_t), hipMemcpyDeviceToHost, st));
+        CIS_CHECK_HIP(hipMemcpyAsync(ix->h_ins, ix->d_stats.p, INS_ALL * sizeof(int64_t), hipMemcpyDeviceToHost, st));
         CIS_CHECK_HIP(hipStreamSynchronize(st));
         if (ix->h_ins[INS_OVERFLOW] == 0) {
             s.n += ix->h_ins[acc_word];
             if (sel == 0) ix->n_inplace += 1;
-            ix->n_total = ix->h_ins[INS_NTOTAL];
-            ix->max_cell = ix->h_ins[INS_MAXCELL];
-            ix->nonempty_cells = ix->h_ins[INS_NONEMPTY];
-            ix->nb_indexed = ix->n_total;
+            adopt_cell_stats(ix);
             ix->stats_fresh = true;
             return CIS_OK;
         }
@@ -890,7 +941,7 @@
                        (const uint32_t*)apre, n, (const int64_t*)loff, (const int64_t*)lend, (const int64_t*)noff, (const uint32_t*)a0v, d_fine, M,
                        s.ids[nxt].as<int64_t>(), ncodes, cmaxp, stats);
     CIS_CHECK_HIP(hipGetLastError());
-    CIS_CHECK_HIP(hipMemcpyAsync(ix->h_ins, ix->d_stats.p, INS_WORDS * sizeof(int64_t), hipMemcpyDeviceToHost, st));
+    CIS_CHECK_HIP(hipMemcpyAsync(ix->h_ins, ix->d_stats.p, INS_ALL * sizeof(int64_t), hipMemcpyDeviceToHost, st));
     CIS_CHECK_HIP(hipStreamSynchronize(st));
     s.n += ix->h_ins[acc_word];
     if (sel == 0) ix->n_rebuild += 1;
@@ -905,7 +956,7 @@
 }
 
 static int stats_fetch(cis_index* ix, hipStream_t st) {
-    CIS_CHECK_HIP(hipMemcpyAsync(ix->h_ins, ix->d_stats.p, INS_WORDS * sizeof(int64_t), hipMemcpyDeviceToHost, st));
+    CIS_CHECK_HIP(hipMemcpyAsync(ix->h_ins, ix->d_stats.p, INS_ALL * sizeof(int64_t), hipMemcpyDeviceToHost, st));
     CIS_CHECK_HIP(hipStreamSynchronize(st));
     return CIS_OK;
 }
@@ -916,11 +967,9 @@
     const int64_t nc = ix->ncells;
     const unsigned grid = (unsigned)std::min<int64_t>(ceil_div(nc, 256), 1024);
     hipLaunchKernelGGL(k_gcount_stats, dim3(grid), dim3(256), 0, st, (const int64_t*)ix->d_gcount.as<int64_t>(), nc, stats);
+    launch_cell_prefix(ix, st);
     CIS_TRY(stats_fetch(ix, st));
-    ix->n_total = ix->h_ins[INS_NTOTAL];
-    ix->max_cell = ix->h_ins[INS_MAXCELL];
-    ix->nonempty_cells = ix->h_ins[INS_NONEMPTY];
-    ix->nb_indexed = ix->n_total;
+    adopt_cell_stats(ix);
     return CIS_OK;
 }
 
diff --git a/columbiaimagesearch_amd/csrc/lopq_plan.hip b/columbiaimagesearch_amd/csrc/lopq_plan.hip
--- a/columbiaimagesearch_amd/csrc/lopq_plan.hip
+++ b/columbiaimagesearch_amd/csrc/lopq_plan.hip
@@ -126,12 +126,14 @@
                                              WorkItem* __restrict__ items, TabDesc* __restrict__ tabs,
                                              int* __restrict__ grp_cnt , const int* __restrict__ grp_base ,
                                              int* __restrict__ grp_cur , int* __restrict__ tab_order ,
-                                             const int* __restrict__ only ) {
+                                             const int* __restrict__ only ,
+                                             const int64_t* __restrict__ d_totals ) {
     extern __shared__ __attribute__((aligned(16))) char smem[];
     int* t = reinterpret_cast<int*>(smem);
     const int q = blockIdx.x;
     const int lane = threadIdx.x;
     if (only && !only[q]) return;
+    if (EMIT && d_totals && d_totals[3] != 0) return;
     const CT* d0 = sorted + ((int64_t)q * 2 + 0) * V;
     const CT* d1 = sorted + ((int64_t)q * 2 + 1) * V;
     const uint16_t* o0 = order + ((int64_t)q * 2 + 0) * V;
@@ -822,7 +824,9 @@
                                                     volatile int64_t* __restrict__ host_totals , int64_t seq,
                                                     int* __restrict__ grp_cnt ,
                                                     int* __restrict__ grp_base, int n_groups,
-                                                    unsigned long long* __restrict__ hint_zero ) {
+                                                    unsigned long long* __restrict__ hint_zero ,
+                                                    int64_t cap_items, int64_t cap_tabs, int64_t cap_cand ) {
+    __shared__ int s_over;
     if (hint_zero && threadIdx.x == 0) { hint_zero[0] = 0ull; hint_zero[1] = 0ull; }
     constexpr int R = 8;
     __shared__ int s_wi[R][16], s_wt[R][16];
@@ -912,7 +916,15 @@
                 qbound[q] = 0x7ff0000000000000ull;
                 ri += plan[q].n_items; rt += plan[q].ntab0 + plan[q].ntab1;
             }
-            totals[0] = ri; totals[1] = rt; totals[2] = rc;
+            const int over = cap_items >= 0 && !cis_totals_fit(ri, rt, rc, cap_items, cap_tabs, cap_cand);
+            if (over) {
+                host_totals[13] = ri; host_totals[14] = rt; host_totals[15] = rc;
+                __threadfence_system();
+                host_totals[12] = seq;
+                ri = 0; rt = 0; rc = 0;
+            }
+            s_over = over;
+            totals[0] = ri; totals[1] = rt; totals[2] = rc; totals[3] = over;
             host_totals[0] = ri; host_totals[1] = rt; host_totals[2] = rc;
             __threadfence_system();
             host_totals[3] = seq;
@@ -925,8 +937,8 @@
     for (int r = 0; r < R; ++r) {
         const int q = r * 1024 + tid;
         if (q < nq) {
-            item_off[q] = s_base_i[r][wv] + xi[r] - ni[r];
-            tab_off[q] = s_base_t[r][wv] + xt[r] - nt[r];
+            item_off[q] = s_over ? 0 : s_base_i[r][wv] + xi[r] - ni[r];
+            tab_off[q] = s_over ? 0 : s_base_t[r][wv] + xt[r] - nt[r];
             qbound[q] = 0x7ff0000000000000ull;
         }
     }
@@ -1235,7 +1247,7 @@
         if (r.par_plan) dump_plan_dbg(nq);
 #endif
     hipLaunchKernelGGL((k_plan<CT, false>), dim3(nq), dim3(64), (size_t)V * sizeof(int), st, sorted, order, ix->gcount_ptr(), ix->loff_ptr(), nq, V,
-                       b.quota, r.seg_max, b.plan, nullptr, nullptr, nullptr, nullptr, b.f.grp_cnt, nullptr, nullptr, nullptr, b.plan_fb);
+                       b.quota, r.seg_max, b.plan, nullptr, nullptr, nullptr, nullptr, b.f.grp_cnt, nullptr, nullptr, nullptr, b.plan_fb, nullptr);
     return CIS_OK;
 }
 template int front_count<float>(Batch&, const Route&);
@@ -1254,10 +1266,48 @@
                            r.seg_max, b.plan, b.item_off, b.tab_off, b.items, b.tabs, nullptr, b.grp_base, b.grp_cur, b.tab_order, b.vis_list,
                            b.plan_fb, b.vis_cap, nullptr, 0);
     hipLaunchKernelGGL((k_plan<CT, true>), dim3(nq), dim3(64), (size_t)V * sizeof(int), st, sorted, order, ix->gcount_ptr(), ix->loff_ptr(), nq, V,
-                       b.quota, r.seg_max, b.plan, b.item_off, b.tab_off, b.items, b.tabs, nullptr, b.grp_base, b.grp_cur, b.tab_order, b.plan_fb);
+                       b.quota, r.seg_max, b.plan, b.item_off, b.tab_off, b.items, b.tabs, nullptr, b.grp_base, b.grp_cur, b.tab_order, b.plan_fb, b.d_tot);
 }
 template void emit_plan<float>(Batch&, const Route&);
 template void emit_plan<double>(Batch&, const Route&);
+
+int settle_pending_totals(cis_index* ix) {
+    if (!ix->stats_pending_seq) return CIS_OK;
+    const int64_t seq = ix->stats_pending_seq;
+    const auto t0 = std::chrono::steady_clock::now();
+    bool got = false;
+    for (;;) {
+        if (__atomic_load_n(&ix->h_totals[3], __ATOMIC_ACQUIRE) == seq) { got = true; break; }
+        if (std::chrono::steady_clock::now() - t0 > std::chrono::milliseconds(2)) break;
+    }
+    if (!got) {
+        CIS_CHECK_HIP(hipStreamSynchronize(ix->pending_stream));
+        CIS_REQUIRE(__atomic_load_n(&ix->h_totals[3], __ATOMIC_ACQUIRE) == seq, "plan totals did not arrive");
+    }
+    const int64_t items = ix->h_totals[0], tabs = ix->h_totals[1], cand = ix->h_totals[2];
+    ix->stats[0] += cand;
+    ix->stats[1] += items;
+    ix->stats[2] += tabs;
+    ix->stats_pending_seq = 0;
+    if (ix->ra_pending_est && __atomic_load_n(&ix->h_totals[12], __ATOMIC_ACQUIRE) != seq) {
+        ix->ra_pending_est->items = items; ix->ra_pending_est->tabs = tabs; ix->ra_pending_est->cand = cand;
+    }
+    ix->ra_pending_est = nullptr;
+    return CIS_OK;
+}
+
+int check_run_ahead_error(cis_index* ix) {
+    if (!ix->h_totals) return CIS_OK;
+    const int64_t bad = __atomic_load_n(&ix->h_totals[12], __ATOMIC_ACQUIRE);
+    if (bad == 0) return CIS_OK;
+    const long long it = ix->h_totals[13], tb = ix->h_totals[14], cd = ix->h_totals[15];
+    ix->h_totals[12] = 0;
+    for (int i = 0; i < cis_index::RA_ESTS; ++i) ix->ra_ests[i].nq = -1;
+    cis_set_error("an earlier batch ran ahead of its plan and the plan exceeded its bounds: %lld work items, %lld tables, %lld candidates "
+                  "against bounds of %lld, %lld, %lld (its results are empty); cis_index_set_run_ahead(ix, -1) turns the run-ahead off",
+                  it, tb, cd, (long long)ix->ra_cap[0], (long long)ix->ra_cap[1], (long long)ix->ra_cap[2]);
+    return CIS_EHIP;
+}
 
 int plan_totals(Batch& b, const Route& r) {
     cis_index* ix = b.ix;
@@ -1265,13 +1315,33 @@
     hipStream_t st = b.st;
     const int V = m->V, nq = b.nq, L = b.L;
     if (!ix->h_totals) {
-        CIS_CHECK_HIP(hipHostMalloc((void**)&ix->h_totals, 12 * sizeof(int64_t), hipHostMallocMapped | hipHostMallocCoherent));
+        CIS_CHECK_HIP(hipHostMalloc((void**)&ix->h_totals, 16 * sizeof(int64_t), hipHostMallocMapped | hipHostMallocCoherent));
         CIS_CHECK_HIP(hipHostGetDevicePointer((void**)&ix->d_h_totals, ix->h_totals, 0));
         ix->h_totals[3] = 0;
         ix->h_totals[4] = 0;
-        for (int i = 6; i < 12; ++i) ix->h_totals[i] = 0;
-    }
+        for (int i = 6; i < 16; ++i) ix->h_totals[i] = 0;
+    }
+    CIS_TRY(settle_pending_totals(ix));
     const int64_t seq = ++ix->plan_seq;
+    static const bool no_bounds = getenv("CIS_NO_BOUNDS") != nullptr;
+    static const bool ra_wait = getenv("CIS_RUN_AHEAD_WAIT") != nullptr;
+    CisBatchBound bound;
+    bound.ok = 0;
+    bool run_ahead = false;
+    cis_index::RunAheadEst* est = nullptr;
+    const bool ra_route = !r.big && !r.stream_hint && !r.par_plan && !r.tiny_cells && r.fast && r.split_tables && m->h <= 256 && ix->ncells <= 4096 &&
+                          nq <= 8192 && ix->world == 1 && m->M <= 8;
+    if (ra_route && !no_bounds && !ra_wait && ix->run_ahead_mode == 0 && !ix->ra_hold) {
+        CisCellStats cs;
+        cs.n_total = ix->n_total; cs.max_cell = ix->max_cell; cs.nonempty = ix->nonempty_cells; cs.ncells = ix->ncells;
+        cs.n_prefix = ix->n_prefix; cs.prefix = ix->cell_prefix;
+        bound = cis_batch_bound(cs, V, r.seg_max, b.quota, nq);
+        est = ix->ra_find(nq, b.quota, L);
+        const bool have_est = est != nullptr;
+        const double need = (double)bound.items * r.geom.S * sizeof(uint64_t) + (double)bound.tabs * m->nf * m->K * sizeof(double);
+        const double budget = (getenv("CIS_WORKSPACE_GB") ? atof(getenv("CIS_WORKSPACE_GB")) : 24.0) * 1.0e9;
+        run_ahead = bound.ok && have_est && need <= budget && bound.items < ((int64_t)1 << 30) && bound.tabs < ((int64_t)1 << 30);
+    }
     const int n_groups = 2 * V * GRP_SUB;
     const bool groups_apart = n_groups > 8192;
     int* grp_cnt = b.f.grp_cnt;
@@ -1279,12 +1349,22 @@
         hipLaunchKernelGGL(k_group_bases, dim3((n_groups + GROUP_TILE - 1) / GROUP_TILE), dim3(256), 0, st, grp_cnt, b.grp_base, n_groups,
                            reinterpret_cast<unsigned long long*>(grp_cnt + GRP_WORDS(V)), (uint32_t)(seq & 0x7fffffff) | 0x80000000u);
     hipLaunchKernelGGL(k_plan_scan, dim3(1), dim3(1024), 0, st, b.plan, nq, b.item_off, b.tab_off, b.totals, b.qbound, ix->d_h_totals, seq, grp_cnt, b.grp_base,
-                       groups_apart ? 0 : n_groups, b.plan_hint ? b.plan_hint + (b.hint_slot ^ 1) * 2 : nullptr);
+                       groups_apart ? 0 : n_groups, b.plan_hint ? b.plan_hint + (b.hint_slot ^ 1) * 2 : nullptr,
+                       run_ahead ? bound.items : (int64_t)-1, bound.tabs, bound.cand);
     volatile int64_t* h_tot = ix->h_totals;
     b.d_tot = nullptr;
     b.n_items = b.n_tabs = b.n_cand_all = 0;
-    {
-        static const bool no_bounds = getenv("CIS_NO_BOUNDS") != nullptr;
+    if (run_ahead) {
+        b.d_tot = b.totals;
+        b.n_items = bound.items; b.n_tabs = bound.tabs; b.n_cand_all = bound.cand;
+        b.est_items = est->items; b.est_cand = est->cand;
+        ix->stats_pending_seq = seq;
+        ix->pending_stream = st;
+        ix->ra_pending_est = est;
+        ix->ra_cap[0] = bound.items; ix->ra_cap[1] = bound.tabs; ix->ra_cap[2] = bound.cand;
+        ix->ra_counters[0] += 1;
+        ix->ra_counters[2] = bound.items; ix->ra_counters[3] = bound.tabs; ix->ra_counters[4] = bound.cand; ix->ra_counters[5] = bound.kvis;
+    } else {
         const int64_t q_eff = b.quota < 0 ? 0 : b.quota;
         const int64_t per_q = (q_eff < ix->n_total ? q_eff : ix->n_total) + ix->max_cell;
         const int64_t items_q = ix->nonempty_cells + per_q / r.seg_max + 2;
@@ -1300,6 +1380,8 @@
             b.n_tabs = (int64_t)nq * 2 * V;
             b.n_cand_all = (int64_t)nq * per_q;
             ix->stats_pending_seq = seq;
+            ix->pending_stream = st;
+            ix->ra_pending_est = nullptr;
         }
     }
     if (!b.d_tot) {
@@ -1317,7 +1399,17 @@
         host_timing(b, t0);
         b.n_items = h_tot[0]; b.n_tabs = h_tot[1]; b.n_cand_all = h_tot[2];
         ix->stats_pending_seq = 0;
-    }
+        if (ra_route) {
+            cis_index::RunAheadEst* e = ix->ra_find(nq, b.quota, L);
+            if (!e) { e = &ix->ra_ests[ix->ra_est_next]; ix->ra_est_next = (ix->ra_est_next + 1) % cis_index::RA_ESTS; }
+            e->nq = nq; e->quota = b.quota; e->L = L; e->n_total = ix->n_total;
+            e->items = b.n_items; e->tabs = b.n_tabs; e->cand = b.n_cand_all;
+            ix->ra_counters[1] += 1;
+            ix->ra_counters[2] = bound.ok ? bound.items : -1; ix->ra_counters[3] = bound.ok ? bound.tabs : -1;
+            ix->ra_counters[4] = bound.ok ? bound.cand : -1; ix->ra_counters[5] = bound.ok ? bound.kvis : -1;
+        }
+    }
+    if (!run_ahead) { b.est_items = b.n_items; b.est_cand = b.n_cand_all; }
     CIS_REQUIRE(b.n_items < ((int64_t)1 << 31) && b.n_tabs < ((int64_t)1 << 31), "query batch too large");
     return CIS_OK;
 }
diff --git a/columbiaimagesearch_amd/csrc/lopq_search.hip b/columbiaimagesearch_amd/csrc/lopq_search.hip
--- a/columbiaimagesearch_amd/csrc/lopq_search.hip
+++ b/columbiaimagesearch_amd/csrc/lopq_search.hip
@@ -1688,14 +1688,21 @@
 
 extern "C" int cis_index_last_stats(cis_index* ix, int64_t stats[4]) {
     CIS_REQUIRE(ix != nullptr && stats != nullptr, "NULL argument");
-    if (ix->stats_pending_seq) {
-        if (__atomic_load_n(&ix->h_totals[3], __ATOMIC_ACQUIRE) != ix->stats_pending_seq) CIS_CHECK_HIP(hipDeviceSynchronize());
-        ix->stats[0] += ix->h_totals[2];
-        ix->stats[1] += ix->h_totals[0];
-        ix->stats[2] += ix->h_totals[1];
-        ix->stats_pending_seq = 0;
-    }
+    CIS_TRY(settle_pending_totals(ix));
     for (int i = 0; i < 4; ++i) stats[i] = ix->stats[i];
+    return CIS_OK;
+}
+
+extern "C" int cis_index_set_run_ahead(cis_index* ix, int mode) {
+    CIS_REQUIRE(ix != nullptr, "index is NULL");
+    CIS_REQUIRE(mode == 0 || mode == -1, "run-ahead mode must be 0 (automatic) or -1 (always wait for the plan totals)");
+    ix->run_ahead_mode = mode;
+    return CIS_OK;
+}
+
+extern "C" int cis_index_run_ahead_counters(cis_index* ix, int64_t out[6]) {
+    CIS_REQUIRE(ix != nullptr && out != nullptr, "NULL argument");
+    for (int i = 0; i < 6; ++i) out[i] = ix->ra_counters[i];
     return CIS_OK;
 }
 
@@ -3062,7 +3069,7 @@
         ix->stats[1] += b.n_items;
         ix->stats[2] += b.n_tabs;
     }
-    r->geom3 = scan3_geom(M, K, L, b.n_items > 0 ? b.n_cand_all / b.n_items : 0, ix->force_two_pass);
+    r->geom3 = scan3_geom(M, K, L, b.est_items > 0 ? b.est_cand / b.est_items : 0, ix->force_two_pass);
     r->S = r->fast ? (r->use3 ? r->geom3.S : r->geom.S) : L;
     r->use5 = false;
     if (!r->stream && !r->big && r->fast && b.n_items > 0) {
@@ -3456,7 +3463,7 @@
     }
     CIS_TRY(mark(b, 3));
     if (r.fast) {
-        const bool many = n_items > nq + nq / 4;
+        const bool many = b.est_items > nq + nq / 4;
         if (L <= 128) merge_survivors_m<256>(b, r, many);
         else if (L <= 256) merge_survivors_m<512>(b, r, many);
         else if (L <= 440) merge_survivors_m<1024>(b, r, many);
@@ -3533,8 +3540,10 @@
     CIS_TRY(cis_index_ready(ix->base ? ix->base : ix));
     ix->sync_from_base();
     CIS_CHECK_HIP(hipSetDevice(ix->m->device));
+    CIS_TRY(check_run_ahead_error(ix));
     for (int i = 0; i < 4; ++i) ix->stats[i] = 0;
     ix->stats_pending_seq = 0;
+    ix->ra_pending_est = nullptr;
     int batch = (ix->batch_hint > 0 && ix->batch_hint_quota == quota) ? ix->batch_hint : QUERY_BATCH;
     for (int a = 0; a < nq;) {
         const int bn = (nq - a < batch) ? (nq - a) : batch;
diff --git a/columbiaimagesearch_amd/lopq/search.py b/columbiaimagesearch_amd/lopq/search.py
--- a/columbiaimagesearch_amd/lopq/search.py
+++ b/columbiaimagesearch_amd/lopq/search.py
@@ -433,6 +433,15 @@
         c = np.zeros(2, dtype=np.int64)
         _lib.check(_lib.lib().cis_index_stream_counters(self._ix, _lib.ptr(c)))
         return int(c[0]), int(c[1])
+
+    def set_run_ahead(self, automatic=True):
+        _lib.check(_lib.lib().cis_index_set_run_ahead(self._ix, 0 if automatic else -1))
+
+    def run_ahead_counters(self):
+        c = np.zeros(6, dtype=np.int64)
+        _lib.check(_lib.lib().cis_index_run_ahead_counters(self._ix, _lib.ptr(c)))
+        return {"ran_ahead": int(c[0]), "waited": int(c[1]), "items": int(c[2]), "tables": int(c[3]), "candidates": int(c[4]),
+                "kvis": int(c[5])}
 
     def last_stats(self):
         st = np.zeros(4, dtype=np.int64)
diff --git a/include/cis_hip.h b/include/cis_hip.h
--- a/include/cis_hip.h
+++ b/include/cis_hip.h
@@ -156,6 +156,8 @@
 int cis_index_set_profiling(cis_index* ix, int level );
 int cis_index_set_scan_mode(cis_index* ix, int mode);
 int cis_index_stream_counters(cis_index* ix, int64_t counters[2]);
+int cis_index_set_run_ahead(cis_index* ix, int mode);
+int cis_index_run_ahead_counters(cis_index* ix, int64_t out[6]);
 int cis_index_read_profile(cis_index* ix, double ms[5], int64_t* launches);
 
 #define CIS_CNN_SENTIBANK 1
```

New measurement: 22.83 million. 0.988x the previous value.
